# VCISwang/STCD

Hardware: AMD Instinct MI355X
Metric: image-pairs/sec (256x256 bf16 SiamUnet_diff train) (higher is better)
Workload: dtype bf16; 1 GPU; SiamUnet_diff(3,2) 256x256 full training step (fwd + cross_entropy + bwd + AdamW), 16 pairs/GPU, synthetic LEVIR-CD-shaped pairs resident in HBM; global_batch=16, image=256, parallelism=dp1

## Files before the change

include/stcd_hip.h:

```cpp
#ifndef STCD_HIP_H
#define STCD_HIP_H

#include <stdint.h>

#ifdef __cplusplus
extern "C" {
#endif

#define STCD_ABI_VERSION 2

#define STCD_ARCH_DIFF 0
#define STCD_ARCH_CONC 1
#define STCD_ARCH_SUB 2
#define STCD_ARCH_SNUNET 3
#define STCD_ARCH_SEGCD 4
#define STCD_ARCH_SEGCD_R18 5
#define STCD_ARCH_SEGCD_R34 6
#define STCD_ARCH_SEGCD_R101 7
#define STCD_ARCH_SEGCD_R152 8
#define STCD_ARCH_FCEF 9
#define STCD_ARCH_XCONC 10
#define STCD_ARCH_SNUNET_CONC 11
#define STCD_ARCH_SNUNET_CONC_DS 12
#define STCD_ARCH_UNETSEG 16
// ... 118 lines not shown
int64_t stcd_loss_iou_scratch_bytes(int batch, int classes, int64_t hw);
int stcd_loss_iou(const float* logits, const int64_t* target, int batch, int classes, int64_t hw, const float* weight, int mode,
                  float* loss_out, float* dlogits, void* scratch, void* hip_stream);
int stcd_confusion_update(const float* logits, const int64_t* target, int batch, int classes, int64_t hw,
                          int64_t* cm, void* hip_stream);

int stcd_adam_step(float* params, const float* grads, float* exp_avg, float* exp_avg_sq, int64_t numel, int64_t step,
                   double lr, double beta1, double beta2, double eps, double weight_decay, int decoupled, void* hip_stream);

int stcd_adam_hyper(int64_t step, double lr, double beta1, double beta2, double eps, double weight_decay, float* hyper_host8);
int stcd_adam_step_dev(float* params, const float* grads, float* exp_avg, float* exp_avg_sq, int64_t numel, const float* hyper_dev8,
                       int decoupled, void* hip_stream);

int stcd_pseudo_pair(const uint8_t* img_a, const uint8_t* donor, const uint8_t* mask, const uint8_t* change, const float* alpha,
                     const int32_t* erase_xywh, uint64_t seed, int batch, int height, int width, const float* mean3,
                     const float* std3, float* x1, float* x2, int64_t* c_label, int64_t* s_label_a, int64_t* s_label_b,
                     void* hip_stream);

int64_t stcd_augment_scratch_bytes(int n_images, int height, int width);
int stcd_augment(const float* x, const float* params, int n_images, int height, int width, const float* mean3, const float* std3,
                 float* out, void* scratch, int64_t scratch_bytes, void* hip_stream);

int stcd_scene_gather(const uint8_t* scene_a, const uint8_t* scene_b, int height, int width, int tile, int stride, int tiles_x,
                      int first_tile, int n_tiles, const float* mean3, const float* std3, float* x1, float* x2, void* hip_stream);
int stcd_scene_stitch(const float* logits, int classes, int height, int width, int tile, int stride, int tiles_x, int tiles_y,
                      int first_tile, int n_tiles, const float* window, float* acc, float* wsum, void* hip_stream);
int stcd_scene_finalize(const float* acc, const float* wsum, int classes, int height, int width, float threshold,
                        const uint8_t* label, uint8_t* mask, float* prob, int64_t* cm, void* hip_stream);
int stcd_scene_gather_d4(const uint8_t* scene_a, const uint8_t* scene_b, int height, int width, int tile, int stride, int tiles_x,
                         int first_tile, int n_tiles, const float* mean3, const float* std3, float* x1, float* x2, int d4,
                         void* hip_stream);
int stcd_scene_stitch_d4(const float* logits, int classes, int height, int width, int tile, int stride, int tiles_x, int tiles_y,
                         int first_tile, int n_tiles, const float* window, float* acc, float* wsum, int d4, void* hip_stream);
int stcd_scene_gather_one_d4(const uint8_t* scene, int height, int width, int tile, int stride, int tiles_x, int first_tile,
                             int n_tiles, const float* mean3, const float* std3, float* x, int d4, void* hip_stream);
#define STCD_SCENE_MAX_HEADS 3
int stcd_scene_stitch_heads_d4(const float* const* logits, int n_heads, int classes, int height, int width, int tile, int stride,
                               int tiles_x, int tiles_y, int first_tile, int n_tiles, const float* window, float* acc, float* wsum,
                               int d4, void* hip_stream);
int stcd_scene_finalize_seg(const float* acc, const float* wsum, int classes, int height, int width, float seg_threshold,
                            float change_threshold, const uint8_t* label_a, const uint8_t* label_b, const uint8_t* label_c,
                            uint8_t* seg_a, uint8_t* seg_b, uint8_t* change, uint8_t* gated, float* prob, int64_t* cm,
                            void* hip_stream);

#define STCD_SELFTRAIN_MAX_MODELS 8
int stcd_selftrain_score(const float* const* logits, int n_models, int batch, int classes, int64_t hw, float threshold,
                         const uint8_t* label, int mask_value, uint8_t* mask, int64_t* agree, int64_t* cm, void* hip_stream);

int stcd_scene_cell_agree(const uint8_t* const* masks, int n_models, int height, int width, int cell, int cells_x, int cells_y,
                          const uint8_t* label, int64_t* agree, int64_t* cm, void* hip_stream);
int stcd_mask_close(const uint8_t* in, int height, int width, int radius, int mask_value, uint8_t* out, void* hip_stream);

typedef struct stcd_conv_geom {
    int32_t n, hi, wi, ci, ldi;
    int32_t hm, wm, in_stride;
    int32_t ho, wo, out_stride, oy0, ox0;
    int32_t co, ldo;
    int32_t ntaps;
    int8_t dy[9], dx[9];
    int8_t pad_[2];
} stcd_conv_geom;

int stcd_op_conv(int dtype, int impl, const stcd_conv_geom* g, const void* in, const float* w, const float* bias,
                 void* out, void* scratch, int64_t scratch_bytes, void* hip_stream);
enum { STCD_CONV_SMALL = 0, STCD_CONV_RES = 1, STCD_CONV_TILE = 2, STCD_CONV_GEMM = 3, STCD_CONV_HALO = 4, STCD_CONV_DMA = 5 };
typedef struct stcd_conv_fused {
    int32_t kernel;
    int32_t groups;
    void* sum_acc;
    int32_t sum_c0, sum_c;
    float sum_scale1, sum_scale2;
    int32_t use_epi, relu;
    const void* gate;
    const void* res;
    int32_t ldg, ldr;
    float alpha, beta;
    const void* bw_y;
    const float* bw_stat;
    const float* bw_mask;
    void* bw_acc;
    int32_t bw_ldy;
    int32_t blocks, tiles_per_group, blocks_per_group, bn_rep;
    int32_t tile_m;
} stcd_conv_fused;
int stcd_op_conv_fused(const stcd_conv_geom* g, stcd_conv_fused* f, const void* in, const float* w, const float* bias, void* out,
                       void* scratch, int64_t scratch_bytes, void* hip_stream);
int stcd_op_wgrad(int dtype, int impl, const stcd_conv_geom* g, const void* in, const void* dout, float* dw,
                  void* scratch, int64_t scratch_bytes, void* hip_stream);
int64_t stcd_op_scratch_bytes(const stcd_conv_geom* g);

typedef struct stcd_map_geom {
    int32_t n, h, w, c, groups;
} stcd_map_geom;
int64_t stcd_op_ew_scratch_bytes(const stcd_map_geom* g);
int stcd_op_bn_act(int dtype, const stcd_map_geom* g, const void* y, int ldy, const float* gamma, const float* beta,
                   float* running_mean, float* running_var, const float* mask, int relu, int training, void* a, int lda,
                   void* pool, int ldp, float* stat, void* scratch, int64_t scratch_bytes, void* hip_stream);
int stcd_op_bn_act_pair(int dtype, const stcd_map_geom* g, const void* y, int ldy, const float* gamma, const float* beta,
                        float* running_mean, float* running_var, const float* mask, int fuse_mode, void* a, int lda, void* pool,
                        int ldp, void* fused, int ldf, float* stat, void* scratch, int64_t scratch_bytes, void* hip_stream);
int stcd_op_bn_act_bwd(int dtype, const stcd_map_geom* g, const void* da, int ldda, const void* y, int ldy, const float* stat,
                       const float* mask, int relu, void* dy, int lddy, float* dgamma, float* dbeta, void* scratch,
                       int64_t scratch_bytes, void* hip_stream);
int stcd_op_maxpool(int dtype, const stcd_map_geom* g, const void* a, int lda, void* pool, int ldp, void* hip_stream);
int stcd_op_maxpool_bwd(int dtype, const stcd_map_geom* g, const void* a, int lda, const void* dpool, int ldp, void* da, int ldda,
                        int accumulate, void* hip_stream);
int stcd_op_maxpool3(int dtype, const stcd_map_geom* g, const void* a, int lda, void* pool, int ldp, void* idx, void* hip_stream);
int stcd_op_maxpool3_bwd(int dtype, const stcd_map_geom* g, const void* idx, const void* dpool, int ldp, void* da, int ldda, void* hip_stream);
int64_t stcd_op_pairdw_scratch_bytes(const stcd_map_geom* g);
int stcd_op_pairdw(int dtype, const stcd_map_geom* g, const void* a, int lda, const float* w, const float* b, void* out, int ldo,
                   void* hip_stream);
int stcd_op_pairdw_bwd(int dtype, const stcd_map_geom* g, const void* a, int lda, const void* dout, int lddo, const float* w, void* da,
                       int ldda, float* dw, void* scratch, int64_t scratch_bytes, void* hip_stream);
int stcd_op_fuse(int dtype, int mode, const stcd_map_geom* g, const void* a, int lda, void* d, int ldd, void* hip_stream);
int stcd_op_fuse_bwd(int dtype, int mode, const stcd_map_geom* g, const void* a, int lda, const void* dd, int ldd, void* da, int ldda,
                     void* hip_stream);
int stcd_op_rep_pad(int dtype, const stcd_map_geom* g, void* d, int ld, int h0, int w0, void* hip_stream);
int stcd_op_rep_pad_bwd(int dtype, const stcd_map_geom* g, void* dd, int ld, int h0, int w0, void* hip_stream);
int stcd_op_skip_bwd(int dtype, int mode, const stcd_map_geom* g, const void* a, int lda, const void* y, int ldy, const void* dd,
                     int ldd, const void* dpool, int ldp, const float* stat, const float* mask, void* da, int ldda, void* dy,
                     int lddy, float* dgamma, float* dbeta, void* scratch, int64_t scratch_bytes, void* hip_stream);

int64_t stcd_op_cf_scratch_bytes(int64_t rows, int channels, int n, int q_tokens, int kv_tokens);
int stcd_op_cf_im2col(int dtype, const void* x, void* col, int ldc, int n, int h, int w, int c, int k, int stride, int pad, void* hip_stream);
int stcd_op_cf_col2im(int dtype, const void* dcol, int ldc, void* dx, int n, int h, int w, int c, int k, int stride, int pad, int accumulate,
                      void* hip_stream);
int stcd_op_cf_layernorm(int dtype, const void* x, void* y, const float* gamma, const float* beta, float* stats, int64_t rows, int c, float eps,
                         void* hip_stream);
int stcd_op_cf_layernorm_bwd(int dtype, const void* dy, const void* dy2, const void* x, const float* stats, const float* gamma, const void* add,
                             void* dx, float* dgamma, float* dbeta, void* scratch, int64_t rows, int c, void* hip_stream);
int stcd_op_cf_colsum(int dtype, const void* x, int64_t rows, int c, float* out, void* scratch, void* hip_stream);
int stcd_op_cf_attention(int dtype, const void* q, const void* kv, void* out, float* lse, int n, int q_tokens, int kv_tokens, int heads, int d,
                         float p, uint64_t seed, void* hip_stream);
int64_t stcd_op_cf_attention_scratch_bytes(int n, int q_tokens, int kv_tokens, int heads, int d);
int stcd_op_cf_attention_bwd(int dtype, const void* q, const void* kv, const void* out, const void* dout, const float* lse, void* dq, void* dkv,
                             void* scratch, int n, int q_tokens, int kv_tokens, int heads, int d, float p, uint64_t seed, void* hip_stream);
int stcd_op_cf_dwgelu(int dtype, const void* h, void* u, void* a, const float* w, const float* b, int n, int height, int width, int ch, float p,
                      uint64_t seed, void* hip_stream);
int64_t stcd_op_cf_dwgelu_scratch_bytes(int n, int height, int width, int ch);
int stcd_op_cf_dwgelu_bwd(int dtype, const void* h, const void* u, void* da, void* dh, const float* w, float* dw, float* db, void* scratch, int n,
                          int height, int width, int ch, float p, uint64_t seed, void* hip_stream);
int stcd_op_cf_resid_drop(int dtype, const void* x, const void* y, void* out, int n, int64_t rows_per_img, int c, float p, float path_p,
                          uint64_t seed, int backward, void* hip_stream);
int stcd_op_cf_bilinear(int dtype, const void* src, void* dst, int n, int h, int w, int out_h, int out_w, int c, int accumulate, int backward,
                        void* hip_stream);
int stcd_op_cf_elementwise(int dtype, int op, const void* x, const void* y, void* out, int64_t rows, int c, const float* alpha, float alpha_f,
                           float beta_f, float p, uint64_t seed, void* hip_stream);
int stcd_op_cf_prelu_bwd(int dtype, const void* dz, const void* y, void* dy, const float* alpha, float* dalpha, void* scratch, int64_t rows, int c,
                         void* hip_stream);

#ifdef __cplusplus
}
#endif
#endif
```

stcd_amd/_lib.py:

```python
from __future__ import annotations

import ctypes as C
import os

import torch

_HERE = os.path.dirname(os.path.abspath(__file__))
LIB_PATH = os.environ.get("STCD_LIB_PATH") or os.path.join(_HERE, "libstcd_hip.so")

ARCH_DIFF, ARCH_CONC, ARCH_SUB, ARCH_SNUNET, ARCH_SEGCD = 0, 1, 2, 3, 4
ARCH_SEGCD_R18, ARCH_SEGCD_R34, ARCH_SEGCD_R101, ARCH_SEGCD_R152 = 5, 6, 7, 8
ARCH_FCEF = 9
ARCH_XCONC = 10
ARCH_SNUNET_CONC = 11
ARCH_SNUNET_CONC_DS = 12
ARCH_UNETSEG = 16
ARCH_FFCTLCD = 32
ARCH_BASE_RESNET = 48
ARCH_BIT = 52
ARCH_CHANGEFORMER = 64
DTYPE_F32, DTYPE_BF16 = 0, 1
ARCH_IDS = {"diff": ARCH_DIFF, "conc": ARCH_CONC, "sub": ARCH_SUB, "fcef": ARCH_FCEF, "xconc": ARCH_XCONC, "snunet": ARCH_SNUNET, "snunet_conc": ARCH_SNUNET_CONC, "snunet_conc_ds": ARCH_SNUNET_CONC_DS, "segcd": ARCH_SEGCD,
            "segcd_resnet50": ARCH_SEGCD, "segcd_resnet18": ARCH_SEGCD_R18, "segcd_resnet34": ARCH_SEGCD_R34,
            "segcd_resnet101": ARCH_SEGCD_R101, "segcd_resnet152": ARCH_SEGCD_R152,
            "unetseg_resnet50": ARCH_UNETSEG, "unetseg_resnet18": ARCH_UNETSEG + 1, "unetseg_resnet34": ARCH_UNETSEG + 2,
            "unetseg_resnet101": ARCH_UNETSEG + 3, "unetseg_resnet152": ARCH_UNETSEG + 4,
            "ffctlcd_resnet50": ARCH_FFCTLCD, "ffctlcd_resnet18": ARCH_FFCTLCD + 1, "ffctlcd_resnet34": ARCH_FFCTLCD + 2,
            "ffctlcd_resnet101": ARCH_FFCTLCD + 3, "ffctlcd_resnet152": ARCH_FFCTLCD + 4,
            "base_resnet18_s5": ARCH_BASE_RESNET, "base_resnet18_s4": ARCH_BASE_RESNET + 1,
            "base_resnet34_s5": ARCH_BASE_RESNET + 2, "base_resnet34_s4": ARCH_BASE_RESNET + 3,
            "bit_s4_dd1_dh64": ARCH_BIT, "bit_s4_dd8_dh64": ARCH_BIT + 1, "bit_s4_dd8_dh8": ARCH_BIT + 2,
            "changeformer": ARCH_CHANGEFORMER}
DTYPE_IDS = {"fp32": DTYPE_F32, "f32": DTYPE_F32, "bf16": DTYPE_BF16}


class TensorInfo(C.Structure):
    _fields_ = [("name", C.c_char * 64), ("ndim", C.c_int32), ("shape", C.c_int64 * 4), ("offset", C.c_int64),
                ("numel", C.c_int64)]


class BnInfo(C.Structure):
    _fields_ = [("name", C.c_char * 64), ("channels", C.c_int32), ("calls_per_forward", C.c_int32),
                ("offset", C.c_int64)]


class DropoutInfo(C.Structure):
    _fields_ = [("name", C.c_char * 64), ("rows", C.c_int32), ("channels", C.c_int32), ("offset", C.c_int64)]


class ConvGeom(C.Structure):
    _fields_ = [("n", C.c_int32), ("hi", C.c_int32), ("wi", C.c_int32), ("ci", C.c_int32), ("ldi", C.c_int32),
                ("hm", C.c_int32), ("wm", C.c_int32), ("in_stride", C.c_int32),
                ("ho", C.c_int32), ("wo", C.c_int32), ("out_stride", C.c_int32), ("oy0", C.c_int32), ("ox0", C.c_int32),
                ("co", C.c_int32), ("ldo", C.c_int32), ("ntaps", C.c_int32),
                ("dy", C.c_int8 * 9), ("dx", C.c_int8 * 9), ("pad_", C.c_int8 * 2)]


class WsTensor(C.Structure):
    _fields_ = [("name", C.c_char * 96), ("offset_bytes", C.c_int64), ("n", C.c_int), ("h", C.c_int), ("w", C.c_int), ("c", C.c_int),
                ("ld", C.c_int), ("dtype", C.c_int)]


class CfConfig(C.Structure):
    _fields_ = [("in_ch", C.c_int32), ("out_ch", C.c_int32), ("embed_dims", C.c_int32 * 4), ("depths", C.c_int32 * 4),
                ("num_heads", C.c_int32 * 4), ("sr_ratios", C.c_int32 * 4), ("mlp_ratio", C.c_int32), ("embedding_dim", C.c_int32),
                ("patch1", C.c_int32), ("patch", C.c_int32), ("drop_rate", C.c_float), ("attn_drop", C.c_float),
                ("drop_path_rate", C.c_float), ("diff_drop", C.c_float)]


class CfSite(C.Structure):
    _fields_ = [("name", C.c_char * 96), ("ndim", C.c_int32), ("dims", C.c_int32 * 4), ("p", C.c_float)]


class MapGeom(C.Structure):
    _fields_ = [("n", C.c_int32), ("h", C.c_int32), ("w", C.c_int32), ("c", C.c_int32), ("groups", C.c_int32)]


CONV_SMALL, CONV_RES, CONV_TILE, CONV_GEMM, CONV_HALO, CONV_DMA = range(6)


class ConvFused(C.Structure):
    _fields_ = [("kernel", C.c_int32), ("groups", C.c_int32),
                ("sum_acc", C.c_void_p), ("sum_c0", C.c_int32), ("sum_c", C.c_int32), ("sum_scale1", C.c_float), ("sum_scale2", C.c_float),
                ("use_epi", C.c_int32), ("relu", C.c_int32), ("gate", C.c_void_p), ("res", C.c_void_p), ("ldg", C.c_int32), ("ldr", C.c_int32),
                ("alpha", C.c_float), ("beta", C.c_float),
                ("bw_y", C.c_void_p), ("bw_stat", C.c_void_p), ("bw_mask", C.c_void_p), ("bw_acc", C.c_void_p), ("bw_ldy", C.c_int32),
                ("blocks", C.c_int32), ("tiles_per_group", C.c_int32), ("blocks_per_group", C.c_int32), ("bn_rep", C.c_int32),
                ("tile_m", C.c_int32)]


_vp, _i, _i64, _f, _d = C.c_void_p, C.c_int, C.c_int64, C.c_float, C.c_double
_PROTOS = {
    "stcd_last_error": (C.c_char_p, []),
    "stcd_abi_version": (_i, []),
    "stcd_create": (_i, [_i, _i, _i, _i, C.POINTER(_vp)]),
    "stcd_destroy": (None, [_vp]),
    "stcd_cf_default_config": (_i, [C.POINTER(CfConfig)]),
    "stcd_create_changeformer": (_i, [C.POINTER(CfConfig), _i, C.POINTER(_vp)]),
    "stcd_output_floats": (_i64, [_vp]),
    "stcd_cf_output_info": (_i, [_vp, _i, C.POINTER(_i64), C.POINTER(_i), C.POINTER(_i)]),
    "stcd_cf_num_sites": (_i, [_vp]),
    "stcd_cf_site_get": (_i, [_vp, _i, C.POINTER(CfSite)]),
    "stcd_cf_site_seed": (C.c_uint32, [C.c_uint64, _i]),
    "stcd_cf_set_drop_rates": (_i, [_vp, _f, _f, _f]),
    "stcd_cf_set_aux_backward": (_i, [_vp, _i]),
    "stcd_set_wgrad_side": (_i, [_vp, _i]),
    "stcd_num_params": (_i, [_vp]),
    "stcd_param_info": (_i, [_vp, _i, C.POINTER(TensorInfo)]),
    "stcd_param_floats": (_i64, [_vp]),
    "stcd_num_bn": (_i, [_vp]),
    "stcd_bn_info_get": (_i, [_vp, _i, C.POINTER(BnInfo)]),
    "stcd_bn_floats": (_i64, [_vp]),
    "stcd_configure": (_i, [_vp, _i, _i, _i]),
    "stcd_workspace_bytes": (_i64, [_vp]),
    "stcd_num_dropout": (_i, [_vp]),
    "stcd_dropout_info_get": (_i, [_vp, _i, C.POINTER(DropoutInfo)]),
    "stcd_dropout_floats": (_i64, [_vp]),
    "stcd_set_dropout_p": (_i, [_vp, _f]),
    "stcd_forward": (_i, [_vp, _vp, _vp, _vp, _vp, _vp, C.c_uint64, _i, _vp, _vp, _vp]),
    "stcd_backward": (_i, [_vp, _vp, _vp, _vp, _vp, _i, _vp]),
    "stcd_grad_stage_range": (_i, [_vp, _i, C.POINTER(_i64), C.POINTER(_i64)]),
    "stcd_set_weights_tag": (_i, [_vp, C.c_uint64]),
    "stcd_set_debug": (_i, [_vp, _i]),
    "stcd_ws_tensor_count": (_i, [_vp]),
    "stcd_ws_tensor_get": (_i, [_vp, _i, C.POINTER(WsTensor)]),
    "stcd_profile_enable": (_i, [_vp, _i]),
    "stcd_profile_read": (_i, [_vp, _i, C.POINTER(C.c_double), C.POINTER(_i64), C.POINTER(C.c_double), C.POINTER(C.c_double)]),
    "stcd_profile_num_kernels": (_i, [_vp]),
    "stcd_profile_kernel": (_i, [_vp, _i, C.c_char_p, _i, C.POINTER(C.c_double), C.POINTER(_i64), C.POINTER(C.c_double), C.POINTER(C.c_double)]),
    "stcd_loss_scratch_bytes": (_i64, []),
    "stcd_loss_ce": (_i, [_vp, _vp, _i, _i, _i64, _i, _vp, _vp, _vp, _vp]),
    "stcd_loss_bce_dice": (_i, [_vp, _vp, _i64, _i, _vp, _vp, _vp, _vp]),
    "stcd_loss_contrastive": (_i, [_vp, _vp, _vp, _i64, _vp, _vp, _vp, _vp]),
    "stcd_loss_focal": (_i, [_vp, _vp, _i, _i, _i64, _vp, _f, _f, _i, _vp, _vp, _vp, _vp]),
    "stcd_loss_iou_scratch_bytes": (_i64, [_i, _i, _i64]),
    "stcd_loss_iou": (_i, [_vp, _vp, _i, _i, _i64, _vp, _i, _vp, _vp, _vp, _vp]),
    "stcd_confusion_update": (_i, [_vp, _vp, _i, _i, _i64, _vp, _vp]),
    "stcd_adam_step": (_i, [_vp, _vp, _vp, _vp, _i64, _i64, _d, _d, _d, _d, _d, _i, _vp]),
    "stcd_adam_hyper": (_i, [_i64, _d, _d, _d, _d, _d, C.POINTER(_f)]),
    "stcd_adam_step_dev": (_i, [_vp, _vp, _vp, _vp, _i64, _vp, _i, _vp]),
    "stcd_pseudo_pair": (_i, [_vp, _vp, _vp, _vp, _vp, _vp, C.c_uint64, _i, _i, _i, C.POINTER(_f), C.POINTER(_f), _vp, _vp, _vp, _vp, _vp, _vp]),
    "stcd_augment_scratch_bytes": (_i64, [_i, _i, _i]),
    "stcd_augment": (_i, [_vp, _vp, _i, _i, _i, C.POINTER(_f), C.POINTER(_f), _vp, _vp, _i64, _vp]),
    "stcd_scene_gather": (_i, [_vp, _vp, _i, _i, _i, _i, _i, _i, _i, C.POINTER(_f), C.POINTER(_f), _vp, _vp, _vp]),
    "stcd_scene_stitch": (_i, [_vp, _i, _i, _i, _i, _i, _i, _i, _i, _i, _vp, _vp, _vp, _vp]),
    "stcd_scene_finalize": (_i, [_vp, _vp, _i, _i, _i, _f, _vp, _vp, _vp, _vp, _vp]),
    "stcd_scene_gather_d4": (_i, [_vp, _vp, _i, _i, _i, _i, _i, _i, _i, C.POINTER(_f), C.POINTER(_f), _vp, _vp, _i, _vp]),
    "stcd_scene_stitch_d4": (_i, [_vp, _i, _i, _i, _i, _i, _i, _i, _i, _i, _vp, _vp, _vp, _i, _vp]),
    "stcd_scene_gather_one_d4": (_i, [_vp, _i, _i, _i, _i, _i, _i, _i, C.POINTER(_f), C.POINTER(_f), _vp, _i, _vp]),
    "stcd_scene_stitch_heads_d4": (_i, [C.POINTER(_vp), _i, _i, _i, _i, _i, _i, _i, _i, _i, _i, _vp, _vp, _vp, _i, _vp]),
    "stcd_scene_finalize_seg": (_i, [_vp, _vp, _i, _i, _i, _f, _f, _vp, _vp, _vp, _vp, _vp, _vp, _vp, _vp, _vp, _vp]),
    "stcd_selftrain_score": (_i, [C.POINTER(_vp), _i, _i, _i, _i64, _f, _vp, _i, _vp, _vp, _vp, _vp]),
    "stcd_scene_cell_agree": (_i, [C.POINTER(_vp), _i, _i, _i, _i, _i, _i, _vp, _vp, _vp, _vp]),
    "stcd_mask_close": (_i, [_vp, _i, _i, _i, _i, _vp, _vp]),
    "stcd_op_conv": (_i, [_i, _i, C.POINTER(ConvGeom), _vp, _vp, _vp, _vp, _vp, _i64, _vp]),
    "stcd_op_conv_fused": (_i, [C.POINTER(ConvGeom), C.POINTER(ConvFused), _vp, _vp, _vp, _vp, _vp, _i64, _vp]),
    "stcd_op_wgrad": (_i, [_i, _i, C.POINTER(ConvGeom), _vp, _vp, _vp, _vp, _i64, _vp]),
    "stcd_op_scratch_bytes": (_i64, [C.POINTER(ConvGeom)]),
    "stcd_op_ew_scratch_bytes": (_i64, [C.POINTER(MapGeom)]),
    "stcd_op_bn_act": (_i, [_i, C.POINTER(MapGeom), _vp, _i, _vp, _vp, _vp, _vp, _vp, _i, _i, _vp, _i, _vp, _i, _vp, _vp, _i64, _vp]),
    "stcd_op_bn_act_pair": (_i, [_i, C.POINTER(MapGeom), _vp, _i, _vp, _vp, _vp, _vp, _vp, _i, _vp, _i, _vp, _i, _vp, _i, _vp, _vp, _i64, _vp]),
    "stcd_op_bn_act_bwd": (_i, [_i, C.POINTER(MapGeom), _vp, _i, _vp, _i, _vp, _vp, _i, _vp, _i, _vp, _vp, _vp, _i64, _vp]),
    "stcd_op_maxpool": (_i, [_i, C.POINTER(MapGeom), _vp, _i, _vp, _i, _vp]),
    "stcd_op_maxpool_bwd": (_i, [_i, C.POINTER(MapGeom), _vp, _i, _vp, _i, _vp, _i, _i, _vp]),
    "stcd_op_maxpool3": (_i, [_i, C.POINTER(MapGeom), _vp, _i, _vp, _i, _vp, _vp]),
    "stcd_op_maxpool3_bwd": (_i, [_i, C.POINTER(MapGeom), _vp, _vp, _i, _vp, _i, _vp]),
    "stcd_op_pairdw_scratch_bytes": (_i64, [C.POINTER(MapGeom)]),
    "stcd_op_pairdw": (_i, [_i, C.POINTER(MapGeom), _vp, _i, _vp, _vp, _vp, _i, _vp]),
    "stcd_op_pairdw_bwd": (_i, [_i, C.POINTER(MapGeom), _vp, _i, _vp, _i, _vp, _vp, _i, _vp, _vp, _i64, _vp]),
    "stcd_op_fuse": (_i, [_i, _i, C.POINTER(MapGeom), _vp, _i, _vp, _i, _vp]),
    "stcd_op_fuse_bwd": (_i, [_i, _i, C.POINTER(MapGeom), _vp, _i, _vp, _i, _vp, _i, _vp]),
    "stcd_op_rep_pad": (_i, [_i, C.POINTER(MapGeom), _vp, _i, _i, _i, _vp]),
    "stcd_op_rep_pad_bwd": (_i, [_i, C.POINTER(MapGeom), _vp, _i, _i, _i, _vp]),
    "stcd_op_skip_bwd": (_i, [_i, _i, C.POINTER(MapGeom), _vp, _i, _vp, _i, _vp, _i, _vp, _i, _vp, _vp, _vp, _i, _vp, _i, _vp, _vp, _vp, _i64, _vp]),
    "stcd_op_cf_scratch_bytes": (_i64, [_i64, _i, _i, _i, _i]),
    "stcd_op_cf_im2col": (_i, [_i, _vp, _vp, _i, _i, _i, _i, _i, _i, _i, _i, _vp]),
    "stcd_op_cf_col2im": (_i, [_i, _vp, _i, _vp, _i, _i, _i, _i, _i, _i, _i, _i, _vp]),
    "stcd_op_cf_layernorm": (_i, [_i, _vp, _vp, _vp, _vp, _vp, _i64, _i, _f, _vp]),
    "stcd_op_cf_layernorm_bwd": (_i, [_i, _vp, _vp, _vp, _vp, _vp, _vp, _vp, _vp, _vp, _vp, _i64, _i, _vp]),
    "stcd_op_cf_colsum": (_i, [_i, _vp, _i64, _i, _vp, _vp, _vp]),
    "stcd_op_cf_attention": (_i, [_i, _vp, _vp, _vp, _vp, _i, _i, _i, _i, _i, _f, C.c_uint64, _vp]),
    "stcd_op_cf_attention_scratch_bytes": (_i64, [_i, _i, _i, _i, _i]),
    "stcd_op_cf_attention_bwd": (_i, [_i, _vp, _vp, _vp, _vp, _vp, _vp, _vp, _vp, _i, _i, _i, _i, _i, _f, C.c_uint64, _vp]),
    "stcd_op_cf_dwgelu": (_i, [_i, _vp, _vp, _vp, _vp, _vp, _i, _i, _i, _i, _f, C.c_uint64, _vp]),
    "stcd_op_cf_dwgelu_scratch_bytes": (_i64, [_i, _i, _i, _i]),
    "stcd_op_cf_dwgelu_bwd": (_i, [_i, _vp, _vp, _vp, _vp, _vp, _vp, _vp, _vp, _i, _i, _i, _i, _f, C.c_uint64, _vp]),
    "stcd_op_cf_resid_drop": (_i, [_i, _vp, _vp, _vp, _i, _i64, _i, _f, _f, C.c_uint64, _i, _vp]),
    "stcd_op_cf_bilinear": (_i, [_i, _vp, _vp, _i, _i, _i, _i, _i, _i, _i, _i, _vp]),
    "stcd_op_cf_elementwise": (_i, [_i, _i, _vp, _vp, _vp, _i64, _i, _vp, _f, _f, _f, C.c_uint64, _vp]),
    "stcd_op_cf_prelu_bwd": (_i, [_i, _vp, _vp, _vp, _vp, _vp, _vp, _i64, _i, _vp]),
}
EXPORTS = tuple(_PROTOS)

_lib = None


class StcdError(RuntimeError):
    pass


def lib():
    global _lib
    if _lib is None:
        if not os.path.exists(LIB_PATH):
            raise StcdError(
                f"{LIB_PATH} is missing: build it with `python -c 'import __graft_entry__ as g; g.build()'` "
                "or `make -C stcd_amd/csrc`.  The engine has no CPU fallback.")
        l = C.CDLL(LIB_PATH)
        for name, (res, args) in _PROTOS.items():
            fn = getattr(l, name)
            fn.restype, fn.argtypes = res, args
        if l.stcd_abi_version() != 2:
            raise StcdError("libstcd_hip.so ABI version mismatch")
        _lib = l
    return _lib


def check(rc: int):
    if rc != 0:
        raise StcdError(lib().stcd_last_error().decode("utf-8", "replace"))
```

stcd_amd/csrc/common.h:

```cpp
#pragma once
#include <hip/hip_runtime.h>
#include <stdint.h>
#include <stdio.h>
#include <stdlib.h>
#include <string>
#include <string.h>

#include "../../include/stcd_hip.h"

namespace stcd {

typedef __bf16 bf16;

enum DType { F32 = STCD_DTYPE_F32, BF16 = STCD_DTYPE_BF16 };
inline size_t dsize(int dt) { return dt == BF16 ? 2 : 4; }

void set_error(const std::string& msg);

static inline int env_int(const char* name, int dflt) { const char* v = getenv(name); return v ? atoi(v) : dflt; }
static inline bool env_flag(const char* name, bool dflt) { const char* v = getenv(name); return v && v[0] == (dflt ? '0' : '1') ? !dflt : dflt; }

#define STCD_CHECK_AS(fn, cond, msg)                                       \
    do {                                                                   \
        if (!(cond)) {                                                     \
// ... 171 lines not shown

void launch_conv_ref(int dt, const stcd_conv_geom& g, const void* in, const float* w, int kpad, int wld,
                     const float* bias, void* out, bool out_nchw_f32, hipStream_t s);
void launch_wgrad_ref(int dt, const stcd_conv_geom& g, const void* in, const void* dout, float* dw, int kpad, int wld,
                      hipStream_t s);
void launch_wgrad_ref_f64(int dt, const stcd_conv_geom& g, const void* in, const void* dout, double* dw, int kpad, int wld,
                          hipStream_t s);

struct ConvMfmaPlan {
    int CiB = 0, nchunks = 0, KS = 0, modeB = 0, NT = 0, NTtot = 0;
    int64_t wf_elems = 0;
    bool ok = false;
};
ConvMfmaPlan conv_mfma_plan(const stcd_conv_geom& g);
void launch_pack_frag(const stcd_conv_geom& g, const ConvMfmaPlan& p, const float* w, int kpad, int wld, void* dst,
                      hipStream_t s);
int launch_conv_mfma(const stcd_conv_geom& g, const ConvMfmaPlan& p, const void* in, const void* wf, const float* bias,
                     void* out, bool out_nchw_f32, hipStream_t s);
bool conv_mfma_x4_ok(const stcd_conv_geom g[4], const ConvMfmaPlan p[4]);
int launch_conv_mfma_x4(const stcd_conv_geom g[4], const ConvMfmaPlan p[4], const void* in, const void* const wf[4],
                        const float* bias, void* out, hipStream_t s);
struct ConvResPlan {
    int NT = 0, CW = 32, nslices = 0, P = 0, blocks = 0;
    int filt_bytes = 0, lds_bytes = 0;
    int single_halo = 0;
    bool ok = false;
};
ConvResPlan conv_res_plan(const stcd_conv_geom& g, const ConvMfmaPlan& p, int groups);
struct BwdSum {
    const void* Y = nullptr; int ldy = 0;
    const float* stat = nullptr;
    const float* mask = nullptr;
    long long* acc = nullptr;
    int groups = 1;
};
int launch_conv_res(const stcd_conv_geom& g, const ConvMfmaPlan& p, const ConvResPlan& rp, const void* in, const void* wf,
                    const float* bias, void* out, int groups, long long* stat_acc, int cpad, hipStream_t s, int stat_c0 = 0,
                    float s1_scale = BN_FS1, float s2_scale = BN_FS2, const XfSrc* xf = nullptr, const BwdSum* bs = nullptr);
bool conv_res_bwdsum_ok(const stcd_conv_geom& g, const ConvResPlan& rp);
bool conv_res_xf_ok(const stcd_conv_geom& g, const ConvResPlan& rp, int groups, const XfSrc& xf);
struct ConvTilePlan {
    int NT = 0, nparts = 0, nbuf = 0, nslices = 0, P = 0, blocks = 0, ntiles = 0;
    int filt_bytes = 0, lds_bytes = 0;
    bool ok = false;
};
ConvTilePlan conv_tile_plan(const stcd_conv_geom& g, const ConvMfmaPlan& p, int groups);
int launch_conv_tile(const stcd_conv_geom& g, const ConvMfmaPlan& p, const ConvTilePlan& tp, const void* in, const void* wf,
                     const float* bias, void* out, int groups, long long* stat_acc, int cpad, hipStream_t s, int stat_c0 = 0,
                     float s1_scale = BN_FS1, float s2_scale = BN_FS2);
struct ConvGemmPlan {
    int W = 0;
    int tiles_m = 0, tiles_n = 0, blocks = 0, lds_bytes = 0;
    int pix_chunks = 0;
    bool ok = false;
};
ConvGemmPlan conv_gemm_plan(const stcd_conv_geom& g, const ConvMfmaPlan& p, int groups);
struct ConvEpi {
    int relu = 0;
    const void* gate = nullptr; int ldg = 0;
    const void* res = nullptr; int ldr = 0;
    float alpha = 1.f, beta = 1.f;
};
int launch_conv_gemm(const stcd_conv_geom& g, const ConvMfmaPlan& p, const ConvGemmPlan& gp, const void* in, const void* wf,
                   const float* bias, void* out, int groups, long long* stat_acc, int cpad, hipStream_t s, int stat_c0 = 0,
                   float s1_scale = BN_FS1, float s2_scale = BN_FS2, const ConvEpi* epi = nullptr);
struct ConvHaloPlan {
    int NH = 0;
    int nslices = 0, P = 0, blocks = 0, lds_bytes = 0;
    bool ok = false;
};
ConvHaloPlan conv_halo_plan(const stcd_conv_geom& g, const ConvMfmaPlan& p);
int launch_conv_halo(const stcd_conv_geom& g, const ConvMfmaPlan& p, const ConvHaloPlan& hp, const void* in, const void* wf,
                     const float* bias, void* out, hipStream_t s, const ConvEpi* epi = nullptr);

struct ConvDmaPlan {
    int tiles_m = 0, tiles_n = 0, blocks = 0, lds_bytes = 0;
    bool ok = false;
};
ConvDmaPlan conv_dma_plan(const stcd_conv_geom& g, const ConvMfmaPlan& p);
int launch_conv_dma(const stcd_conv_geom& g, const ConvMfmaPlan& p, const ConvDmaPlan& dp, const void* in, const void* wf,
                    const float* bias, void* out, hipStream_t s, const ConvEpi* epi = nullptr);

bool conv_small_ok(const stcd_conv_geom& g, const ConvMfmaPlan& p);
int conv_small_blocks(const stcd_conv_geom& g, int groups);
int launch_conv_small(const stcd_conv_geom& g, const void* in, const void* wf_modeB, const float* bias, void* out,
                      bool out_nchw_f32, int groups, long long* stat_acc, int cpad, hipStream_t s, const XfSrc* xf = nullptr,
                      const BwdSum* bs = nullptr);
bool conv_small_call_ok(const stcd_conv_geom& g, int groups, const XfSrc* xf);
bool conv_small_bwdsum_ok(const stcd_conv_geom& g);
struct WgradMfmaPlan {
    int WCI = 1, NTW = 1, gx = 1, gy = 1, gz = 1;
    int64_t slab_floats = 0;
    int wi_valid = 0;
    int gemm = 0;
    int dma = 0;
    bool ok = false;
};
WgradMfmaPlan wgrad_mfma_plan(const stcd_conv_geom& g, int kpad, int wld, bool allow_wide = false, int force_co64 = -1);
int launch_wgrad_mfma(const stcd_conv_geom& g, const WgradMfmaPlan& p, const void* in, const void* dout, float* slab,
                      int kpad, int wld, hipStream_t s);
struct WgradJob {
    stcd_conv_geom g;
    int64_t in_off, dout_off, slab_off;
    int kpad, wld;
    int dymin, dxmin, HH, HWp;
    int tiles_x, tiles_y, ntiles;
    int xrow_bytes;
    int x_bytes, y_bytes;
    int co_valid;
    unsigned in_bytes, dout_bytes;
    int gx, gy, gz;
    int start;
    int lds_bytes;
    int wi_valid;
    int dma_L, dma_nk;
    int pad_;
    int64_t xf_stat_off, xf_mask_off;
    int xf_C, xf_groups, xf_npg, pad2_;
};
WgradMfmaPlan wgrad_gemm_plan(const stcd_conv_geom& g, int kpad, int wld);
WgradJob wgrad_gemm_make_job(const stcd_conv_geom& g, const WgradMfmaPlan& p, int64_t in_off, int64_t dout_off, int64_t slab_off,
                             int kpad, int wld);
int launch_wgrad_gemm_group(int W, const WgradJob* jobs_dev, int njobs, int total_blocks, const char* base, hipStream_t s);
WgradMfmaPlan wgrad_dma_plan(const stcd_conv_geom& g, int kpad, int wld);
void wgrad_dma_set_split(WgradMfmaPlan& p, const stcd_conv_geom& g, int S, int kpad, int wld);
WgradJob wgrad_dma_make_job(const stcd_conv_geom& g, const WgradMfmaPlan& p, int64_t in_off, int64_t dout_off, int64_t slab_off,
                            int kpad, int wld);
int launch_wgrad_dma_group(const WgradJob* jobs_dev, int njobs, int total_blocks, const char* base, hipStream_t s);
WgradJob wgrad_make_job(const stcd_conv_geom& g, const WgradMfmaPlan& p, int64_t in_off, int64_t dout_off, int64_t slab_off,
                        int kpad, int wld);
void wgrad_job_set_xf(WgradJob& a, int64_t stat_off, int64_t mask_off, int C, int groups, int npg);
int wgrad_variant_slots(int WCI, int NTW, bool t9, int lds_bytes);
int launch_wgrad_group(int WCI, int NTW, bool t9, const WgradJob* jobs_dev, int njobs, int total_blocks, int lds_bytes,
                       const char* base, hipStream_t s, bool xf = false);
struct PackSpec;
struct ReduceJob {
    int64_t start, count;
    int64_t slab_off;
    int64_t out_off;
    int64_t slab_stride;
    int gx, ntaps, K, N, kpad, wld;
    int ks, kn_major;
    int8_t ky[9], kx[9];
    int8_t tiled, parts, pad_[4];
};
void launch_reduce_jobs(const ReduceJob* jobs_dev, int njobs, int64_t total, const char* ws, float* grads, hipStream_t s);
void launch_reduce_dw(const float* slab, int gx, const stcd_conv_geom& g, int K, int N, int kpad, int wld,
                      const PackSpec* ps, float* out, hipStream_t s);

struct PackSpec {
    int ks;
    int kn_major;
    int K, N, wld;
    int kpad;
    int ntaps;
    int8_t ky[9], kx[9];
};
void launch_pack_w(const PackSpec& ps, const float* src, float* dst, hipStream_t s);
void launch_unpack_dw(const PackSpec& ps, const double* dwe, float* gsrc, hipStream_t s);

struct PackJob {
    int64_t start, count;
    int64_t src_off;
    int64_t dst_off;
    int kind;
    PackSpec ps;
    int Ci, Co, CiB, nchunks, KS, NTtot, modeB;
    int aux;
};
void launch_pack_jobs(const PackJob* jobs_dev, int njobs, int64_t total, const float* params, char* ws, hipStream_t s);
// ... 243 lines not shown
```

stcd_amd/csrc/engine.hip:

```cpp
#include <algorithm>
#include <climits>
#include <cstdint>
#include <array>
#include <cstring>
#include <memory>
#include <vector>

#include "common.h"

namespace stcd {

static thread_local std::string g_err;
void set_error(const std::string& msg) { g_err = msg; }

enum ConvKind { K_CONV3 = 0, K_CONVT3_S1 = 1, K_UPCONV = 2, K_CONV1 = 3, K_CONVT2 = 4, K_CONV3_S2 = 5, K_CONV1_S2 = 6, K_STEM7 = 7 };

struct TRef { int64_t off = -1; int ld = 0; };
struct GRef { int64_t off = -1; int ld = 0; int64_t goff = 0; };

static inline int round8(int c) { return (c + 7) & ~7; }

struct ConvW {
    std::string name;
    int kind = 0, cin = 0, cout = 0;
    int kin_p = 0, nout_p = 0;
    int64_t w_off = 0, b_off = 0;
    PackSpec fwd{}, dgrad{};
    int64_t wpk_fwd = -1, wpk_dgrad = -1, dwe = -1;
    int64_t dwe_floats = 0;
};
struct BnP {
    std::string name;
    int C = 0, calls = 1;
    int64_t g_off = 0, b_off = 0;
    int64_t run_off = 0;
};
struct DropP { std::string name; int rows = 0, C = 0; int64_t off = 0; };

struct ConvOp {
    stcd_conv_geom g{};
    int conv = -1; bool dgrad = false;
    int tap0 = 0;
    int kreal = 0, nreal = 0;
    ConvMfmaPlan plan; int64_t wf = -1;
    bool small = false;
    ConvResPlan res; int res_groups = 1;
    ConvGemmPlan gemm;
    ConvDmaPlan dma;
    ConvHaloPlan halo;
    ConvTilePlan tile;
};
struct WgradOp {
    stcd_conv_geom g{};
    int conv = -1, tap0 = 0, kreal = 0, nreal = 0;
    WgradMfmaPlan plan;
    int64_t slab = -1;
    int stage = 0;
    int64_t in_off = -1, dout_off = -1;
    bool grouped = false;
    int group = -1;
    int64_t xf_stat_off = -1, xf_mask_off = -1; int xf_C = 0, xf_groups = 1, xf_npg = 1;
    bool own_taps = false;
    int8_t oky[9] = {0}, okx[9] = {0};
};
struct WgradGroup {
    int WCI = 1, NTW = 1; bool t9 = false;
    bool xf = false;
    int gemm = 0;
    int dma = 0;
    std::vector<WgradJob> jobs;
    int total_blocks = 0, lds_bytes = 0;
    int64_t table_off = -1;
    double flops = 0.0, bytes = 0.0;
    int seen = 0; bool launched = false;
};

struct Cbrd {
    ConvOp fwd, dgr; WgradOp wg;
    int conv = -1, bn = -1, drop = -1;
    int N = 0, H = 0, W = 0, groups = 1, npg = 0;
    TRef in; int K = 0;
    TRef Y; GRef A; TRef P; TRef dPool; bool pool = false;
    GRef dA; TRef dY; TRef dIn; bool has_dIn = false;
    int64_t stat = -1;
    int64_t facc = -1, bacc = -1;
    const Cbrd* dgr_bwd = nullptr;
    bool bwd_sums_fused = false;
    int64_t dgr_sum_acc = -1; int dgr_sum_c0 = 0, dgr_sum_C = 0;
    TRef fuse_dst;
    bool virt = false; const Cbrd* xsrc = nullptr;
};
struct XConc {
    int level = 0, C = 0;
    int64_t w_off = 0, b_off = 0;
    int bn1 = -1;
    TRef G, dG, R, dR;
    int64_t stat1 = -1, facc1 = -1, bacc1 = -1, part = -1;
    Cbrd res;
};
struct UpConv {
    int conv = -1, level = 0;
    int N = 0, h = 0, w = 0, Ho = 0, Wo = 0, C = 0;
    TRef in, out, dOut, dIn;
    ConvOp fwd[4], dgr; WgradOp wg[4];
    int64_t bias_acc = -1; bool bias_fused = false;
};

enum ProfClass { PC_CONV = 0, PC_WGRAD = 1, PC_BN_STATS = 2, PC_BN_ACT = 3, PC_BN_BWD_REDUCE = 4, PC_BN_BWD_APPLY = 5,
                 PC_POOL_FUSE = 6, PC_PACK = 7, PC_COUNT = 8 };
struct ProfRec { hipEvent_t a, b; int klass; int name_id; double flops, bytes; };
struct Prof {
    bool on = false;
    std::vector<ProfRec> recs;
    std::vector<hipEvent_t> pool;
    std::vector<std::string> names;
    size_t used = 0;
    int intern(const std::string& n) {
        for (size_t i = 0; i < names.size(); ++i)
            if (names[i] == n) return (int)i;
        names.push_back(n);
        return (int)names.size() - 1;
    }
    hipEvent_t get() {
        if (used == pool.size()) { hipEvent_t ev; (void)hipEventCreate(&ev); pool.push_back(ev); }
        return pool[used++];
    }
    ~Prof() { for (auto ev : pool) (void)hipEventDestroy(ev); }
};

struct ViewRef { int64_t off = 0; int ld = 0; int64_t goff = 0; int gmask = 1; };
struct GLayer {
    std::string name;
    int conv = -1, bn = -1, kind = K_CONV3;
    int N = 0, Hi = 0, Wi = 0, Ho = 0, Wo = 0, K = 0, C = 0, groups = 2, npg = 0;
    bool relu = true;
    TRef in, Y, A, res;
    TRef dA, dIn, dRes;
    bool has_dIn = true;
    std::vector<ViewRef> extra_dst;
    std::vector<ViewRef> grad_src;
    bool grad_base = true;
    ConvOp fwd, dgr[4]; int ndgr = 0; WgradOp wg[8]; int nwg = 0;
    int64_t stat = -1, coef = -1, facc = -1, bacc = -1;
    int g_first = 0;
};
enum GStepKind { GS_LAYER = 0, GS_MAXPOOL = 1, GS_UPSAMPLE = 2, GS_ABSDIFF = 3, GS_BCONV = 4, GS_ABSPAIR = 5, GS_BILINEAR = 6,
                 GS_TOKENIZE = 7, GS_TOKENENC = 8, GS_TOKENDEC = 9 };
struct GStep { int kind = GS_LAYER; int layer = -1; TRef src, dst, dsrc, ddst; int N = 0, h = 0, w = 0, C = 0; };

struct SrcSlice { TRef src; TRef dsrc; int C = 0; int prod = -1; int grp = -1; };
struct NBlock {
    std::string name;
    int c1 = -1, bn1 = -1, c2 = -1, bn2 = -1;
    int N = 0, H = 0, W = 0, groups = 1, npg = 0, Cin = 0, C = 0;
    TRef in, dIn;
    std::vector<SrcSlice> srcs;
    int up = -1;
    TRef Y1, A1, Y2, Out, P, dOut, dP, dZ2, dA1;
    bool pool = false;
    int64_t stat1 = -1, stat2 = -1;
    int64_t facc1 = -1, bacc1 = -1, facc2 = -1, bacc2 = -1;
    int64_t d1_sum_acc = -1; int d1_sum_c0 = 0, d1_sum_C = 0;
    std::vector<ViewRef> extra_dst;
    std::vector<ViewRef> grad_src;
    bool grad_base = false;
    ConvOp f1, f2, d1, d2; WgradOp w1, w2;
};
struct SnUp {
    int conv = -1, N = 0, h = 0, w = 0, C = 0;
    TRef src, dsrc, out, dOut, tmp;
    ConvOp fwd[4], dgr; WgradOp wg[4];
    int64_t bias_acc = -1; bool bias_fused = false; int coff = 0;
};

struct CfPlan;
struct stcd_engine_impl {
    Prof prof;
    std::shared_ptr<CfPlan> cf;
    std::vector<NBlock> sn_blocks;
    std::vector<SnUp> sn_ups;
    std::vector<int> sn_order;
    std::vector<XConc> xc;
    int sn_final = -1;
    int64_t sn_w[4] = {0, 0, 0, 0};
    TRef snE, sndE, snZ, sndZ;
    int64_t sn_pool = -1, sn_argm = -1, sn_att = -1, sn_hid = -1, sn_sums = -1, sn_dpool = -1, sn_part = -1;
    int64_t sn_dout_begin = -1, sn_dout_end = -1;
    ConvOp sn_final_fwd, sn_final_dgr; WgradOp sn_final_wg;
    int64_t snc_w[5] = {0, 0, 0, 0, 0}, snc_b[5] = {0, 0, 0, 0, 0}, snc_scratch = -1;
    std::vector<GLayer> g_layers;
    std::vector<GStep> g_fwd;
    int g_stem = -1, g_head_conv = -1;
    int debug_flags = 0;
    std::vector<stcd_ws_tensor> ws_tensors;
    std::vector<std::array<int, 4>> g_blocks;
    int seg_x = 4, seg_layers[4] = {3, 4, 6, 3};
    int seg_dates = 2;
    bool seg_ffc = false;
    TRef g_pool_idc;
    std::vector<std::array<int, 2>> g_dec;
    TRef gP0, gdP0, gX3, gdX3, gFuseTmp;
    int64_t g_pool_idx = -1;
    int64_t g_stem_part = -1;
    int64_t g_raw3 = -1, g_draw3 = -1;
    ConvOp g_head_fwd, g_head_dgr; WgradOp g_head_wg;
    bool bres = false; int seg_nstage = 4;
    int g_head_c = 16;
    int g_cls = -1, g_pred_conv = -1;
    ConvOp g_pred_fwd, g_pred_dgr; WgradOp g_pred_wg;
    int64_t g_pred_bias_acc = -1;
    struct BitPlan {
        bool on = false; int L = 1, dh = 64;
        int64_t pos_off = 0, wa_off = 0, enc_off = 0, dec_off = 0;
        int64_t tok_in = -1, tok_out = -1, dtok_out = -1, dtok_in = -1, stat = -1, AP = -1, dAP = -1, xs = -1, dG = -1, dec_part = -1,
                dmh = -1, dm = -1, enc_part = -1, tok_part = -1;
        TRef dec_din;
    } bit;
    int arch = 0, in_ch = 3, label = 2, dt = F32;
    int64_t min_bn_count = 0;
    float drop_p = 0.2f;
    std::vector<stcd_tensor_info> params;
    int64_t param_floats = 0, enc_param_end = 0;
    std::vector<ConvW> convs;
    std::vector<BnP> bns;
    int64_t bn_floats = 0;
    bool configured = false, fwd_training = false;
    int B = 0, H = 0, W = 0;
    std::vector<DropP> drops;
    int64_t drop_floats = 0;
    int64_t ws_bytes = 0;
    std::vector<Cbrd> enc, dec;
    std::vector<UpConv> ups;
    int final_conv = -1;
    ConvOp final_fwd, final_dgr; WgradOp final_wg;
    const Cbrd* final_dgr_bwd = nullptr;
    const Cbrd* final_xsrc = nullptr;
    int use_virt = 0;
    int fc_virt_layers = 0;
    std::vector<ConvOp*> conv_ops;
    int64_t slab = -1, slab_floats = 0;
    std::vector<WgradOp*> wgrad_ops;
    std::vector<WgradGroup> wgroups[2];
    std::vector<ReduceJob> rjobs[2];
    int64_t rjobs_total[2] = {0, 0}, rjobs_off[2] = {-1, -1};
    std::vector<PackJob> jobs[2];
    int64_t jobs_total[2] = {0, 0}, jobs_off[2] = {-1, -1};
    const void* jobs_uploaded_ws = nullptr;
    uint64_t weights_tag = 0, packed_tag = 0;
    const void* packed_ws = nullptr; const void* packed_params = nullptr; int packed_level = -1;
    TRef X0, G, finalIn, dFinalIn;
    int Hs[5] = {0}, Ws[5] = {0};
    TRef D[4], dD[4], P[4], dP[4];
    int64_t zero_begin = -1, zero_end = -1;
    int64_t final_bias_acc = -1;
    std::vector<BiasJob> bias_jobs; int64_t bias_jobs_off = -1;
    int64_t masks = -1, dwe_begin = -1, dwe_end = -1, scratch8 = -1;
    int use_mfma = 1, use_small = 1, use_wgroup = 1, use_res = 1, use_skip_fused = 1, use_act_fuse = 1, use_gemm = 1, use_skip_recompute = 1, use_bwdsum = 1, use_bwdsum_res = 0, use_tile = 1, use_halo = 0;
    int wg_side_on = 1;
    static constexpr int WG_SIDE_DIV = 4;
    static constexpr int WGROUP_ROUNDS = 1, WGROUP_MIN_TILES = 8;
    bool wg_early = false; hipStream_t wg_cur_side = nullptr;
    hipStream_t wg_side = nullptr; hipEvent_t wg_fork = nullptr, wg_join = nullptr; int wg_side_dev = -1;
};

}

using namespace stcd;
struct stcd_engine : stcd_engine_impl {};

namespace stcd {

static const int ENC_STAGE_CONVS[4] = {2, 2, 3, 3};
static const int ENC_C[4] = {16, 32, 64, 128};
static const int SKIP_IDX[4] = {1, 3, 6, 9};

static void add_param(stcd_engine& e, const std::string& name, std::initializer_list<int64_t> shape, int64_t* off_out) {
    stcd_tensor_info ti;
    memset(&ti, 0, sizeof(ti));
    snprintf(ti.name, sizeof(ti.name), "%s", name.c_str());
    ti.ndim = (int)shape.size();
    int64_t n = 1;
    int i = 0;
    for (auto s : shape) { ti.shape[i++] = s; n *= s; }
    ti.numel = n;
    ti.offset = e.param_floats;
    *off_out = ti.offset;
    e.param_floats += (n + 3) & ~(int64_t)3;
    e.params.push_back(ti);
}

static void make_specs(ConvW& c, bool need_dgrad) {
    if (c.kind == K_STEM7) {
        c.fwd = PackSpec{}; c.dgrad = PackSpec{};
        c.fwd.ks = 7; c.fwd.K = c.cin; c.fwd.N = c.cout; c.fwd.kpad = c.kin_p; c.fwd.wld = c.nout_p;
        return;
    }
    if (c.kind == K_CONV3_S2) {
        PackSpec& f = c.fwd;
        f.ks = 3; f.K = c.cin; f.N = c.cout; f.kpad = c.kin_p; f.wld = c.nout_p; f.ntaps = 9; f.kn_major = 0;
        {
            int t = 0;
            for (int py = 0; py < 2; ++py)
                for (int px = 0; px < 2; ++px)
                    for (int ky = 0; ky < 3; ++ky)
                        for (int kx = 0; kx < 3; ++kx)
                            if ((ky != 1) == (py == 1) && (kx != 1) == (px == 1)) { f.ky[t] = ky; f.kx[t] = kx; ++t; }
        }
        PackSpec& d = c.dgrad;
        d.ks = 3; d.K = c.cout; d.N = c.cin; d.kpad = c.nout_p; d.wld = round8(c.cin); d.ntaps = need_dgrad ? 9 : 0; d.kn_major = 1;
        int t = 0;
        for (int py = 0; py < 2; ++py)
            for (int px = 0; px < 2; ++px)
                for (int dy = 0; dy <= py; ++dy)
                    for (int dx = 0; dx <= px; ++dx) { d.ky[t] = py + 1 - 2 * dy; d.kx[t] = px + 1 - 2 * dx; ++t; }
        return;
    }
    if (c.kind == K_CONV1 || c.kind == K_CONVT2 || c.kind == K_CONV1_S2) {
        const int ks = c.kind == K_CONVT2 ? 2 : 1;
        PackSpec& f = c.fwd;
        f.ks = ks; f.K = c.cin; f.N = c.cout; f.kpad = c.kin_p; f.wld = c.nout_p;
        f.ntaps = ks * ks;
        f.kn_major = c.kind == K_CONVT2;
        for (int t = 0; t < f.ntaps; ++t) { f.ky[t] = t / ks; f.kx[t] = t % ks; }
        PackSpec& d = c.dgrad;
        d.ks = ks; d.K = c.cout; d.N = c.cin; d.kpad = c.nout_p; d.wld = round8(c.cin);
        d.ntaps = need_dgrad ? ks * ks : 0;
        d.kn_major = c.kind != K_CONVT2;
        for (int t = 0; t < ks * ks; ++t) { d.ky[t] = t / ks; d.kx[t] = t % ks; }
        return;
    }
    PackSpec& f = c.fwd;
    f.ks = 3;
    f.K = c.cin; f.N = c.cout; f.kpad = c.kin_p; f.wld = c.nout_p;
    PackSpec& d = c.dgrad;
    d.ks = 3;
    d.K = c.cout; d.N = c.cin; d.kpad = c.nout_p; d.wld = round8(c.cin);
    d.ntaps = 0;
    if (c.kind == K_CONV3 || c.kind == K_CONVT3_S1) {
        f.ntaps = 9;
        f.kn_major = c.kind == K_CONVT3_S1;
// ... 114 lines not shown
        }
    }
}

struct Bump {
    int64_t cur = 0;
    int64_t take(int64_t bytes) {
        int64_t o = cur;
        cur += (bytes + 255) & ~(int64_t)255;
        return o;
    }
};

static int conv_index(const stcd_engine& e, const std::string& name) {
    for (size_t i = 0; i < e.convs.size(); ++i)
        if (e.convs[i].name == name) return (int)i;
    return -1;
}
static int bn_index(const stcd_engine& e, const std::string& name) {
    for (size_t i = 0; i < e.bns.size(); ++i)
        if (e.bns[i].name == name) return (int)i;
    return -1;
}

static stcd_conv_geom geom3(int N, int H, int W, int K, int ldi, int co, int ldo) {
    stcd_conv_geom g;
    memset(&g, 0, sizeof(g));
    g.n = N; g.hi = H; g.wi = W; g.ci = K; g.ldi = ldi;
    g.hm = H; g.wm = W; g.in_stride = 1;
    g.ho = H; g.wo = W; g.out_stride = 1; g.oy0 = 0; g.ox0 = 0;
    g.co = co; g.ldo = ldo;
    g.ntaps = 9;
    for (int t = 0; t < 9; ++t) { g.dy[t] = (int8_t)(t / 3 - 1); g.dx[t] = (int8_t)(t % 3 - 1); }
    return g;
}

static stcd_conv_geom geom_up_phase(const UpConv& U, int py, int px, int ldi, int ldo, int* tap0) {
    stcd_conv_geom g;
    memset(&g, 0, sizeof(g));
    g.n = U.N; g.hi = U.h; g.wi = U.w; g.ci = U.C; g.ldi = ldi;
    g.hm = U.h; g.wm = U.w; g.in_stride = 1;
    g.ho = U.Ho; g.wo = U.Wo; g.out_stride = 2; g.oy0 = py; g.ox0 = px;
    g.co = U.C; g.ldo = ldo;
    int t = 0;
    for (int dy = 0; dy <= py; ++dy)
        for (int dx = 0; dx <= px; ++dx) { g.dy[t] = (int8_t)dy; g.dx[t] = (int8_t)dx; ++t; }
    g.ntaps = t;
    static const int start[4] = {0, 1, 3, 5};
    *tap0 = start[py * 2 + px];
    return g;
}

static void conv_work(const stcd_engine& e, const stcd_conv_geom& g, int kreal, int nreal, double* flops, double* bytes);

static void pick_gemm_or_res(const stcd_engine& e, ConvOp& op, const stcd_conv_geom& g, int groups) {
    if (!e.use_gemm || op.small) return;
    if (op.res.ok && !(e.cf && op.res.NT == 1)) return;
    op.gemm = conv_gemm_plan(g, op.plan, groups);
    if (!op.gemm.ok) return;
    op.res = ConvResPlan();
    if ((int64_t)g.n * g.hm * g.wm >= 256 * 192) op.dma = conv_dma_plan(g, op.plan);
    if (e.use_halo && (int64_t)g.n * ((g.hm + 15) / 16) * ((g.wm + 15) / 16) >= 512) op.halo = conv_halo_plan(g, op.plan);
}

constexpr int TILE_MAX_TILES = 512;
static void pick_tile(const stcd_engine& e, ConvOp& op, const stcd_conv_geom& g, int groups) {
    if (!e.use_tile || !op.res.ok || op.gemm.ok || op.small) return;
    const ConvTilePlan tp = conv_tile_plan(g, op.plan, groups);
    if (tp.ok && tp.ntiles <= TILE_MAX_TILES) op.tile = tp;
}

static WgradMfmaPlan pick_wgrad_plan(const stcd_engine& e, const stcd_conv_geom& g, int kpad, int wld) {
    if (e.use_gemm && e.use_wgroup && 2.0 * g.n * g.hm * g.wm * (double)g.ci * g.co >= 0.8e9) {
        WgradMfmaPlan p = wgrad_gemm_plan(g, kpad, wld);
        if (p.ok) return p;
    }
    if (e.use_wgroup && (g.ntaps == 9 || (e.cf && g.ntaps == 4)) && (int64_t)g.n * g.hm * g.wm >= 65536) {
        WgradMfmaPlan p = wgrad_dma_plan(g, kpad, wld);
        if (p.ok) return p;
    }
    return wgrad_mfma_plan(g, kpad, wld, is_snunet(e.arch) || (e.cf && g.ntaps == 9));
}

static void plan_conv(const stcd_engine& e, ConvOp& op, int groups, bool with_tile) {
    op.plan = conv_mfma_plan(op.g);
    op.small = conv_small_ok(op.g, op.plan);
    if (e.use_res && !op.small) op.res = conv_res_plan(op.g, op.plan, groups);
    pick_gemm_or_res(e, op, op.g, groups);
    if (with_tile) pick_tile(e, op, op.g, groups);
}
static bool conv_on_ref(bool mfma, const ConvOp& op) { return !(mfma && op.plan.ok && op.wf >= 0); }
struct Binder {
    stcd_engine& e; Bump& ws;
    bool with_tile = false;
    void conv(ConvOp& op, const stcd_conv_geom& g, int conv, bool dgrad, int tap0, int kreal, int nreal, int groups = 1) const {
        op = ConvOp();
        op.g = g; op.conv = conv; op.dgrad = dgrad; op.tap0 = tap0; op.kreal = kreal; op.nreal = nreal; op.res_groups = groups;
        if (e.dt == BF16) plan_conv(e, op, groups, with_tile);
        if (op.plan.ok) op.wf = ws.take(op.plan.wf_elems * 2);
        e.conv_ops.push_back(&op);
    }
    void stem(ConvOp& op, const stcd_conv_geom& g, int conv, int groups) const {
        op = ConvOp();
        op.g = g; op.conv = conv; op.kreal = e.convs[conv].cin; op.nreal = g.co; op.res_groups = groups;
        op.plan = conv_mfma_plan(g);
        if (g.ldi == 8 && g.co % 64 == 0) op.gemm = conv_gemm_plan(g, op.plan, groups);
        op.gemm.pix_chunks = 1;
        if (!op.gemm.ok) return;
        op.wf = ws.take(op.plan.wf_elems * 2);
        e.conv_ops.push_back(&op);
    }
    void wgrad(WgradOp& op, const stcd_conv_geom& g, int conv, int64_t in_off, int64_t dout_off, int stage = 0, int tap0 = 0,
               int wi_valid = 0, const int8_t* own_ky = nullptr, const int8_t* own_kx = nullptr) const {
        const ConvW& cv = e.convs[conv];
        op = WgradOp();
        op.g = g; op.conv = conv; op.tap0 = tap0; op.kreal = cv.cin; op.nreal = cv.cout;
        op.in_off = in_off; op.dout_off = dout_off; op.stage = stage;
        op.own_taps = own_ky != nullptr;
        for (int t = 0; t < g.ntaps && op.own_taps; ++t) { op.oky[t] = own_ky[t]; op.okx[t] = own_kx[t]; }
        if (e.dt == BF16) { op.plan = pick_wgrad_plan(e, g, cv.fwd.kpad, cv.fwd.wld); op.plan.wi_valid = wi_valid; }
        e.wgrad_ops.push_back(&op);
    }
};
static void take_ref_images(stcd_engine& e, Bump& ws, bool with_dwe = true) {
    for (auto& c : e.convs) {
        c.wpk_fwd = ws.take((int64_t)c.fwd.ntaps * c.fwd.kpad * c.fwd.wld * 4);
        if (c.dgrad.ntaps) c.wpk_dgrad = ws.take((int64_t)c.dgrad.ntaps * c.dgrad.kpad * c.dgrad.wld * 4);
    }
    e.dwe_begin = ws.cur;
    for (auto& c : e.convs) {
        c.dwe_floats = (int64_t)c.fwd.ntaps * c.fwd.kpad * c.fwd.wld;
        c.dwe = with_dwe ? ws.take(c.dwe_floats * 8) : -1;
    }
    e.dwe_end = ws.cur;
}

static bool same_group(const WgradGroup& G, const WgradOp& op) {
    const bool t9 = !op.plan.dma && op.g.ntaps == 9;
    return G.gemm == op.plan.gemm && G.dma == op.plan.dma && G.WCI == op.plan.WCI && G.NTW == op.plan.NTW && G.t9 == t9 && G.xf == (op.xf_C > 0);
}

static bool cf_side_on() { static const bool on = env_flag("STCD_CF_SIDE", true); return on; }

static void build_pack_jobs(stcd_engine& e, Bump& ws) {
    for (int st = 0; st < 2; ++st) { e.rjobs[st].clear(); e.rjobs_total[st] = 0; }
    for (int st = 0; st < 2; ++st) e.wgroups[st].clear();
    if (e.dt == BF16 && e.use_mfma) {
        if (e.use_wgroup) {
            for (WgradOp* op : e.wgrad_ops) {
                if (!op->plan.ok) continue;
                const bool t9 = !op->plan.dma && op->g.ntaps == 9;
                std::vector<WgradGroup>& gs = e.wgroups[op->stage];
                size_t gi = 0;
                while (gi < gs.size() && !same_group(gs[gi], *op)) ++gi;
                if (gi == gs.size()) { WgradGroup g; g.WCI = op->plan.WCI; g.NTW = op->plan.NTW; g.t9 = t9; g.gemm = op->plan.gemm; g.dma = op->plan.dma; g.xf = op->xf_C > 0; gs.push_back(g); }
                op->grouped = true;
            }
            for (int st = 0; st < 2; ++st)
                for (WgradGroup& G : e.wgroups[st]) {
                    if (G.gemm) { G.lds_bytes = 2 * 2 * G.gemm * (64 * 64 + 8 * 32); continue; }
                    if (G.dma) {
                        G.lds_bytes = 128 * 1024;
                        std::vector<WgradOp*> dops;
                        for (WgradOp* op : e.wgrad_ops)
                            if (op->grouped && op->stage == st && op->plan.dma) dops.push_back(op);
                        auto blocks_at = [&](int64_t kt) {
                            int64_t b = 0;
                            for (WgradOp* op : dops) {
                                const int64_t M = (int64_t)op->g.n * op->g.hi * op->g.wi;
                                b += ((M + kt * 64 - 1) / (kt * 64)) * op->plan.gy * op->plan.gz;
                            }
                            return b;
                        };
                        int64_t lo = 1, hi = 1;
                        const int dma_blocks = e.wg_side_on && cf_side_on() ? 192 : 256;
                        while (blocks_at(hi) > dma_blocks) hi *= 2;
                        while (lo < hi) { const int64_t mid = (lo + hi) / 2; if (blocks_at(mid) <= dma_blocks) hi = mid; else lo = mid + 1; }
                        for (WgradOp* op : dops) {
                            const ConvW& cv = e.convs[op->conv];
                            const int64_t M = (int64_t)op->g.n * op->g.hi * op->g.wi;
                            int64_t S = (M + lo * 64 - 1) / (lo * 64);
                            const int64_t slab_bytes = (int64_t)op->g.ntaps * cv.fwd.kpad * cv.fwd.wld * 4;
                            S = std::min<int64_t>(S, std::max<int64_t>(1, ((int64_t)64 << 20) / slab_bytes));
                            wgrad_dma_set_split(op->plan, op->g, (int)S, cv.fwd.kpad, cv.fwd.wld);
                        }
                        continue;
                    }
                    std::vector<WgradOp*> ops;
                    int64_t W = 0;
                    for (WgradOp* op : e.wgrad_ops)
                        if (op->grouped && op->stage == st && same_group(G, *op)) {
                            ops.push_back(op);
                            const int64_t ntiles = (int64_t)op->g.n * ((op->g.wm + 15) / 16) * ((op->g.hm + 7) / 8);
// ... 217 lines not shown
            L.conv = conv_index(e, std::string("conv") + d.sfx[j]);
            L.bn = bn_index(e, std::string("bn") + d.sfx[j]);
            L.drop = add_drop(std::string("do") + d.sfx[j], B, d.cout[j]);
            const int C = d.cout[j];
            L.N = B; L.H = h; L.W = w; L.groups = 1; L.npg = B;
            L.in = in; L.K = K;
            L.Y = plain(B, h, w, C);
            TRef a = plain(B, h, w, C), da = plain(B, h, w, C);
            L.A.off = a.off; L.A.ld = C; L.A.goff = 0;
            L.dA.off = da.off; L.dA.ld = C; L.dA.goff = 0;
            L.dY = da;
            L.has_dIn = true; L.dIn = dIn;
            L.stat = ws.take((int64_t)4 * C * 4);
            e.dec.push_back(L);
            in = a; dIn = da; K = C;
            prevA = a; prevdA = da;
        }
    }
    if (fc_cross(e)) {
        for (int s = 0; s < 4; ++s) {
            XConc& X = e.xc[s];
            const int C = ENC_C[s], h = e.Hs[s], w = e.Ws[s];
            X.G = plain(B, h, w, C); X.dG = plain(B, h, w, C); X.R = plain(B, h, w, C); X.dR = plain(B, h, w, C);
            X.stat1 = ws.take((int64_t)4 * C * 4);
            X.part = ws.take(pairdw_partial_floats(B, h, w, C) * 4);
            Cbrd& L = X.res;
            L.drop = -1; L.N = B; L.H = h; L.W = w; L.groups = 1; L.npg = B;
            L.in = X.R; L.K = C;
            L.Y = plain(B, h, w, C);
            L.A.off = e.D[s].off + C * T; L.A.ld = e.D[s].ld; L.A.goff = 0;
            L.dA.off = e.dD[s].off + C * T; L.dA.ld = e.dD[s].ld; L.dA.goff = 0;
            L.dY = plain(B, h, w, C);
            L.has_dIn = true; L.dIn = X.dR;
            L.stat = ws.take((int64_t)4 * C * 4);
        }
    }
    e.G = plain(B, H, W, 8);
    for (auto& X : e.xc) {
        X.facc1 = za.take(bn_acc_bytes(1, X.C)); X.bacc1 = za.take(bn_acc_bytes(1, X.C));
        X.res.facc = za.take(bn_acc_bytes(1, X.C)); X.res.bacc = za.take(bn_acc_bytes(1, X.C));
    }
    for (auto& L : e.enc) { L.facc = za.take(bn_acc_bytes(L.groups, e.convs[L.conv].cout)); L.bacc = za.take(bn_acc_bytes(L.groups, e.convs[L.conv].cout)); }
    for (auto& L : e.dec) { L.facc = za.take(bn_acc_bytes(L.groups, e.convs[L.conv].cout)); L.bacc = za.take(bn_acc_bytes(L.groups, e.convs[L.conv].cout)); }
    for (auto& U : e.ups) U.bias_acc = za.take(bn_acc_bytes(1, U.C));
    e.final_bias_acc = za.take(bn_acc_bytes(1, 8));
    if (za.cur > e.zero_end) { set_error("internal: zero arena overflow"); return 1; }
    e.scratch8 = ws.take(256);
    e.masks = ws.take(e.drop_floats * 4);
    take_ref_images(e, ws);

    e.conv_ops.clear();
    e.wgrad_ops.clear();
    e.slab_floats = 0;
    const Binder bind{e, ws, true};
    auto wg_stage = [&](int conv) { return e.convs[conv].w_off < e.enc_param_end ? 1 : 0; };
    auto bind_cbrd = [&](Cbrd& L) {
        const ConvW& cv = e.convs[L.conv];
        bind.conv(L.fwd, geom3(L.N, L.H, L.W, L.K, L.in.ld, cv.cout, L.Y.ld), L.conv, false, 0, cv.cin, cv.cout, L.groups);
        bind.wgrad(L.wg, geom3(L.N, L.H, L.W, L.K, L.in.ld, cv.cout, L.dY.ld), L.conv, L.in.off, L.dY.off, wg_stage(L.conv));
        if (L.has_dIn)
            bind.conv(L.dgr, geom3(L.N, L.H, L.W, cv.dgrad.kpad, L.dY.ld, cv.cin, L.dIn.ld), L.conv, true, 0, cv.cout, cv.cin,
                      (e.use_bwdsum && e.use_bwdsum_res) ? L.groups : 1);
    };
    for (auto& L : e.enc) bind_cbrd(L);
    for (auto& L : e.dec) bind_cbrd(L);
    for (auto& X : e.xc) bind_cbrd(X.res);
    for (auto& U : e.ups) {
        const ConvW& cv = e.convs[U.conv];
        for (int ph = 0; ph < 4; ++ph) {
            int tap0;
            stcd_conv_geom g = geom_up_phase(U, ph >> 1, ph & 1, U.in.ld, U.out.ld, &tap0);
            bind.conv(U.fwd[ph], g, U.conv, false, tap0, U.C, U.C);
            bind.wgrad(U.wg[ph], g, U.conv, U.in.off, U.dOut.off, wg_stage(U.conv), tap0);
        }
        stcd_conv_geom gd;
        memset(&gd, 0, sizeof(gd));
        gd.n = U.N; gd.hi = U.Ho; gd.wi = U.Wo; gd.ci = cv.dgrad.kpad; gd.ldi = U.dOut.ld;
        gd.hm = U.h; gd.wm = U.w; gd.in_stride = 2;
        gd.ho = U.h; gd.wo = U.w; gd.out_stride = 1;
        gd.co = U.C; gd.ldo = U.dIn.ld;
        gd.ntaps = 9;
        for (int t = 0; t < 9; ++t) { gd.dy[t] = (int8_t)(t / 3 - 1); gd.dx[t] = (int8_t)(t % 3 - 1); }
        bind.conv(U.dgr, gd, U.conv, true, 0, U.C, U.C);
    }
    {
        const ConvW& cv = e.convs[e.final_conv];
        bind.conv(e.final_fwd, geom3(B, H, W, cv.kin_p, e.finalIn.ld, e.label, e.label), e.final_conv, false, 0, cv.cin, e.label);
        bind.wgrad(e.final_wg, geom3(B, H, W, cv.kin_p, e.finalIn.ld, e.label, 8), e.final_conv, e.finalIn.off, e.G.off, wg_stage(e.final_conv));
        bind.conv(e.final_dgr, geom3(B, H, W, cv.dgrad.kpad, 8, cv.cin, e.dFinalIn.ld), e.final_conv, true, 0, e.label, cv.cin);
    }
    e.slab = ws.take(e.slab_floats * 4);

    for (auto& L : e.enc) { L.dgr_bwd = nullptr; L.bwd_sums_fused = false; }
    for (auto& L : e.dec) { L.dgr_bwd = nullptr; L.bwd_sums_fused = false; }
    e.final_dgr_bwd = nullptr;
    if (e.use_bwdsum && e.dt == BF16 && e.use_mfma && e.use_small && !e.use_virt) {
        const int res_too = e.use_bwdsum_res;
        auto dest_ok = [&](const Cbrd& P, const ConvOp& dgr, int64_t dIn_off, int dIn_ld, int N) {
            const bool kern = (dgr.small && conv_small_bwdsum_ok(dgr.g)) ||
                              (res_too && !dgr.small && !dgr.gemm.ok && e.use_res && dgr.res.ok && dgr.res_groups == P.groups &&
                               conv_res_bwdsum_ok(dgr.g, dgr.res));
            return !P.pool && P.fuse_dst.off < 0 && !P.virt && kern && dgr.wf >= 0 && dIn_off == P.dA.off && dIn_ld == P.dA.ld &&
                   e.convs[P.conv].cout == dgr.g.co && P.N == N && N % P.groups == 0 &&
                   (P.groups == 1 || P.dA.goff == (int64_t)P.npg * P.H * P.W * P.dA.ld);
        };
        auto scan = [&](std::vector<Cbrd>& v) {
            for (size_t i = 1; i < v.size(); ++i) {
                Cbrd& N = v[i]; Cbrd& P = v[i - 1];
                if (N.has_dIn && N.dgr_sum_acc < 0 && dest_ok(P, N.dgr, N.dIn.off, N.dIn.ld, N.N)) { N.dgr_bwd = &P; P.bwd_sums_fused = true; }
            }
        };
        scan(e.enc); scan(e.dec);
        if (!e.dec.empty() && dest_ok(e.dec.back(), e.final_dgr, e.dFinalIn.off, e.dFinalIn.ld, e.dec.back().N)) {
            e.final_dgr_bwd = &e.dec.back(); e.dec.back().bwd_sums_fused = true;
        }
    }

    e.final_xsrc = nullptr; e.fc_virt_layers = 0;
    for (auto& L : e.enc) { L.virt = false; L.xsrc = nullptr; }
    for (auto& L : e.dec) { L.virt = false; L.xsrc = nullptr; }
    if (e.use_virt && e.dt == BF16 && e.use_mfma && e.use_wgroup && !fc_cross(e)) {
        auto fwd_ok = [&](const ConvOp& op, bool nchw) {
            if (op.wf < 0 || (op.gemm.ok && !nchw)) return false;
            if (op.small && e.use_small) return true;
            return op.res.ok && !nchw && !op.res.single_halo;
        };
        auto wg_ok = [&](const WgradOp& op) { return op.plan.ok && !op.plan.gemm && !op.plan.dma && op.plan.WCI < 4 && op.plan.NTW < 4; };
        auto link = [&](Cbrd& P, ConvOp& cf, WgradOp& cw, bool nchw) {
            if (P.pool || P.fuse_dst.off >= 0) return false;
            if (!fwd_ok(cf, nchw) || !wg_ok(cw)) return false;
            P.virt = true; ++e.fc_virt_layers;
            cw.in_off = P.Y.off;
            cw.xf_stat_off = P.stat;
            cw.xf_mask_off = (P.drop >= 0) ? e.masks + e.drops[P.drop].off * 4 : -1;
            cw.xf_C = e.convs[P.conv].cout; cw.xf_groups = P.groups; cw.xf_npg = P.npg;
            return true;
        };
        for (size_t i = 0; i + 1 < e.enc.size(); ++i) {
            Cbrd& P = e.enc[i]; Cbrd& Cn = e.enc[i + 1];
            if (Cn.in.off != P.A.off) continue;
            if (link(P, Cn.fwd, Cn.wg, false)) { Cn.xsrc = &P; Cn.in.off = P.Y.off; Cn.in.ld = P.Y.ld; }
        }
        for (size_t i = 0; i < e.dec.size(); ++i) {
            Cbrd& P = e.dec[i];
            if (i + 1 < e.dec.size() && e.dec[i + 1].in.off == P.A.off) {
                Cbrd& Cn = e.dec[i + 1];
                if (link(P, Cn.fwd, Cn.wg, false)) { Cn.xsrc = &P; Cn.in.off = P.Y.off; Cn.in.ld = P.Y.ld; }
            } else if (e.finalIn.off == P.A.off) {
                if (link(P, e.final_fwd, e.final_wg, true)) { e.final_xsrc = &P; e.finalIn.off = P.Y.off; e.finalIn.ld = P.Y.ld; }
            }
        }
    }

    e.bias_jobs.clear();
    {
        size_t di = 0;
        for (int k = 0; k < 4; ++k) {
            UpConv& U = e.ups[k];
            Cbrd& L = e.dec[di];
            int nb = 0;
            for (int j = 0; j < DEC[k].n; ++j) nb += DEC[k].cout[j] >= 0;
            di += nb;
            U.bias_fused = false;
            const bool even = 2 * U.h == U.Ho && 2 * U.w == U.Wo;
            if (e.dt == BF16 && e.use_mfma && nb > 0 && L.has_dIn && L.dIn.off == U.dOut.off && L.dgr.res.ok && L.dgr.wf >= 0 && even) {
                U.bias_fused = true;
// ... 51 lines not shown

struct Ctx {
    stcd_engine& e;
    char* ws;
    const float* params;
    float* grads;
    hipStream_t s;
    template <typename P = void> P* at(int64_t off) const { return (P*)(ws + off); }
};

struct ProfScope {
    Prof& p; hipStream_t s; bool on; hipEvent_t b;
    ProfScope(const Ctx& c, int klass, double flops, double bytes, const char* kernel = nullptr);
    ~ProfScope() { if (on) (void)hipEventRecord(b, s); }
};

ProfScope::ProfScope(const Ctx& c, int klass, double flops, double bytes, const char* kernel)
    : p(c.e.prof), s(c.s), on(c.e.prof.on), b(nullptr) {
    if (!on) return;
    static const char* DEF[PC_COUNT] = {"k_conv", "k_wgrad", "k_bn_reduce<T, 0>", "k_bn_act", "k_bn_reduce<T, 1>", "k_bn_bwd_apply",
                                        "k_pool_bwd|k_fuse|k_slice", "k_pack_jobs|k_reduce_dw"};
    ProfRec r;
    r.a = p.get(); r.b = p.get(); r.klass = klass; r.flops = flops; r.bytes = bytes;
    r.name_id = p.intern(kernel ? kernel : DEF[klass]);
    b = r.b;
    p.recs.push_back(r);
    (void)hipEventRecord(r.a, s);
}

static void conv_work(const stcd_engine& e, const stcd_conv_geom& g, int kreal, int nreal, double* flops, double* bytes) {
    double pos = (double)g.n * g.hm * g.wm;
    *flops = 2.0 * pos * g.ntaps * kreal * nreal;
    double in_px = g.in_stride == 1 ? pos : (double)g.n * (2.0 * g.hm) * (2.0 * g.wm);
    *bytes = (in_px * kreal + pos * nreal + (double)g.ntaps * kreal * nreal) * (double)dsize(e.dt);
}

static bool mfma_on(const stcd_engine& e) { return e.dt == BF16 && e.use_mfma; }

struct StatReq { long long* acc = nullptr; int groups = 1; int c0 = 0; int C = 0; float s1 = BN_FS1, s2 = BN_FS2; };

enum class ConvKernel { REF, MFMA, SMALL, RES, TILE, GEMM, HALO, DMA };
constexpr unsigned conv_kernel_bit(ConvKernel k) { return 1u << (int)k; }
struct ConvCall {
    bool nchw = false;
    int stat_groups = 0;
    bool bn_form = false;
    const XfSrc* xf = nullptr;
    bool bwd = false;
    unsigned allowed = ~0u;
};
static int conv_small_groups(const ConvCall& k) {
    return (k.xf && k.xf->on) ? k.xf->groups : (k.stat_groups > 0 && k.bn_form) ? k.stat_groups : 1;
}
static ConvKernel conv_kernel(bool mfma, bool use_small, const ConvOp& op, const ConvCall& k) {
    auto may = [&](ConvKernel x) { return (k.allowed & conv_kernel_bit(x)) != 0; };
    if (conv_on_ref(mfma, op)) return ConvKernel::REF;
    const bool xf_on = k.xf && k.xf->on, stats = k.stat_groups > 0;
    const bool small = op.small && use_small;
    if (k.bwd) return small ? ConvKernel::SMALL : ConvKernel::RES;
    if (op.gemm.ok && !k.nchw) {
        if (op.dma.ok && op.res_groups == 1 && !stats && may(ConvKernel::DMA)) return ConvKernel::DMA;
        if (op.halo.ok && !stats && may(ConvKernel::HALO)) return ConvKernel::HALO;
        return ConvKernel::GEMM;
    }
    if (small && conv_small_call_ok(op.g, conv_small_groups(k), k.xf)) return ConvKernel::SMALL;
    if (op.res.ok && !k.nchw && !small) {
        if (op.tile.ok && !xf_on && may(ConvKernel::TILE)) return ConvKernel::TILE;
        if (!xf_on || conv_res_xf_ok(op.g, op.res, op.res_groups, *k.xf)) return ConvKernel::RES;
    }
    return ConvKernel::MFMA;
}
static void conv_kernel_name(ConvKernel kern, const ConvOp& op, bool bwd, char (&kname)[64]) {
    switch (kern) {
        case ConvKernel::DMA: snprintf(kname, sizeof(kname), "k_conv_dma"); break;
        case ConvKernel::HALO: snprintf(kname, sizeof(kname), "k_conv_halo"); break;
        case ConvKernel::GEMM: snprintf(kname, sizeof(kname), "k_conv_gemm<%d>", op.gemm.W); break;
        case ConvKernel::TILE: snprintf(kname, sizeof(kname), "k_conv_tile<%d>", op.tile.NT); break;
        case ConvKernel::RES:
            if (bwd) snprintf(kname, sizeof(kname), "k_conv_res<bwd>");
            else snprintf(kname, sizeof(kname), "k_conv_res<%d, %d, %s>", op.res.NT, op.res.CW, op.res.single_halo ? "true" : "false");
            break;
        case ConvKernel::SMALL:
            if (bwd) snprintf(kname, sizeof(kname), "k_conv_small<bwd>");
            else snprintf(kname, sizeof(kname), "k_conv_small<1, %d>", (op.g.ntaps * op.g.ci + 31) / 32 <= 5 ? 5 : 9);
            break;
        case ConvKernel::MFMA: snprintf(kname, sizeof(kname), "k_conv_mfma<%d>", op.plan.NT); break;
        case ConvKernel::REF: snprintf(kname, sizeof(kname), "k_conv_ref"); break;
    }
}

static void exec_conv(const Ctx& c, const ConvOp& op, const void* in, const float* bias, void* out, bool nchw,
                      const StatReq* sr = nullptr, int* stat_chunks = nullptr, const ConvEpi* epi = nullptr, int* epi_fused = nullptr,
                      const XfSrc* xf = nullptr, const BwdSum* bs = nullptr) {
    const ConvW& cv = c.e.convs[op.conv];
    long long* stat_acc = sr ? sr->acc : nullptr;
    ConvCall call;
    call.nchw = nchw; call.xf = xf; call.bwd = bs != nullptr;
    call.stat_groups = stat_acc ? sr->groups : 0;
    call.bn_form = sr && sr->c0 == 0 && sr->C == op.g.co && sr->s1 == BN_FS1 && sr->s2 == BN_FS2;
    const ConvKernel kern = conv_kernel(mfma_on(c.e), c.e.use_small, op, call);
    double fl, by;
    conv_work(c.e, op.g, op.kreal, op.nreal, &fl, &by);
    if (bs) by += (double)op.g.n * op.g.ho * op.g.wo * op.g.co * 2.0;
    char kname[64];
    conv_kernel_name(kern, op, bs != nullptr, kname);
    ProfScope prof(c, PC_CONV, fl, by, kname);
    if (stat_chunks) *stat_chunks = 0;
    if (epi_fused) *epi_fused = 0;
    if (xf && xf->on && kern != ConvKernel::SMALL && kern != ConvKernel::RES) {
        set_error("internal: a virtual-activation input reached a convolution kernel without the staging transform");
        return;
    }
    const void* wf = op.wf >= 0 ? c.at(op.wf) : nullptr;
    const bool want = call.stat_groups > 0 && call.stat_groups == op.res_groups;
    long long* sp = want ? stat_acc : nullptr;
    const int sC = want ? sr->C : op.g.co, sc0 = want ? sr->c0 : 0;
    const float s1 = want ? sr->s1 : BN_FS1, s2 = want ? sr->s2 : BN_FS2;
    int rc = 0;
    switch (kern) {
        case ConvKernel::DMA:
        case ConvKernel::HALO:
            rc = kern == ConvKernel::DMA ? launch_conv_dma(op.g, op.plan, op.dma, in, wf, bias, out, c.s, epi)
                                         : launch_conv_halo(op.g, op.plan, op.halo, in, wf, bias, out, c.s, epi);
            if (epi_fused && epi) *epi_fused = 1;
            break;
        case ConvKernel::GEMM:
            rc = launch_conv_gemm(op.g, op.plan, op.gemm, in, wf, bias, out, op.res_groups, sp, sC, c.s, sc0, s1, s2, epi);
            if (stat_chunks && want) *stat_chunks = 1;
            if (epi_fused && epi) *epi_fused = 1;
            break;
        case ConvKernel::SMALL:
            if (bs) {
                rc = launch_conv_small(op.g, in, wf, bias, out, nchw, bs->groups, nullptr, op.g.co, c.s, nullptr, bs);
            } else {
                const int groups = conv_small_groups(call);
                long long* ssp = (call.stat_groups > 0 && call.bn_form && call.stat_groups == groups) ? stat_acc : nullptr;
                rc = launch_conv_small(op.g, in, wf, bias, out, nchw, groups, ssp, op.g.co, c.s, xf);
                if (stat_chunks && ssp) *stat_chunks = 1;
            }
            break;
        case ConvKernel::TILE:
            rc = launch_conv_tile(op.g, op.plan, op.tile, in, wf, bias, out, op.res_groups, sp, sC, c.s, sc0, s1, s2);
            if (stat_chunks && want) *stat_chunks = 1;
            break;
        case ConvKernel::RES:
            if (bs) {
                rc = launch_conv_res(op.g, op.plan, op.res, in, wf, bias, out, op.res_groups, nullptr, op.g.co, c.s, 0, BN_BS, BN_BS, nullptr, bs);
            } else {
                rc = launch_conv_res(op.g, op.plan, op.res, in, wf, bias, out, op.res_groups, sp, sC, c.s, sc0, s1, s2, xf);
                if (stat_chunks && want) *stat_chunks = 1;
            }
            break;
        case ConvKernel::MFMA:
            rc = launch_conv_mfma(op.g, op.plan, in, wf, bias, out, nchw, c.s);
            break;
        case ConvKernel::REF: {
            const PackSpec& ps = op.dgrad ? cv.dgrad : cv.fwd;
            const float* w = c.at<float>(op.dgrad ? cv.wpk_dgrad : cv.wpk_fwd) + (int64_t)op.tap0 * ps.kpad * ps.wld;
            launch_conv_ref(c.e.dt, op.g, in, w, ps.kpad, ps.wld, bias, out, nchw, c.s);
            break;
        }
    }
    if (rc != 0)
        set_error(bs ? std::string("fused BatchNorm-backward sums: the data-gradient launch of ") + cv.name + " does not fit " + kname
                     : std::string("internal: ") + kname + " rejected the " + (op.dgrad ? "data-gradient" : "forward") + " launch of " +
                           cv.name + " it was chosen for");
}

static bool exec_conv_x4(const Ctx& c, const ConvOp ops[4], const void* in, const float* bias, void* out) {
    if (!mfma_on(c.e)) return false;
    stcd_conv_geom g[4]; ConvMfmaPlan p[4]; const void* wf[4];
    double fl = 0.0, by = 0.0;
    for (int k = 0; k < 4; ++k) {
        if (!ops[k].plan.ok || ops[k].wf < 0) return false;
        g[k] = ops[k].g; p[k] = ops[k].plan; wf[k] = c.at(ops[k].wf);
        double f1, b1;
        conv_work(c.e, ops[k].g, ops[k].kreal, ops[k].nreal, &f1, &b1);
        fl += f1; by += b1;
    }
    if (!conv_mfma_x4_ok(g, p)) return false;
    char kname[64];
    snprintf(kname, sizeof(kname), "k_conv_mfma_x4<%d>", p[0].NT);
    ProfScope prof(c, PC_CONV, fl, by, kname);
    if (launch_conv_mfma_x4(g, p, in, wf, bias, out, c.s) != 0) set_error(std::string("internal: ") + kname + " rejected the launch it was chosen for");
    return true;
}

static void wgroup_member_ready(const Ctx& c, const WgradOp& op);
static void exec_wgrad(const Ctx& c, const WgradOp& op, const void* in, const void* dout) {
    const ConvW& cv = c.e.convs[op.conv];
    PackSpec sub = cv.fwd;
    sub.ntaps = op.g.ntaps;
    for (int t = 0; t < op.g.ntaps; ++t) {
        sub.ky[t] = op.own_taps ? op.oky[t] : cv.fwd.ky[op.tap0 + t];
        sub.kx[t] = op.own_taps ? op.okx[t] : cv.fwd.kx[op.tap0 + t];
    }
    double fl, by;
    conv_work(c.e, op.g, op.kreal, op.nreal, &fl, &by);
    if (mfma_on(c.e) && op.plan.ok && op.grouped) {
        if (c.e.wg_early) wgroup_member_ready(c, op);
        return;
    }
    if (mfma_on(c.e) && op.plan.ok) {
        int rc;
        {
            char kname[64];
            snprintf(kname, sizeof(kname), "k_wgrad_mfma<%d, %d>", op.plan.WCI, op.plan.NTW);
            ProfScope prof(c, PC_WGRAD, fl, by, kname);
            rc = launch_wgrad_mfma(op.g, op.plan, in, dout, c.at<float>(op.slab), sub.kpad, sub.wld, c.s);
        }
        if (rc == 0) return;
    }
    if (op.own_taps) { set_error("internal: no reference fallback for a launch with its own tap table"); return; }
    double* dwe = c.at<double>(cv.dwe) + (int64_t)op.tap0 * sub.kpad * sub.wld;
    if (mfma_on(c.e))
        (void)hipMemsetAsync(dwe, 0, (size_t)sub.ntaps * sub.kpad * sub.wld * 8, c.s);
    {
        ProfScope prof(c, PC_WGRAD, fl, by, "k_wgrad_ref");
        launch_wgrad_ref_f64(c.e.dt, op.g, in, dout, dwe, sub.kpad, sub.wld, c.s);
    }
    launch_unpack_dw(sub, dwe, c.grads + cv.w_off, c.s);
}

static int pack_all_weights(const Ctx& c, bool with_dgrad) {
    stcd_engine& e = c.e;
    if (e.jobs_uploaded_ws != (const void*)c.ws) {
        for (int k = 0; k < 2; ++k) {
            if (!e.jobs[k].empty())
                STCD_HIP(hipMemcpyAsync(c.at(e.jobs_off[k]), e.jobs[k].data(), e.jobs[k].size() * sizeof(PackJob),
                                        hipMemcpyHostToDevice, c.s));
            if (!e.rjobs[k].empty())
                STCD_HIP(hipMemcpyAsync(c.at(e.rjobs_off[k]), e.rjobs[k].data(), e.rjobs[k].size() * sizeof(ReduceJob),
                                        hipMemcpyHostToDevice, c.s));
            for (WgradGroup& G : e.wgroups[k])
                STCD_HIP(hipMemcpyAsync(c.at(G.table_off), G.jobs.data(), G.jobs.size() * sizeof(WgradJob), hipMemcpyHostToDevice, c.s));
        }
        if (!e.bias_jobs.empty())
            STCD_HIP(hipMemcpyAsync(c.at(e.bias_jobs_off), e.bias_jobs.data(), e.bias_jobs.size() * sizeof(BiasJob), hipMemcpyHostToDevice, c.s));
        e.jobs_uploaded_ws = c.ws;
    }
    const int k = with_dgrad ? 1 : 0;
    if (k == 0 && e.weights_tag != 0 && e.weights_tag == e.packed_tag && e.packed_ws == (const void*)c.ws && e.packed_params == (const void*)c.params)
        return 0;
    ProfScope prof(c, PC_PACK, 0.0, 0.0);
    launch_pack_jobs(c.at<PackJob>(e.jobs_off[k]), (int)e.jobs[k].size(), e.jobs_total[k], c.params, c.ws, c.s);
    e.packed_tag = k == 0 ? e.weights_tag : 0; e.packed_ws = c.ws; e.packed_params = c.params; e.packed_level = k;
    return 0;
}

static void launch_wgroup(const Ctx& c, WgradGroup& G) {
    {
        char kname[64];
        if (G.dma) snprintf(kname, sizeof(kname), "k_wgrad_dma");
        else if (G.gemm) snprintf(kname, sizeof(kname), "k_wgrad_gemm<%d>", G.gemm);
        else snprintf(kname, sizeof(kname), "k_wgrad_group<%d, %d, %s>", G.WCI, G.NTW, G.t9 ? "true" : "false");
        ProfScope prof(c, PC_WGRAD, G.flops, G.bytes, kname);
        G.launched = true;
        if (G.dma) {
            launch_wgrad_dma_group(c.at<WgradJob>(G.table_off), (int)G.jobs.size(), G.total_blocks, c.ws, c.s);
            return;
        }
// ... 50 lines not shown
static void cbrd_forward(const Ctx& c, const Cbrd& L, float* bn_running, bool training) {
    stcd_engine& e = c.e;
    const ConvW& cv = e.convs[L.conv];
    const BnP& bn = e.bns[L.bn];
    const int C = cv.cout;
    int fused_chunks = 0;
    StatReq sr; sr.acc = training ? c.at<long long>(L.facc) : nullptr; sr.groups = L.groups; sr.C = C;
    XfSrc xf;
    if (L.xsrc) xf = xf_source(c, *L.xsrc, bn_running, training);
    exec_conv(c, L.fwd, c.at(L.in.off), c.params + cv.b_off, c.at(L.Y.off), false, &sr, &fused_chunks, nullptr, nullptr, L.xsrc ? &xf : nullptr);
    const int64_t ppg = (int64_t)L.npg * L.H * L.W;
    const double act_bytes = (double)L.N * L.H * L.W * C * (double)dsize(e.dt);
    float* stat = c.at<float>(L.stat);
    if (training) {
        if (!fused_chunks) {
            ProfScope ps(c, PC_BN_STATS, 0.0, act_bytes);
            launch_bn_stats(e.dt, c.at(L.Y.off), L.Y.ld, C, L.groups, ppg, c.at<long long>(L.facc), c.s);
        }
    }
    if (L.virt) return;
    BnActArgs a;
    a.Y = c.at(L.Y.off); a.ldy = L.Y.ld;
    a.A = skip_recomputed(e, L) ? nullptr : c.at(L.A.off); a.lda = L.A.ld; a.a_group_off = L.A.goff;
    a.P = L.pool ? c.at(L.P.off) : nullptr; a.ldp = L.P.ld;
    a.stat = stat;
    a.mask = (training && e.drop_p > 0.f && L.drop >= 0) ? c.at<float>(e.masks) + e.drops[L.drop].off : nullptr;
    a.C = C; a.groups = L.groups; a.npg = L.npg; a.H = L.H; a.W = L.W; a.relu = 1;
    a.facc = training ? c.at<long long>(L.facc) : nullptr;
    a.gamma = c.params + bn.g_off; a.beta = c.params + bn.b_off;
    a.running_mean = bn_running + bn.run_off; a.running_var = bn_running + bn.run_off + C;
    if (L.fuse_dst.off >= 0 && e.use_act_fuse && L.groups == 2) {
        ProfScope ps(c, PC_BN_ACT, 0.0, act_bytes * (a.A ? 2.75 : 1.75), "k_bn_act_pair");
        launch_bn_act_pair(e.dt, a, c.at(L.fuse_dst.off), L.fuse_dst.ld, e.arch == STCD_ARCH_DIFF ? 0 : 1, c.s);
        return;
    }
    ProfScope ps(c, PC_BN_ACT, 0.0, act_bytes * (L.pool ? 2.25 : 2.0));
    launch_bn_act(e.dt, a, c.s);
}

static BwdSum bwd_sum_of(const Ctx& c, const Cbrd& P) {
    stcd_engine& e = c.e;
    BwdSum b;
    b.Y = c.at(P.Y.off); b.ldy = P.Y.ld; b.stat = c.at<float>(P.stat);
    b.mask = (e.drop_p > 0.f && P.drop >= 0) ? c.at<float>(e.masks) + e.drops[P.drop].off : nullptr;
    b.acc = c.at<long long>(P.bacc); b.groups = P.groups;
    return b;
}

static void cbrd_backward(const Ctx& c, const Cbrd& L, int skip_chunks = 0) {
    stcd_engine& e = c.e;
    const ConvW& cv = e.convs[L.conv];
    const BnP& bn = e.bns[L.bn];
    const int C = cv.cout;
    const int64_t HW = (int64_t)L.H * L.W, ppg = (int64_t)L.npg * HW;
    const float* stat = c.at<float>(L.stat);
    const float* mask = (e.drop_p > 0.f && L.drop >= 0) ? c.at<float>(e.masks) + e.drops[L.drop].off : nullptr;
    long long* bacc = c.at<long long>(L.bacc);
    const double act_bytes = (double)L.N * HW * C * (double)dsize(e.dt);
    (void)ppg;
    if (!skip_chunks && !L.bwd_sums_fused) {
        ProfScope ps(c, PC_BN_BWD_REDUCE, 0.0, 2.0 * act_bytes);
        launch_bn_bwd_reduce(e.dt, c.at(L.dA.off), L.dA.ld, L.dA.goff, c.at(L.Y.off), L.Y.ld, stat, mask, C, L.groups, L.npg, HW, 1,
                             bacc, c.s);
    }
    {
        ProfScope ps(c, PC_BN_BWD_APPLY, 0.0, 3.0 * act_bytes);
        launch_bn_bwd_apply(e.dt, c.at(L.dA.off), L.dA.ld, L.dA.goff, c.at(L.dY.off), L.dY.ld, c.at(L.Y.off), L.Y.ld, stat, bacc,
                            c.grads + bn.g_off, c.grads + bn.b_off, mask, C, L.groups, L.npg, HW, 1, c.s);
    }
    exec_wgrad(c, L.wg, c.at(L.in.off), c.at(L.dY.off));
    if (L.has_dIn) {
        StatReq sr;
        if (L.dgr_sum_acc >= 0) { sr.acc = c.at<long long>(L.dgr_sum_acc); sr.groups = 1; sr.c0 = L.dgr_sum_c0; sr.C = L.dgr_sum_C; sr.s1 = sr.s2 = BN_BS; }
        BwdSum bs;
        if (L.dgr_bwd) bs = bwd_sum_of(c, *L.dgr_bwd);
        exec_conv(c, L.dgr, c.at(L.dY.off), nullptr, c.at(L.dIn.off), false, L.dgr_sum_acc >= 0 ? &sr : nullptr, nullptr, nullptr, nullptr, nullptr,
                  L.dgr_bwd ? &bs : nullptr);
    }
}

static void upconv_forward(const Ctx& c, const UpConv& U) {
    stcd_engine& e = c.e;
    const ConvW& cv = e.convs[U.conv];
    if (!exec_conv_x4(c, U.fwd, c.at(U.in.off), c.params + cv.b_off, c.at(U.out.off)))
        for (int ph = 0; ph < 4; ++ph) exec_conv(c, U.fwd[ph], c.at(U.in.off), c.params + cv.b_off, c.at(U.out.off), false);
    launch_rep_pad(e.dt, c.at(U.out.off), U.out.ld, U.N, U.Ho, U.Wo, 2 * U.h, 2 * U.w, U.C, c.s);
}

static void upconv_backward(const Ctx& c, const UpConv& U) {
    stcd_engine& e = c.e;
    const ConvW& cv = e.convs[U.conv];
    launch_rep_pad_bwd(e.dt, c.at(U.dOut.off), U.dOut.ld, U.N, U.Ho, U.Wo, 2 * U.h, 2 * U.w, U.C, c.s);
    if (U.bias_fused && mfma_on(e)) {
    } else if (2 * U.h == U.Ho && 2 * U.w == U.Wo) {
        launch_bias_grad(e.dt, c.at(U.dOut.off), U.dOut.ld, (int64_t)U.N * U.Ho * U.Wo, U.C, c.grads + cv.b_off, c.s,
                         e.dt == BF16 ? c.at<long long>(U.bias_acc) : nullptr);
    } else {
        const int64_t T = (int64_t)dsize(e.dt);
        for (int n = 0; n < U.N; ++n)
            for (int y = 0; y < 2 * U.h; ++y)
                launch_bias_grad(e.dt, c.at<char>(U.dOut.off) + ((int64_t)(n * U.Ho + y) * U.Wo) * U.dOut.ld * T, U.dOut.ld,
                                 2 * U.w, U.C, c.grads + cv.b_off, c.s, e.dt == BF16 ? c.at<long long>(U.bias_acc) : nullptr);
    }
    for (int ph = 0; ph < 4; ++ph) exec_wgrad(c, U.wg[ph], c.at(U.in.off), c.at(U.dOut.off));
    exec_conv(c, U.dgr, c.at(U.dOut.off), nullptr, c.at(U.dIn.off), false);
}

static void xconc_forward(const Ctx& c, const XConc& X, const Cbrd& skip, float* bn_running, bool training) {
    stcd_engine& e = c.e;
    const BnP& bn = e.bns[X.bn1];
    const int C = X.C, B = X.res.N, h = X.res.H, w = X.res.W;
    {
        ProfScope ps(c, PC_POOL_FUSE, 0.0, 3.0 * B * h * w * C * (double)dsize(e.dt), "k_pairdw_fwd");
        launch_pairdw_fwd(e.dt, c.at(skip.A.off), skip.A.ld, skip.A.goff, c.at(X.G.off), X.G.ld, c.params + X.w_off, c.params + X.b_off, B, h, w, C, c.s);
    }
    if (training) launch_bn_stats(e.dt, c.at(X.G.off), X.G.ld, C, 1, (int64_t)B * h * w, c.at<long long>(X.facc1), c.s);
    BnActArgs a;
    a.Y = c.at(X.G.off); a.ldy = X.G.ld;
    a.A = c.at(X.R.off); a.lda = X.R.ld; a.a_group_off = 0;
    a.P = nullptr; a.ldp = 0;
    a.stat = c.at<float>(X.stat1);
    a.mask = nullptr;
    a.C = C; a.groups = 1; a.npg = B; a.H = h; a.W = w; a.relu = 1;
    a.facc = training ? c.at<long long>(X.facc1) : nullptr;
    a.gamma = c.params + bn.g_off; a.beta = c.params + bn.b_off;
    a.running_mean = bn_running + bn.run_off; a.running_var = bn_running + bn.run_off + C;
    launch_bn_act(e.dt, a, c.s);
    cbrd_forward(c, X.res, bn_running, training);
}
static void xconc_backward(const Ctx& c, const XConc& X, const Cbrd& skip) {
    stcd_engine& e = c.e;
    const BnP& bn = e.bns[X.bn1];
    const int C = X.C, B = X.res.N, h = X.res.H, w = X.res.W;
    const int64_t HW = (int64_t)h * w;
    cbrd_backward(c, X.res);
    launch_bn_bwd_reduce(e.dt, c.at(X.dR.off), X.dR.ld, 0, c.at(X.G.off), X.G.ld, c.at<float>(X.stat1), nullptr, C, 1, B, HW, 1,
                         c.at<long long>(X.bacc1), c.s);
    launch_bn_bwd_apply(e.dt, c.at(X.dR.off), X.dR.ld, 0, c.at(X.dG.off), X.dG.ld, c.at(X.G.off), X.G.ld, c.at<float>(X.stat1),
                        c.at<long long>(X.bacc1), c.grads + bn.g_off, c.grads + bn.b_off, nullptr, C, 1, B, HW, 1, c.s);
    ProfScope ps(c, PC_POOL_FUSE, 0.0, 6.0 * B * h * w * C * (double)dsize(e.dt), "k_pairdw_bwd");
    launch_pairdw_bwd_data(e.dt, c.at(X.dG.off), X.dG.ld, c.at(skip.dA.off), skip.dA.ld, skip.dA.goff, c.params + X.w_off, B, h, w, C, c.s);
    launch_pairdw_bwd_filter(e.dt, c.at(skip.A.off), skip.A.ld, skip.A.goff, c.at(X.dG.off), X.dG.ld, c.grads + X.w_off, c.at<float>(X.part),
                             B, h, w, C, c.s);
}

static int forward_fcsiam(stcd_engine& e, const float* x1, const float* x2, const float* params, float* bn_running,
                          const float* masks, uint64_t seed, int training, float* logits, void* workspace, hipStream_t s) {
    Ctx c{e, (char*)workspace, params, nullptr, s};
    const int B = e.B, dt = e.dt;
    const int64_t T = (int64_t)dsize(dt);
    if (training && e.drop_p > 0.f) {
        if (masks) STCD_HIP(hipMemcpyAsync(c.at(e.masks), masks, e.drop_floats * 4, hipMemcpyDeviceToDevice, s));
        else launch_dropout_gen(c.at<float>(e.masks), e.drop_floats, seed, e.drop_p, s);
    } else if (training && e.fc_virt_layers > 0) {
        launch_dropout_gen(c.at<float>(e.masks), e.drop_floats, seed, 0.f, s);
    }
    if (pack_all_weights(c, training != 0)) return 1;
    if (training) STCD_HIP(hipMemsetAsync(c.at(e.zero_begin), 0, e.zero_end - e.zero_begin, s));
    launch_in_pack(dt, x1, x2, c.at(e.X0.off), B, e.in_ch, e.H, e.W, s, e.arch == STCD_ARCH_FCEF ? 0 : 2);
    for (auto& L : e.enc) cbrd_forward(c, L, bn_running, training != 0);
    size_t di = 0;
    for (int k = 0; k < 4; ++k) {
        const UpConv& U = e.ups[k];
        const int s_ = U.level, C = ENC_C[s_];
        upconv_forward(c, U);
        const Cbrd& skip = e.enc[SKIP_IDX[s_]];
        if (fc_cross(e)) xconc_forward(c, e.xc[s_], skip, bn_running, training != 0);
// ... 1288 lines not shown
                        c.at(e.gFuseTmp.off), 16, (int64_t)B * HW * 16, B, HW, 16, s);
    }
    for (int k = (int)e.g_fwd.size() - 1; k >= 0; --k) {
        const GStep& st = e.g_fwd[k];
        if (st.kind == GS_LAYER) glayer_backward(c, e.g_layers[st.layer]);
        else if (st.kind == GS_UPSAMPLE)
            launch_upsample2_bwd(dt, c.at(st.ddst.off), st.ddst.ld, c.at(st.dsrc.off), st.dsrc.ld, st.N, st.h, st.w, st.C, s);
        else if (st.kind == GS_ABSDIFF) {
            const int64_t hw = (int64_t)st.h * st.w;
            launch_fuse_bwd(dt, 0, c.at(st.src.off), st.src.ld, (int64_t)st.N * hw * st.src.ld,
                            c.at<char>(st.dsrc.off) + (int64_t)2 * st.N * hw * st.dsrc.ld * T, st.dsrc.ld,
                            c.at(st.ddst.off), st.ddst.ld, (int64_t)st.N * hw * st.ddst.ld, st.N, hw, st.C, s);
        }
        else if (st.kind == GS_TOKENDEC) {
            auto& b = e.bit;
            const int n = st.h * st.w;
            const double rows = (double)st.N * n;
            {
                ProfScope ps(c, PC_POOL_FUSE, 3.0 * 12288.0 * b.L * rows, rows * 32 * ((b.L + 2.0) * (double)T + 8.0 * (b.L - 1)), "k_bit_dec_bwd");
                if (launch_bit_dec_bwd(dt, c.at(st.src.off), c.at(b.xs), c.at(st.ddst.off), c.at<float>(b.dG), c.at(st.dsrc.off), c.at<float>(b.AP),
                                       params + b.dec_off, c.at<float>(b.dec_part), n, st.N, b.L, b.dh, s)) return 1;
            }
            ProfScope ps(c, PC_POOL_FUSE, 2.0 * b.L * st.N * 6.0 * 8 * b.dh * 32 * 4, 4.0 * (double)bit_dec_part_floats(n, st.N, b.L), "k_bit_sum_parts|k_bit_dec_unfold|k_bit_dec_mfinish");
            launch_bit_dec_finish(c.at<float>(b.dec_part), c.at<float>(b.dAP), c.at<float>(b.tok_out), params + b.dec_off, grads + b.dec_off,
                                  c.at<float>(b.dmh), c.at<float>(b.dm), c.at<float>(b.dtok_out), n, st.N, b.L, b.dh, s);
        } else if (st.kind == GS_TOKENENC) {
            auto& b = e.bit;
            ProfScope ps(c, PC_POOL_FUSE, 6.0 * B * 8 * (4.0 * 512 * 32 + 2.0 * 32 * 64), 4.0 * (double)bit_enc_part_floats(B, 64) * 2, "k_bit_enc<true>");
            launch_bit_enc_bwd(c.at<float>(b.tok_in), params + b.pos_off, params + b.enc_off, c.at<float>(b.dtok_out), c.at<float>(b.dtok_in),
                               c.at<float>(b.enc_part), grads + b.enc_off, grads + b.pos_off, B, 64, s);
        } else if (st.kind == GS_TOKENIZE) {
            auto& b = e.bit;
            ProfScope ps(c, PC_POOL_FUSE, 48.0 * 32 * st.N * st.h * st.w, 4.0 * st.N * st.h * st.w * 32 * (double)T, "k_bit_tok_bwd");
            launch_bit_tok_bwd(dt, c.at(st.src.off), params + b.wa_off, c.at<float>(b.stat), c.at<float>(b.dtok_in), c.at(b.dec_din.off),
                               c.at(st.dsrc.off), c.at<float>(b.tok_part), grads + b.wa_off, st.N, st.h * st.w, s);
        }
        else if (st.kind == GS_BILINEAR) {
            ProfScope ps(c, PC_POOL_FUSE, 0.0, 17.0 * st.N * st.h * st.w * st.C * (double)T, "k_bilinear_bwd");
            launch_bilinear_bwd(dt, c.at(st.ddst.off), st.ddst.ld, c.at(st.dsrc.off), st.dsrc.ld, st.N, st.h, st.w, 4 * st.h, 4 * st.w, st.C, 0, s);
        } else if (st.kind == GS_ABSPAIR) {
            const int64_t hw = (int64_t)st.h * st.w;
            ProfScope ps(c, PC_POOL_FUSE, 0.0, 5.0 * st.N * hw * st.C * (double)T, "k_fuse_bwd");
            launch_fuse_bwd(dt, 0, c.at(st.src.off), st.src.ld, (int64_t)st.N * hw * st.src.ld, c.at(st.ddst.off), st.ddst.ld,
                            c.at(st.dsrc.off), st.dsrc.ld, (int64_t)st.N * hw * st.dsrc.ld, st.N, hw, st.C, s);
        } else if (st.kind == GS_BCONV) {
            { ProfScope ps(c, PC_POOL_FUSE, 0.0, (double)st.N * st.h * st.w * 32 * (double)T, "k_bias_grad");
            launch_bias_grad(dt, c.at(st.ddst.off), st.ddst.ld, (int64_t)st.N * st.h * st.w, 32, grads + e.convs[e.g_pred_conv].b_off, s,
                             dt == BF16 ? c.at<long long>(e.g_pred_bias_acc) : nullptr); }
            exec_wgrad(c, e.g_pred_wg, c.at(st.src.off), c.at(st.ddst.off));
            exec_conv(c, e.g_pred_dgr, c.at(st.ddst.off), nullptr, c.at(st.dsrc.off), false);
        }
        else {
            launch_slice(dt, c.at(st.ddst.off), st.ddst.ld, c.at(e.g_pool_idc.off), e.g_pool_idc.ld, (int64_t)st.N * (st.h / 2) * (st.w / 2), st.C, 1, s);
            launch_maxpool3_bwd(dt, c.at<unsigned char>(e.g_pool_idx), c.at(st.ddst.off), st.ddst.ld, c.at(st.dsrc.off), st.dsrc.ld, st.N, st.h, st.w, st.C, s);
        }
    }
    reduce_stage(c, 0);
    launch_bias_finish(c.at<BiasJob>(e.bias_jobs_off), (int)e.bias_jobs.size(), c.ws, c.grads, s);
    STCD_HIP(hipGetLastError());
    return 0;
}

#include "engine_cf.inl"

}

extern "C" {

const char* stcd_last_error(void) { return stcd::g_err.c_str(); }
int stcd_abi_version(void) { return STCD_ABI_VERSION; }

static void engine_env_switches(stcd_engine* e) {
    e->use_mfma = !env_flag("STCD_FORCE_REF_KERNELS", false);
    e->use_small = !env_flag("STCD_NO_SMALL_KERNEL", false);
    e->use_gemm = !env_flag("STCD_NO_GEMM_KERNEL", false);
    e->use_res = !env_flag("STCD_NO_RES_KERNEL", false);
    e->use_halo = env_flag("STCD_HALO_KERNEL", false);
    e->use_tile = !env_flag("STCD_NO_TILE_KERNEL", false);
    e->use_wgroup = !env_flag("STCD_NO_WGRAD_GROUPS", false);
    e->use_act_fuse = !env_flag("STCD_NO_ACT_FUSE", false);
    e->use_skip_fused = !env_flag("STCD_NO_SKIP_FUSED", false);
    e->use_skip_recompute = !env_flag("STCD_NO_SKIP_RECOMPUTE", false);
    e->use_bwdsum = !env_flag("STCD_NO_BWDSUM_FUSE", false);
    e->use_bwdsum_res = env_flag("STCD_BWDSUM_RES", false);
    e->use_virt = env_int("STCD_VIRT_ACT", e->use_virt) != 0;
    e->wg_side_on = env_int("STCD_WGRAD_SIDE", e->wg_side_on) != 0;
}

int stcd_cf_default_config(stcd_cf_config* cfg) {
    STCD_CHECK(cfg != nullptr, "cfg is null");
    static const int E[4] = {64, 128, 320, 512}, DP[4] = {3, 3, 4, 3}, HD[4] = {1, 2, 4, 8}, SR[4] = {8, 4, 2, 1};
    memset(cfg, 0, sizeof(*cfg));
    cfg->in_ch = 3; cfg->out_ch = 2;
    for (int i = 0; i < 4; ++i) { cfg->embed_dims[i] = E[i]; cfg->depths[i] = DP[i]; cfg->num_heads[i] = HD[i]; cfg->sr_ratios[i] = SR[i]; }
    cfg->mlp_ratio = 4; cfg->embedding_dim = 256; cfg->patch1 = 7; cfg->patch = 7;
    cfg->drop_rate = 0.1f; cfg->attn_drop = 0.1f; cfg->drop_path_rate = 0.1f; cfg->diff_drop = 0.6f;
    return 0;
}

int stcd_create_changeformer(const stcd_cf_config* cfg, int dtype, stcd_engine** out) {
    STCD_CHECK(out != nullptr && cfg != nullptr, "null argument");
    STCD_CHECK(cfg->in_ch >= 1 && cfg->in_ch <= 8, "in_ch must be in [1,8]");
    STCD_CHECK(cfg->out_ch >= 1 && cfg->out_ch <= 8, "out_ch must be in [1,8]");
    STCD_CHECK(dtype == STCD_DTYPE_F32 || dtype == STCD_DTYPE_BF16, "unknown dtype");
    STCD_CHECK(cfg->mlp_ratio >= 1 && cfg->embedding_dim >= 8 && cfg->embedding_dim % 8 == 0, "embedding_dim must be a positive multiple of 8");
    STCD_CHECK((cfg->embedding_dim & (cfg->embedding_dim - 1)) == 0, "embedding_dim must be a power of two (BatchNorm kernels)");
    STCD_CHECK((cfg->patch1 & 1) && (cfg->patch & 1) && cfg->patch1 >= 3 && cfg->patch >= 3, "patch sizes must be odd and >= 3");
    for (int i = 0; i < 4; ++i) {
        STCD_CHECK(cfg->embed_dims[i] >= 8 && cfg->embed_dims[i] % 8 == 0 && cfg->embed_dims[i] <= 1024, "embed_dims must be multiples of 8, <= 1024");
        STCD_CHECK(cfg->depths[i] >= 1 && cfg->num_heads[i] >= 1 && cfg->sr_ratios[i] >= 1, "depths, num_heads and sr_ratios must be >= 1");
        STCD_CHECK(cfg->embed_dims[i] % cfg->num_heads[i] == 0, "embed_dims must be divisible by num_heads");
    }
    for (float p : {cfg->drop_rate, cfg->attn_drop, cfg->drop_path_rate, cfg->diff_drop}) STCD_CHECK(p >= 0.f && p < 1.f, "drop rates must be in [0,1)");
    std::unique_ptr<stcd_engine> e(new stcd_engine());
    e->arch = STCD_ARCH_CHANGEFORMER; e->in_ch = cfg->in_ch; e->label = cfg->out_ch; e->dt = dtype;
    engine_env_switches(e.get());
    e->cf = std::make_shared<CfPlan>();
    CfPlan& P = *e->cf;
    for (int i = 0; i < 4; ++i) { P.E[i] = cfg->embed_dims[i]; P.depths[i] = cfg->depths[i]; P.heads[i] = cfg->num_heads[i]; P.srs[i] = cfg->sr_ratios[i]; }
    P.mlp_ratio = cfg->mlp_ratio; P.D = cfg->embedding_dim; P.patch1 = cfg->patch1; P.patch = cfg->patch;
    P.drop = cfg->drop_rate; P.attn_drop = cfg->attn_drop; P.drop_path = cfg->drop_path_rate; P.diff_drop = cfg->diff_drop;
    build_cf_tables(*e);
    *out = e.release();
    return 0;
}

int stcd_cf_num_sites(const stcd_engine* e) { return e && e->cf && e->configured ? (int)e->cf->sites.size() : 0; }
int stcd_cf_site_get(const stcd_engine* e, int i, stcd_cf_site* out) {
    STCD_CHECK(e && e->cf && e->configured && out && i >= 0 && i < (int)e->cf->sites.size(), "bad argument");
    memset(out, 0, sizeof(*out));
    const CfPlan::Site& s = e->cf->sites[i];
    snprintf(out->name, sizeof(out->name), "%s", s.name.c_str());
    out->ndim = s.nd;
    for (int k = 0; k < s.nd; ++k) out->dims[k] = s.dims[k];
    out->p = s.p;
    return 0;
}
uint32_t stcd_cf_site_seed(uint64_t seed, int site) { return cf_site_seed(seed, site); }
int stcd_cf_set_aux_backward(stcd_engine* e, int on) {
    STCD_CHECK(e && e->cf, "not a ChangeFormer engine");
    if (e->cf->aux_bwd != (on != 0)) e->configured = false;
    e->cf->aux_bwd = on != 0;
    return 0;
}
int stcd_set_wgrad_side(stcd_engine* e, int on) {
    STCD_CHECK(e, "null engine");
    if ((e->wg_side_on != 0) != (on != 0)) e->configured = false;
    e->wg_side_on = on != 0;
    return 0;
}
int stcd_cf_set_drop_rates(stcd_engine* e, float drop_rate, float attn_drop, float diff_drop) {
    STCD_CHECK(e && e->cf, "not a ChangeFormer engine");
    for (float p : {drop_rate, attn_drop, diff_drop}) STCD_CHECK(p >= 0.f && p < 1.f, "drop rates must be in [0,1)");
    e->cf->drop = drop_rate; e->cf->attn_drop = attn_drop; e->cf->diff_drop = diff_drop;
    e->configured = false;
    return 0;
}
int64_t stcd_output_floats(const stcd_engine* e) {
    if (!e || !e->configured) return 0;
    if (e->cf) return e->cf->out_floats;
    const int maps = (is_segcd(e->arch) && !is_unetseg(e->arch) && !is_bres(e->arch)) ? 3 : sn_out_maps(e->arch);
    return (int64_t)maps * e->B * e->label * e->H * e->W;
}
int stcd_cf_output_info(const stcd_engine* e, int i, int64_t* offset, int* height, int* width) {
    STCD_CHECK(e && e->cf && e->configured && offset && height && width && i >= 0 && i < 5, "bad argument");
    if (i < 4) { *offset = e->cf->df[i].out_off; *height = e->cf->df[i].h; *width = e->cf->df[i].w; }
// ... 370 lines not shown
    if (wd.ok) wgrad_dma_set_split(wd, *g, op_dma_splits(*g, wd), g->ci, g->co);
    return std::max<int64_t>(p.wf_elems * 2, std::max(std::max(std::max(w.slab_floats, ww.slab_floats), wg.ok ? wg.slab_floats : 0), wd.ok ? wd.slab_floats : 0) * 4) + 1024;
}
int stcd_op_conv(int dtype, int impl, const stcd_conv_geom* g, const void* in, const float* w, const float* bias,
                 void* out, void* scratch, int64_t scratch_bytes, void* hip_stream) {
    if (check_geom(g)) return 1;
    STCD_CHECK(in && w && out, "null pointer argument");
    if (impl == 1 || impl == 2 || impl == 3 || impl == 6 || impl == 8) {
        STCD_CHECK(dtype == STCD_DTYPE_BF16, "the MFMA implementation is bf16 only");
        ConvMfmaPlan p = conv_mfma_plan(*g);
        STCD_CHECK(p.ok, "geometry not supported by the MFMA kernel");
        STCD_CHECK(scratch && scratch_bytes >= p.wf_elems * 2, "scratch too small for the fragment-order filter");
        launch_pack_frag(*g, p, w, g->ci, g->co, scratch, (hipStream_t)hip_stream);
        if (impl == 3) {
            const ConvHaloPlan hp = conv_halo_plan(*g, p);
            STCD_CHECK(hp.ok, "geometry not supported by the resident-halo kernel (3x3 stride 1, Ci % 64 == 0, Co % 128 == 0)");
            STCD_CHECK(launch_conv_halo(*g, p, hp, in, scratch, bias, out, (hipStream_t)hip_stream) == 0, "launch failed");
            STCD_HIP(hipGetLastError());
            return 0;
        }
        if (impl == 6) {
            const ConvDmaPlan dp = conv_dma_plan(*g, p);
            STCD_CHECK(dp.ok, "geometry not supported by the LDS-DMA kernel (Ci % 64 == 0, Co % 256 == 0, (Ci / 64) * taps even and >= 4)");
            STCD_CHECK(launch_conv_dma(*g, p, dp, in, scratch, bias, out, (hipStream_t)hip_stream) == 0, "launch failed");
            STCD_HIP(hipGetLastError());
            return 0;
        }
        if (impl == 8) {
            const ConvTilePlan tp = conv_tile_plan(*g, p, 1);
            STCD_CHECK(tp.ok, "geometry not supported by the LDS-DMA tile kernel (3x3 stride 1 over the full map, Ci % 64 == 0, Co % 16 == 0)");
            STCD_CHECK(launch_conv_tile(*g, p, tp, in, scratch, bias, out, 1, nullptr, g->co, (hipStream_t)hip_stream) == 0, "launch failed");
            STCD_HIP(hipGetLastError());
            return 0;
        }
        if (impl == 1) {
            stcd_engine sw;
            sw.dt = BF16;
            engine_env_switches(&sw);
            ConvOp op;
            op.g = *g;
            plan_conv(sw, op, 1, false);
            op.wf = 0;
            ConvCall call;
            call.allowed = ~(conv_kernel_bit(ConvKernel::DMA) | conv_kernel_bit(ConvKernel::HALO) | conv_kernel_bit(ConvKernel::TILE));
            int rc = 1;
            switch (conv_kernel(true, sw.use_small, op, call)) {
                case ConvKernel::SMALL: rc = launch_conv_small(*g, in, scratch, bias, out, false, 1, nullptr, g->co, (hipStream_t)hip_stream); break;
                case ConvKernel::RES: rc = launch_conv_res(*g, p, op.res, in, scratch, bias, out, 1, nullptr, g->co, (hipStream_t)hip_stream); break;
                case ConvKernel::GEMM: rc = launch_conv_gemm(*g, p, op.gemm, in, scratch, bias, out, 1, nullptr, g->co, (hipStream_t)hip_stream); break;
                case ConvKernel::MFMA: rc = launch_conv_mfma(*g, p, in, scratch, bias, out, false, (hipStream_t)hip_stream); break;
                default: break;
            }
            STCD_CHECK(rc == 0, "the chosen kernel rejected the geometry");
            STCD_HIP(hipGetLastError());
            return 0;
        }
        STCD_CHECK(launch_conv_mfma(*g, p, in, scratch, bias, out, false, (hipStream_t)hip_stream) == 0, "LDS budget exceeded");
        STCD_HIP(hipGetLastError());
        return 0;
    }
    STCD_CHECK(impl == 0, "impl must be 0 (reference FMA), 1 (MFMA, auto-selected kernel), 2 (generic MFMA kernel), 3 (resident-halo kernel), 6 (LDS-DMA kernel) or 8 (LDS-DMA tile kernel)");
    launch_conv_ref(dtype, *g, in, w, g->ci, g->co, bias, out, false, (hipStream_t)hip_stream);
    STCD_HIP(hipGetLastError());
    return 0;
}
int stcd_op_conv_fused(const stcd_conv_geom* g, stcd_conv_fused* f, const void* in, const float* w, const float* bias, void* out,
                       void* scratch, int64_t scratch_bytes, void* hip_stream) {
    if (check_geom(g)) return 1;
    STCD_CHECK(f != nullptr, "the fused-features request is null");
    f->blocks = f->tiles_per_group = f->blocks_per_group = f->tile_m = 0;
    f->bn_rep = BN_REP;
    STCD_CHECK(in && w && out, "null pointer argument");
    STCD_CHECK(f->kernel >= STCD_CONV_SMALL && f->kernel <= STCD_CONV_DMA, "kernel must be one of STCD_CONV_*");
    const int groups = f->groups;
    STCD_CHECK(groups >= 1 && g->n % groups == 0, "groups must be >= 1 and divide n (whole images per BatchNorm group)");
    const bool sums = f->sum_acc != nullptr, epi_on = f->use_epi != 0, bwd = f->bw_acc != nullptr;
    const bool k_small = f->kernel == STCD_CONV_SMALL, k_res = f->kernel == STCD_CONV_RES, k_tile = f->kernel == STCD_CONV_TILE;
    const bool k_gemm = f->kernel == STCD_CONV_GEMM, k_halo = f->kernel == STCD_CONV_HALO, k_dma = f->kernel == STCD_CONV_DMA;
    STCD_CHECK(!sums || k_small || k_res || k_tile || k_gemm, "fused sums: k_conv_small, k_conv_res, k_conv_tile and k_conv_gemm only");
    STCD_CHECK(!epi_on || k_gemm || k_halo || k_dma, "ConvEpi: k_conv_gemm, k_conv_halo and k_conv_dma only");
    STCD_CHECK(!bwd || k_small || k_res, "BatchNorm-backward sums: k_conv_small and k_conv_res only");
    STCD_CHECK(!(k_halo || k_dma) || groups == 1, "k_conv_halo and k_conv_dma know one group");
    STCD_CHECK(!(bwd && sums), "a data gradient with BatchNorm-backward sums carries no forward sums");
    if (sums) {
        STCD_CHECK(f->sum_c0 >= 0 && f->sum_c >= 1 && f->sum_c0 + f->sum_c <= g->co, "the summed channel slice lies outside the output channels");
        STCD_CHECK(f->sum_scale1 > 0.f && f->sum_scale2 > 0.f, "the sum scales must be positive");
        STCD_CHECK(!k_small || (f->sum_c0 == 0 && f->sum_c == g->co && f->sum_scale1 == BN_FS1 && f->sum_scale2 == BN_FS2),
                   "k_conv_small sums all its channels at the BatchNorm scales (2^26, 2^18)");
    }
    ConvEpi epi;
    if (epi_on) {
        STCD_CHECK(!f->gate || (f->ldg >= g->co && f->ldg % 8 == 0), "gate: the pixel stride must be a multiple of 8 and >= co");
        STCD_CHECK(!f->res || (f->ldr >= g->co && f->ldr % 8 == 0), "res: the pixel stride must be a multiple of 8 and >= co");
        STCD_CHECK(f->res || (f->alpha == 1.f && f->beta == 1.f), "alpha / beta combine the output with a residual: without one they must be 1");
        epi.relu = f->relu ? 1 : 0;
        epi.gate = f->gate; epi.ldg = f->ldg; epi.res = f->res; epi.ldr = f->ldr; epi.alpha = f->alpha; epi.beta = f->beta;
    }
    BwdSum bs;
    if (bwd) {
        STCD_CHECK(f->bw_y && f->bw_stat, "BatchNorm-backward sums need the layer's conv output and its statistics");
        STCD_CHECK(f->bw_ldy >= g->co && f->bw_ldy % 4 == 0, "bw_y: the pixel stride must be a multiple of 4 and >= co");
        bs.Y = f->bw_y; bs.ldy = f->bw_ldy; bs.stat = f->bw_stat; bs.mask = f->bw_mask; bs.acc = (long long*)f->bw_acc; bs.groups = groups;
    }
    const ConvMfmaPlan p = conv_mfma_plan(*g);
    STCD_CHECK(p.ok, "geometry not supported by the MFMA kernels");
    STCD_CHECK(scratch && scratch_bytes >= p.wf_elems * 2, "scratch too small for the fragment-order filter");
    hipStream_t s = (hipStream_t)hip_stream;
    long long* const acc = (long long*)f->sum_acc;
    const int sC = sums ? f->sum_c : g->co, sc0 = sums ? f->sum_c0 : 0;
    const float s1 = sums ? f->sum_scale1 : BN_FS1, s2 = sums ? f->sum_scale2 : BN_FS2;
    const int64_t tiles16 = (int64_t)g->n * ((g->hm + 15) / 16) * ((g->wm + 15) / 16);
    ConvResPlan rp; ConvTilePlan tp; ConvGemmPlan gp; ConvHaloPlan hp; ConvDmaPlan dp;
    if (k_small) {
        STCD_CHECK(conv_small_ok(*g, p) && conv_small_call_ok(*g, groups, nullptr), "geometry not supported by k_conv_small (one n-tile, <= 5 k-steps)");
        STCD_CHECK(!bwd || conv_small_bwdsum_ok(*g), "k_conv_small forms BatchNorm-backward sums for 16 channels out, whole 8 x 16 tiles, 3 or 5 k-steps");
        f->blocks = conv_small_blocks(*g, groups);
        f->blocks_per_group = f->blocks / groups;
        f->tiles_per_group = (int)((int64_t)g->n * ((g->hm + 7) / 8) * ((g->wm + 15) / 16) / groups);
    } else if (k_res) {
        rp = conv_res_plan(*g, p, groups);
        STCD_CHECK(rp.ok, "geometry not supported by k_conv_res (3x3 stride 1, Ci % 32 == 0)");
        STCD_CHECK(!bwd || conv_res_bwdsum_ok(*g, rp), "this k_conv_res plan forms no BatchNorm-backward sums (slices of one or two n-tiles, double halo)");
        f->blocks = rp.blocks; f->blocks_per_group = rp.P; f->tiles_per_group = (int)(tiles16 / groups);
    } else if (k_tile) {
        tp = conv_tile_plan(*g, p, groups);
        STCD_CHECK(tp.ok, "geometry not supported by k_conv_tile (3x3 stride 1 over the full map, Ci % 64 == 0, Co % 16 == 0)");
        f->blocks = tp.blocks; f->blocks_per_group = tp.P; f->tiles_per_group = (int)(tiles16 / groups);
    } else if (k_gemm) {
        gp = conv_gemm_plan(*g, p, groups);
        STCD_CHECK(gp.ok, "geometry not supported by k_conv_gemm (Ci % 64 == 0, Co % 64 == 0)");
        f->blocks = gp.blocks; f->blocks_per_group = gp.tiles_m; f->tiles_per_group = gp.tiles_m; f->tile_m = 32 * gp.W;
    } else if (k_halo) {
        hp = conv_halo_plan(*g, p);
        STCD_CHECK(hp.ok, "geometry not supported by k_conv_halo (3x3 stride 1, Ci % 128 == 0, Co % 128 == 0)");
        f->blocks = hp.blocks; f->blocks_per_group = hp.P; f->tiles_per_group = (int)tiles16;
    } else {
        dp = conv_dma_plan(*g, p);
        STCD_CHECK(dp.ok, "geometry not supported by k_conv_dma (Ci % 64 == 0, Co % 256 == 0, (Ci / 64) * taps even and >= 4)");
        f->blocks = dp.blocks; f->blocks_per_group = std::min(dp.blocks, dp.tiles_m); f->tiles_per_group = dp.tiles_m;
    }
    launch_pack_frag(*g, p, w, g->ci, g->co, scratch, s);
    int rc = 1;
    if (k_small) rc = launch_conv_small(*g, in, scratch, bias, out, false, groups, acc, sC, s, nullptr, bwd ? &bs : nullptr);
    else if (k_res) rc = launch_conv_res(*g, p, rp, in, scratch, bias, out, groups, acc, sC, s, sc0, s1, s2, nullptr, bwd ? &bs : nullptr);
    else if (k_tile) rc = launch_conv_tile(*g, p, tp, in, scratch, bias, out, groups, acc, sC, s, sc0, s1, s2);
    else if (k_gemm) rc = launch_conv_gemm(*g, p, gp, in, scratch, bias, out, groups, acc, sC, s, sc0, s1, s2, epi_on ? &epi : nullptr);
    else if (k_halo) rc = launch_conv_halo(*g, p, hp, in, scratch, bias, out, s, epi_on ? &epi : nullptr);
    else rc = launch_conv_dma(*g, p, dp, in, scratch, bias, out, s, epi_on ? &epi : nullptr);
    STCD_CHECK(rc == 0, "the named kernel's launcher rejected the combination");
    STCD_HIP(hipGetLastError());
    return 0;
}
int stcd_op_wgrad(int dtype, int impl, const stcd_conv_geom* g, const void* in, const void* dout, float* dw, void* scratch,
                  int64_t scratch_bytes, void* hip_stream) {
    if (check_geom(g)) return 1;
    STCD_CHECK(in && dout && dw, "null pointer argument");
    if (impl == 1 || impl == 4 || impl == 5) {
        STCD_CHECK(dtype == STCD_DTYPE_BF16, "the MFMA implementation is bf16 only");
        WgradMfmaPlan p = wgrad_mfma_plan(*g, g->ci, g->co, impl >= 4, impl == 5 ? 1 : 0);
        STCD_CHECK(p.ok, "geometry not supported by the MFMA kernel");
        STCD_CHECK(scratch && scratch_bytes >= p.slab_floats * 4, "scratch too small for the partial slabs");
        STCD_CHECK(launch_wgrad_mfma(*g, p, in, dout, (float*)scratch, g->ci, g->co, (hipStream_t)hip_stream) == 0, "LDS budget exceeded");
        launch_reduce_dw((const float*)scratch, p.gx, *g, g->ci, g->co, g->ci, g->co, nullptr, dw, (hipStream_t)hip_stream);
        STCD_HIP(hipGetLastError());
        return 0;
    }
    if (impl == 7) {
        STCD_CHECK(dtype == STCD_DTYPE_BF16, "the MFMA implementation is bf16 only");
        WgradMfmaPlan p = wgrad_dma_plan(*g, g->ci, g->co);
        STCD_CHECK(p.ok, "geometry not supported by the LDS-DMA weight-gradient kernel (stride 1, full map >= 64 wide, Ci % 256 == 0, Co % 256 == 0)");
        wgrad_dma_set_split(p, *g, op_dma_splits(*g, p), g->ci, g->co);
        const int64_t table = (p.slab_floats * 4 + 255) & ~(int64_t)255;
        STCD_CHECK(scratch && scratch_bytes >= table + (int64_t)sizeof(WgradJob), "scratch too small for the partial slabs + job table");
        WgradJob j = wgrad_dma_make_job(*g, p, (int64_t)(intptr_t)in, (int64_t)(intptr_t)dout, (int64_t)(intptr_t)scratch, g->ci, g->co);
        STCD_HIP(hipMemcpyAsync((char*)scratch + table, &j, sizeof(j), hipMemcpyHostToDevice, (hipStream_t)hip_stream));
        STCD_HIP(hipStreamSynchronize((hipStream_t)hip_stream));
        launch_wgrad_dma_group((const WgradJob*)((char*)scratch + table), 1, p.gx * p.gy * p.gz, nullptr, (hipStream_t)hip_stream);
        launch_reduce_dw((const float*)scratch, p.gx, *g, g->ci, g->co, g->ci, g->co, nullptr, dw, (hipStream_t)hip_stream);
        STCD_HIP(hipGetLastError());
        return 0;
    }
    if (impl == 3) {
        STCD_CHECK(dtype == STCD_DTYPE_BF16, "the MFMA implementation is bf16 only");
        WgradMfmaPlan p = wgrad_gemm_plan(*g, g->ci, g->co);
        STCD_CHECK(p.ok, "geometry not supported by the GEMM weight-gradient kernel (one tap, Ci >= 64, Co >= 64)");
        const int64_t table = (p.slab_floats * 4 + 255) & ~(int64_t)255;
        STCD_CHECK(scratch && scratch_bytes >= table + (int64_t)sizeof(WgradJob), "scratch too small for the partial slabs + job table");
        WgradJob j = wgrad_gemm_make_job(*g, p, (int64_t)(intptr_t)in, (int64_t)(intptr_t)dout, (int64_t)(intptr_t)scratch, g->ci, g->co);
        STCD_HIP(hipMemcpyAsync((char*)scratch + table, &j, sizeof(j), hipMemcpyHostToDevice, (hipStream_t)hip_stream));
        STCD_HIP(hipStreamSynchronize((hipStream_t)hip_stream));
        launch_wgrad_gemm_group(p.gemm, (const WgradJob*)((char*)scratch + table), 1, p.gx * p.gy * p.gz, nullptr, (hipStream_t)hip_stream);
        launch_reduce_dw((const float*)scratch, p.gx, *g, g->ci, g->co, g->ci, g->co, nullptr, dw, (hipStream_t)hip_stream);
        STCD_HIP(hipGetLastError());
        return 0;
    }
    STCD_CHECK(impl == 0, "impl must be 0 (reference FMA), 1 / 4 (MFMA tile kernel, 4: wide tile allowed), 3 (MFMA position-GEMM kernel) or 7 (LDS-DMA kernel)");
    STCD_HIP(hipMemsetAsync(dw, 0, (size_t)g->ntaps * g->ci * g->co * 4, (hipStream_t)hip_stream));
    launch_wgrad_ref(dtype, *g, in, dout, dw, g->ci, g->co, (hipStream_t)hip_stream);
    STCD_HIP(hipGetLastError());
    return 0;
}

}
```

stcd_amd/csrc/kernels_conv_mfma.hip:

```cpp
#include "common.h"

namespace stcd {

typedef __attribute__((ext_vector_type(8))) __bf16 bf16x8;
typedef __attribute__((ext_vector_type(4))) float f32x4;
typedef __attribute__((ext_vector_type(4))) unsigned u32x4;

struct ConvMfmaArgs {
    stcd_conv_geom g;
    const bf16* in;
    const bf16* wf;
    const float* bias;
    void* out;
    int out_nchw;
    int CiB, nchunks, KS;
    int modeB;
    int NTtot;
    int dymin, dxmin, HH, HWp, swmask;
    int tiles_x, tiles_y;
    int halo_bytes, wbuf_bytes;
    int tap[9];
};

static inline void fill_taps(const stcd_conv_geom& g, int* tap) {
// ... 858 lines not shown
    (void)hipGetLastError();
    return std::max(1, per_cu) * cus;
}

int launch_wgrad_group(int WCI, int NTW, bool t9, const WgradJob* jobs_dev, int njobs, int total_blocks, int lds_bytes,
                       const char* base, hipStream_t s, bool xf) {
    if (njobs <= 0 || total_blocks <= 0) return 0;
    if (lds_bytes > 128 * 1024) return 1;
    if (lds_bytes > 64 * 1024) {
        static bool attr_set = false;
        if (!attr_set) {
            (void)hipFuncSetAttribute((const void*)k_wgrad_group<4, 2, true>, hipFuncAttributeMaxDynamicSharedMemorySize, 160 * 1024);
            (void)hipFuncSetAttribute((const void*)k_wgrad_group<4, 2, false>, hipFuncAttributeMaxDynamicSharedMemorySize, 160 * 1024);
            (void)hipFuncSetAttribute((const void*)k_wgrad_group<4, 4, true>, hipFuncAttributeMaxDynamicSharedMemorySize, 160 * 1024);
            (void)hipFuncSetAttribute((const void*)k_wgrad_group<4, 4, false>, hipFuncAttributeMaxDynamicSharedMemorySize, 160 * 1024);
            attr_set = true;
        }
    }
    if (xf) {
#define WG_GROUP_XF(W_, N_, T_) k_wgrad_group<W_, N_, T_, true><<<(unsigned)total_blocks, 256, (size_t)lds_bytes, s>>>(jobs_dev, njobs, base)
        if (WCI == 4 || NTW == 4) return 1;
        WG_DISPATCH(WCI, NTW, t9, WG_GROUP_XF);
#undef WG_GROUP_XF
        return 0;
    }
#define WG_GROUP(W_, N_, T_) k_wgrad_group<W_, N_, T_><<<(unsigned)total_blocks, 256, (size_t)lds_bytes, s>>>(jobs_dev, njobs, base)
    WG_DISPATCH(WCI, NTW, t9, WG_GROUP);
#undef WG_GROUP
    return 0;
}

int launch_wgrad_mfma(const stcd_conv_geom& g, const WgradMfmaPlan& p, const void* in, const void* dout, float* slab,
                      int kpad, int wld, hipStream_t s) {
    if (!p.ok) return 1;
    const WgradJob a = wgrad_make_job(g, p, (int64_t)(intptr_t)in, (int64_t)(intptr_t)dout, (int64_t)(intptr_t)slab, kpad, wld);
    if (a.lds_bytes > 128 * 1024) return 1;
    if (a.lds_bytes > 64 * 1024) {
        static bool attr_set = false;
        if (!attr_set) {
            (void)hipFuncSetAttribute((const void*)k_wgrad_mfma<4, 2, true>, hipFuncAttributeMaxDynamicSharedMemorySize, 160 * 1024);
            (void)hipFuncSetAttribute((const void*)k_wgrad_mfma<4, 2, false>, hipFuncAttributeMaxDynamicSharedMemorySize, 160 * 1024);
            (void)hipFuncSetAttribute((const void*)k_wgrad_mfma<4, 4, true>, hipFuncAttributeMaxDynamicSharedMemorySize, 160 * 1024);
            (void)hipFuncSetAttribute((const void*)k_wgrad_mfma<4, 4, false>, hipFuncAttributeMaxDynamicSharedMemorySize, 160 * 1024);
            attr_set = true;
        }
    }
    dim3 grid((unsigned)p.gx, (unsigned)p.gy, (unsigned)p.gz);
    const bool t9 = g.ntaps == 9;
#define WG_ONE(W_, N_, T_) k_wgrad_mfma<W_, N_, T_><<<grid, 256, (size_t)a.lds_bytes, s>>>(a)
    WG_DISPATCH(p.WCI, p.NTW, t9, WG_ONE);
#undef WG_ONE
    return 0;
}

void launch_reduce_dw(const float* slab, int gx, const stcd_conv_geom& g, int K, int N, int kpad, int wld,
                      const PackSpec* ps, float* out, hipStream_t s) {
    const int total = g.ntaps * K * N;
    PackSpec dummy{};
    if (gx >= 128 && total <= 16384)
        k_reduce_dw<64><<<(total + 3) / 4, 256, 0, s>>>(slab, gx, (int64_t)g.ntaps * kpad * wld, g.ntaps, K, N, kpad, wld,
                                                          ps ? *ps : dummy, ps ? 1 : 0, out);
    else
        k_reduce_dw<16><<<(total + 15) / 16, 256, 0, s>>>(slab, gx, (int64_t)g.ntaps * kpad * wld, g.ntaps, K, N, kpad, wld,
                                                            ps ? *ps : dummy, ps ? 1 : 0, out);
}

struct ConvSmallArgs {
    stcd_conv_geom g;
    const bf16* in;
    const bf16* wf;
    const float* bias;
    void* out;
    int out_nchw;
    int KS, NTtot, Ci;
    int dymin, dxmin, HH, HWp;
    int tiles_x, tiles_y, ntiles, groups;
    int halo_bytes;
    long long* stat_acc;
    int cpad;
    int tap[9];
    XfSrc xf;
    const bf16* bw_Y; int bw_ldy; const float* bw_stat; const float* bw_mask;
    float s1_scale, s2_scale;
};

template <int NT, int KSMAX, bool XF = false, int FAST = 0, bool BWD = false>
__global__ void __launch_bounds__(256, 2)
k_conv_small(const ConvSmallArgs a) {
    constexpr bool EXACT = FAST >= 1, FULL = FAST == 2;
    static_assert(!BWD || (FULL && NT == 1 && !XF), "BWD: full-tile single-n-tile data gradients only");
    extern __shared__ __attribute__((aligned(16))) char smem[];
    const int tid = threadIdx.x, lane = tid & 63, wid = tid >> 6;
    const int q = lane >> 4, r = lane & 15;
    const int is = a.g.in_stride, HWp = a.HWp, Ci = a.Ci, nch8 = Ci >> 3;
    const int KS = a.KS;
    bf16* const halo0 = reinterpret_cast<bf16*>(smem);
    const int halo_elems = a.halo_bytes >> 1;

    bf16x8 wreg[KSMAX][NT];
    int aoff[KSMAX];
#pragma unroll
    for (int ks = 0; ks < KSMAX; ++ks) {
        const int kk = EXACT ? ks : min(ks, KS - 1);
#pragma unroll
        for (int t2 = 0; t2 < NT; ++t2)
            wreg[ks][t2] = *reinterpret_cast<const bf16x8*>(a.wf + ((int64_t)(kk * a.NTtot + t2) * 64 + lane) * 8);
        const int kl = kk * 32 + 8 * q;
        int t = kl / Ci, c = kl - t * Ci;
        if (t >= a.g.ntaps) { t = 0; c = 0; }
        int tw = 0;
#pragma unroll
        for (int tt = 0; tt < 9; ++tt) tw = t == tt ? a.tap[tt] : tw;
        aoff[ks] = ((TAP_DY(tw) - a.dymin) * HWp + (TAP_DX(tw) - a.dxmin)) * Ci + c;
    }

    const int bpg = gridDim.x / a.groups, grp = blockIdx.x / bpg, bl = blockIdx.x - grp * bpg;
    const int tpg = a.ntiles / a.groups;
    float s1[NT][4], s2[NT][4];
#pragma unroll
    for (int t2 = 0; t2 < NT; ++t2)
#pragma unroll
        for (int j = 0; j < 4; ++j) s1[t2][j] = s2[t2][j] = 0.f;

    const int npieces = a.HH * HWp * nch8;
    constexpr int MAXP = 3;
    int poff[MAXP], phy[MAXP], phx[MAXP];
#pragma unroll
    for (int p = 0; p < MAXP; ++p) {
        const int i = tid + p * 256;
        const int ch = i % nch8, pix = i / nch8;
        phx[p] = pix % HWp + a.dxmin;
        phy[p] = (i < npieces) ? pix / HWp + a.dymin : (1 << 28);
        poff[p] = (phy[p] * a.g.wi + phx[p]) * a.g.ldi + ch * 8;
    }
    float bv[NT][4];
#pragma unroll
    for (int t2 = 0; t2 < NT; ++t2)
#pragma unroll
        for (int j = 0; j < 4; ++j) {
            const int cb = t2 * 16 + 4 * q + j;
            bv[t2][j] = (a.bias && cb < a.g.co) ? a.bias[cb] : 0.f;
        }
    float bw_mean[4], bw_inv[4], bw_sc[4], bw_sh[4];
    if constexpr (BWD) {
        const float* st = a.bw_stat + (int64_t)grp * 4 * a.g.co + 4 * q;
#pragma unroll
        for (int j = 0; j < 4; ++j) { bw_mean[j] = st[j]; bw_inv[j] = st[a.g.co + j]; bw_sc[j] = st[2 * a.g.co + j]; bw_sh[j] = st[3 * a.g.co + j]; }
    }
    const int tiles_img = a.tiles_x * a.tiles_y;
    const int dn = bpg / tiles_img, drem = bpg - dn * tiles_img, dty = drem / a.tiles_x, dtx = drem - dty * a.tiles_x;
    int tile = grp * tpg + bl;
    const int tile_end = (grp + 1) * tpg;
    int tn = tile / tiles_img, trem = tile - tn * tiles_img, tty = trem / a.tiles_x, ttx = trem - tty * a.tiles_x;
    auto advance = [&](int& n_, int& y_, int& x_) {
        x_ += dtx; if (x_ >= a.tiles_x) { x_ -= a.tiles_x; ++y_; }
        y_ += dty; if (y_ >= a.tiles_y) { y_ -= a.tiles_y; ++n_; }
        n_ += dn;
    };
    uint4 pre[MAXP];
    unsigned xf_ok = 0;
    float4 xf_m0 = make_float4(1.f, 1.f, 1.f, 1.f), xf_m1 = xf_m0;
    float xf_sc[8], xf_sh[8];
    float xf_fs[8], xf_fh[8];
    const int xch = (tid % nch8) * 8;
    auto fetch = [&](int n_, int y_, int x_) {
        const int gy0 = y_ * 8 * is, gx0 = x_ * 16 * is;
        const bf16* org = a.in + (((int64_t)n_ * a.g.hi + gy0) * a.g.wi + gx0) * a.g.ldi;
        if constexpr (XF) xf_ok = 0;
#pragma unroll
        for (int p = 0; p < MAXP; ++p) {
            const unsigned gy = (unsigned)(gy0 + phy[p]), gx = (unsigned)(gx0 + phx[p]);
            pre[p] = make_uint4(0, 0, 0, 0);
            if (gy < (unsigned)a.g.hi && gx < (unsigned)a.g.wi) {
                pre[p] = *reinterpret_cast<const uint4*>(org + poff[p]);
                if constexpr (XF) xf_ok |= 1u << p;
            }
        }
        if constexpr (XF) {
            if (a.xf.mask) {
                const float4* mp = reinterpret_cast<const float4*>(a.xf.mask + (int64_t)n_ * a.xf.C + xch);
                xf_m0 = mp[0]; xf_m1 = mp[1];
            }
        }
    };
    auto stash = [&](int buf_) {
        if constexpr (XF) {
            xf_fold8(xf_sc, xf_sh, xf_m0, xf_m1, xf_fs, xf_fh);
#pragma unroll
            for (int p = 0; p < MAXP; ++p) {
                const int i = tid + p * 256;
                if (i < npieces) *reinterpret_cast<uint4*>(halo0 + buf_ * halo_elems + i * 8) = xf_act8(pre[p], xf_fs, xf_fh, 0u - ((xf_ok >> p) & 1u));
            }
        } else {
#pragma unroll
            for (int p = 0; p < MAXP; ++p) {
                const int i = tid + p * 256;
                if (i < npieces) *reinterpret_cast<uint4*>(halo0 + buf_ * halo_elems + i * 8) = pre[p];
            }
        }
    };

    int buf = 0;
    if (tile < tile_end) fetch(tn, tty, ttx);
    if constexpr (XF) {
        float* tab = reinterpret_cast<float*>(smem + 2 * a.halo_bytes);
        bn_fwd_table(tab, a.xf.facc, a.xf.gamma, a.xf.beta, a.xf.rmean, a.xf.rvar, a.xf.stat, a.xf.C, a.xf.groups, a.xf.ppg,
                     a.xf.momentum, a.xf.eps, a.xf.publish != 0 && blockIdx.x == 0);
        __syncthreads();
#pragma unroll
        for (int j = 0; j < 8; ++j) { xf_sc[j] = tab[(grp * 2 + 0) * a.xf.C + xch + j]; xf_sh[j] = tab[(grp * 2 + 1) * a.xf.C + xch + j]; }
    }
    if (tile < tile_end) stash(0);
    __syncthreads();
    const int base0 = ((wid * 2) * is * HWp + r * is) * Ci, rowstep = is * HWp * Ci;
    for (; tile < tile_end; tile += bpg, buf ^= 1) {
        int nn = tn, ny = tty, nx = ttx;
        advance(nn, ny, nx);
        const bool have_next = tile + bpg < tile_end;
        if (have_next) fetch(nn, ny, nx);
        uint2 bw_y[2];
        float4 bw_mk = make_float4(1.f, 1.f, 1.f, 1.f);
        if constexpr (BWD) {
            const bf16* yrow = a.bw_Y + (((int64_t)tn * a.g.ho + tty * 8 + wid * 2) * a.g.wo + ttx * 16 + r) * a.bw_ldy + 4 * q;
            bw_y[0] = *reinterpret_cast<const uint2*>(yrow);
            bw_y[1] = *reinterpret_cast<const uint2*>(yrow + (int64_t)a.g.wo * a.bw_ldy);
            if (a.bw_mask) bw_mk = *reinterpret_cast<const float4*>(a.bw_mask + (int64_t)tn * a.g.co + 4 * q);
        }
        f32x4 acc[2][NT];
#pragma unroll
        for (int m = 0; m < 2; ++m)
#pragma unroll
            for (int t2 = 0; t2 < NT; ++t2) acc[m][t2] = f32x4{0.f, 0.f, 0.f, 0.f};
        const bf16* hb = halo0 + buf * halo_elems;
#pragma unroll
        for (int ks = 0; ks < KSMAX; ++ks) {
            if (EXACT || ks < KS) {
                const bf16x8 a0 = *reinterpret_cast<const bf16x8*>(hb + base0 + aoff[ks]);
                const bf16x8 a1 = *reinterpret_cast<const bf16x8*>(hb + base0 + rowstep + aoff[ks]);
#pragma unroll
                for (int t2 = 0; t2 < NT; ++t2) {
                    acc[0][t2] = __builtin_amdgcn_mfma_f32_16x16x32_bf16(wreg[ks][t2], a0, acc[0][t2], 0, 0, 0);
                    acc[1][t2] = __builtin_amdgcn_mfma_f32_16x16x32_bf16(wreg[ks][t2], a1, acc[1][t2], 0, 0, 0);
                }
            }
        }
        if (have_next) stash(buf ^ 1);
        const int mx = ttx * 16 + r;
#pragma unroll
        for (int m = 0; m < 2; ++m) {
            const int my = tty * 8 + wid * 2 + m;
            if constexpr (FULL) {
                const int oy = my * a.g.out_stride + a.g.oy0, ox = mx * a.g.out_stride + a.g.ox0;
                bf16* orow = reinterpret_cast<bf16*>(a.out) + (((int64_t)tn * a.g.ho + oy) * a.g.wo + ox) * a.g.ldo + 4 * q;
#pragma unroll
                for (int t2 = 0; t2 < NT; ++t2) {
                    uint2 pk;
                    pk.x = pack_bf16x2(acc[m][t2][0] + bv[t2][0], acc[m][t2][1] + bv[t2][1]);
                    pk.y = pack_bf16x2(acc[m][t2][2] + bv[t2][2], acc[m][t2][3] + bv[t2][3]);
                    *reinterpret_cast<uint2*>(orow + t2 * 16) = pk;
                    const float rv[4] = {__uint_as_float(pk.x << 16), __uint_as_float(pk.x & 0xffff0000u),
                                         __uint_as_float(pk.y << 16), __uint_as_float(pk.y & 0xffff0000u)};
                    if constexpr (BWD) {
                        const float y[4] = {__uint_as_float(bw_y[m].x << 16), __uint_as_float(bw_y[m].x & 0xffff0000u),
                                            __uint_as_float(bw_y[m].y << 16), __uint_as_float(bw_y[m].y & 0xffff0000u)};
                        const float mk[4] = {bw_mk.x, bw_mk.y, bw_mk.z, bw_mk.w};
#pragma unroll
                        for (int j = 0; j < 4; ++j) {
                            const float z = y[j] * bw_sc[j] + bw_sh[j];
                            float dz = rv[j] * mk[j];
                            if (!(z > 0.f)) dz = 0.f;
                            s1[t2][j] += dz;
                            s2[t2][j] += dz * (y[j] - bw_mean[j]) * bw_inv[j];
                        }
                    } else {
#pragma unroll
                        for (int j = 0; j < 4; ++j) { s1[t2][j] += rv[j]; s2[t2][j] += rv[j] * rv[j]; }
                    }
                }
                continue;
            }
            if (my >= a.g.hm || mx >= a.g.wm) continue;
            const int oy = my * a.g.out_stride + a.g.oy0, ox = mx * a.g.out_stride + a.g.ox0;
            if (a.out_nchw) {
                float* o = reinterpret_cast<float*>(a.out) + ((int64_t)tn * a.g.co * a.g.ho + oy) * a.g.wo + ox;
#pragma unroll
                for (int t2 = 0; t2 < NT; ++t2)
#pragma unroll
                    for (int j = 0; j < 4; ++j) {
                        const int cb = t2 * 16 + 4 * q + j;
                        if (cb < a.g.co) o[(int64_t)cb * a.g.ho * a.g.wo] = acc[m][t2][j] + bv[t2][j];
                    }
            } else {
                bf16* orow = reinterpret_cast<bf16*>(a.out) + (((int64_t)tn * a.g.ho + oy) * a.g.wo + ox) * a.g.ldo + 4 * q;
#pragma unroll
                for (int t2 = 0; t2 < NT; ++t2) {
                    const int cb = t2 * 16 + 4 * q;
                    if (cb >= a.g.co) continue;
                    float v[4];
#pragma unroll
                    for (int j = 0; j < 4; ++j) v[j] = acc[m][t2][j] + bv[t2][j];
                    bf16* o = orow + t2 * 16;
                    if (cb + 3 < a.g.co) {
                        uint2 pk;
                        pk.x = pack_bf16x2(v[0], v[1]);
                        pk.y = pack_bf16x2(v[2], v[3]);
                        *reinterpret_cast<uint2*>(o) = pk;
                    } else {
#pragma unroll
                        for (int j = 0; j < 4; ++j)
                            if (cb + j < a.g.co) o[j] = (bf16)v[j];
                    }
#pragma unroll
                    for (int j = 0; j < 4; ++j) {
                        const float rv = round_as<bf16>(v[j]);
                        s1[t2][j] += rv;
                        s2[t2][j] += rv * rv;
                    }
                }
            }
        }
        tn = nn; tty = ny; ttx = nx;
        barrier_lds();
    }

    if (a.stat_acc) {
        float* red = reinterpret_cast<float*>(smem);
#pragma unroll
        for (int t2 = 0; t2 < NT; ++t2)
#pragma unroll
            for (int j = 0; j < 4; ++j) {
                float x = s1[t2][j], y = s2[t2][j];
#pragma unroll
                for (int o = 1; o < 16; o <<= 1) { x += __shfl_xor(x, o, 64); y += __shfl_xor(y, o, 64); }
                if (r == 0) {
                    red[(((wid * NT + t2) * 4 + q) * 4 + j) * 2] = x;
                    red[(((wid * NT + t2) * 4 + q) * 4 + j) * 2 + 1] = y;
                }
            }
        __syncthreads();
        for (int i = tid; i < NT * 16 * 2; i += 256) {
            const int which = i / (NT * 16), c = i - which * NT * 16;
            const int t2 = c >> 4, qq = (c >> 2) & 3, j = c & 3;
            float acc_ = 0.f;
#pragma unroll
            for (int w = 0; w < 4; ++w) acc_ += red[(((w * NT + t2) * 4 + qq) * 4 + j) * 2 + which];
            if (c < a.cpad) bn_acc_add(a.stat_acc, bl, a.groups, a.cpad, grp, which, c, acc_, which ? a.s2_scale : a.s1_scale);
        }
    }
}

bool conv_small_ok(const stcd_conv_geom& g, const ConvMfmaPlan& p) {
    if (!p.ok || (!p.modeB && p.nchunks != 1)) return false;
    const int K = g.ntaps * g.ci;
    const int ks = (K + 31) / 32;
    const int nt = (g.co + 15) / 16;
    int dymin, dymax, dxmin, dxmax;
    taps_extent(g, &dymin, &dymax, &dxmin, &dxmax);
    const int HH = 7 * g.in_stride + (dymax - dymin) + 1, HWp = 15 * g.in_stride + (dxmax - dxmin) + 1;
    return ks <= 5 && nt <= 1 && g.ci <= 32 && HH * HWp * (g.ci / 8) <= 3 * 256;
}

int conv_small_blocks(const stcd_conv_geom& g, int groups) {
    const int64_t ntiles = (int64_t)g.n * ((g.hm + 7) / 8) * ((g.wm + 15) / 16);
    int64_t per_group = ntiles / groups;
    int64_t bpg = std::min<int64_t>(per_group, 2048 / groups);
    if (bpg < 1) bpg = 1;
    return (int)(bpg * groups);
}

bool conv_small_bwdsum_ok(const stcd_conv_geom& g) {
    const int ks = (g.ntaps * g.ci + 31) / 32;
    return g.co == 16 && g.hm % 8 == 0 && g.wm % 16 == 0 && g.hm == g.ho && g.wm == g.wo && g.out_stride == 1 && g.oy0 == 0 && g.ox0 == 0 &&
           (ks == 3 || ks == 5);
}
bool conv_small_call_ok(const stcd_conv_geom& g, int groups, const XfSrc* xf) {
    if (groups < 1 || g.n % groups != 0) return false;
    return !(xf && xf->on) || (xf->C == g.ci && xf->groups == groups);
}
int launch_conv_small(const stcd_conv_geom& g, const void* in, const void* wf_modeB, const float* bias, void* out,
                      bool out_nchw, int groups, long long* stat_acc, int cpad, hipStream_t s, const XfSrc* xf, const BwdSum* bs) {
    ConvSmallArgs a;
    a.bw_Y = nullptr; a.bw_ldy = 0; a.bw_stat = nullptr; a.bw_mask = nullptr; a.s1_scale = BN_FS1; a.s2_scale = BN_FS2;
    a.g = g;
    a.in = (const bf16*)in; a.wf = (const bf16*)wf_modeB; a.bias = bias; a.out = out; a.out_nchw = out_nchw ? 1 : 0;
    a.Ci = g.ci;
    a.KS = (g.ntaps * g.ci + 31) / 32;
    const int nt = (g.co + 15) / 16;
    a.NTtot = nt;
    int dymax, dxmax;
    taps_extent(g, &a.dymin, &dymax, &a.dxmin, &dxmax);
    a.HH = 7 * g.in_stride + (dymax - a.dymin) + 1;
    a.HWp = 15 * g.in_stride + (dxmax - a.dxmin) + 1;
    a.tiles_x = (g.wm + 15) / 16;
    a.tiles_y = (g.hm + 7) / 8;
    a.ntiles = g.n * a.tiles_x * a.tiles_y;
    a.groups = groups;
    a.halo_bytes = (a.HH * a.HWp * g.ci * 2 + 255) & ~255;
    a.stat_acc = stat_acc;
    a.cpad = cpad;
    fill_taps(g, a.tap);
    if (!conv_small_call_ok(g, groups, xf)) return 1;
    const int blocks = conv_small_blocks(g, groups);
    size_t lds = std::max<size_t>(2 * (size_t)a.halo_bytes, 4 * 2 * 16 * 2 * 4 * 2);
    const bool use_xf = xf && xf->on;
    if (use_xf) {
        a.xf = *xf;
        lds = 2 * (size_t)a.halo_bytes + (size_t)xf->groups * 2 * xf->C * 4;
    }
    if (bs) {
        if (!conv_small_bwdsum_ok(g) || out_nchw || use_xf || nt != 1 || stat_acc || bs->groups != groups || !bs->acc) return 1;
        a.bw_Y = (const bf16*)bs->Y; a.bw_ldy = bs->ldy; a.bw_stat = bs->stat; a.bw_mask = bs->mask;
        a.stat_acc = bs->acc; a.cpad = g.co; a.s1_scale = BN_BS; a.s2_scale = BN_BS;
        if (a.KS == 3) k_conv_small<1, 3, false, 2, true><<<blocks, 256, lds, s>>>(a);
        else k_conv_small<1, 5, false, 2, true><<<blocks, 256, lds, s>>>(a);
        return 0;
    }
    if (nt != 1) return 1;
    const bool full = !out_nchw && g.co == nt * 16 && g.hm % 8 == 0 && g.wm % 16 == 0;
#define LAUNCH_SMALL(N_, K_, F_) do { if (use_xf) k_conv_small<N_, K_, true, F_><<<blocks, 256, lds, s>>>(a); else k_conv_small<N_, K_, false, F_><<<blocks, 256, lds, s>>>(a); } while (0)
#define LAUNCH_SMALL_K(N_, K_) do { if (full) LAUNCH_SMALL(N_, K_, 2); else LAUNCH_SMALL(N_, K_, 1); } while (0)
#define LAUNCH_SMALL_N(N_) do { \
        if (a.KS == 3) LAUNCH_SMALL_K(N_, 3); \
        else if (a.KS == 5) LAUNCH_SMALL_K(N_, 5); \
        else if (a.KS <= 5) LAUNCH_SMALL(N_, 5, 0); \
        else if (a.KS == 9) LAUNCH_SMALL_K(N_, 9); \
        else LAUNCH_SMALL(N_, 9, 0); } while (0)
    LAUNCH_SMALL_N(1);
#undef LAUNCH_SMALL_K
#undef LAUNCH_SMALL_N
#undef LAUNCH_SMALL
    return 0;
}

struct ConvResArgs {
    stcd_conv_geom g;
    const bf16* in;
    const bf16* wf;
    const float* bias;
    bf16* out;
    int NTtot, KSp;
    int nchunks;
    int nslices, P, groups;
    int tiles_x, tiles_y, ntiles;
    int filt_bytes;
    long long* stat_acc;
    int cpad;
    int stat_c0;
    float s1_scale, s2_scale;
    unsigned in_bytes;
    int8_t tix[3][3];
    XfSrc xf;
    const bf16* bw_Y; int bw_ldy; const float* bw_stat; const float* bw_mask;
};

constexpr int RES_HW = 18;

template <int NT, int CW, bool SH = false, bool PIPE = false, bool XF = false, bool BWD = false>
__global__ void __launch_bounds__(256, (CW == 64 && NT == 4) ? 1 : 2)
k_conv_res(const ConvResArgs a) {
    static_assert(!BWD || (NT <= 2 && !SH && !XF), "BWD: one or two n-tiles, double halo, plain input");
    extern __shared__ __attribute__((aligned(16))) char smem[];
    constexpr int KSC = CW / 32, CH8 = CW / 8, LG8 = CW == 64 ? 3 : 2, SW = CH8 - 1;
    constexpr int HALO_BYTES = RES_HW * RES_HW * CW * 2;
    constexpr int NPIECE = RES_HW * RES_HW * CH8, MAXP = (NPIECE + 255) / 256, PIXSTEP = 256 >> LG8;
    const int tid = threadIdx.x, lane = tid & 63, wid = tid >> 6;
    const int q = lane >> 4, r = lane & 15;
    const int P = a.P;
    const int bl = blockIdx.x % P, rest = blockIdx.x / P, slice = rest % a.nslices, grp = rest / a.nslices;
    char* const filt = smem;
    char* const halo0 = smem + a.filt_bytes;
    float* const xf_tab = reinterpret_cast<float*>(smem + a.filt_bytes + (SH ? 1 : 2) * HALO_BYTES);
    const int ntaps = 9;
    const int nsteps = a.nchunks / KSC;

    const int nfrag = a.nchunks * ntaps * NT;
    constexpr int FB = 9;
    auto filt_src = [&](int f) -> int64_t {
        const int ntl = f % NT, ft = f / NT, t = ft % ntaps, c32 = ft / ntaps;
        return ((int64_t)((c32 / a.KSp) * ntaps + t) * a.KSp + (c32 % a.KSp)) * a.NTtot + slice * NT + ntl;
    };
    const int swid = __builtin_amdgcn_readfirstlane(wid);
    uint4 fv[FB];
#pragma unroll
    for (int k = 0; k < FB; ++k) fv[k] = *reinterpret_cast<const uint4*>(a.wf + (filt_src(min(swid + 4 * k, nfrag - 1)) * 64 + lane) * 8);

    const int ch = tid & SW;
    int pyx[MAXP], poff[MAXP], plds[MAXP];
#pragma unroll
    for (int p = 0; p < MAXP; ++p) {
        const int pix = min((tid >> LG8) + p * PIXSTEP, RES_HW * RES_HW - 1);
        const int hx = pix % RES_HW, hy = pix / RES_HW;
        pyx[p] = ((hy - 1) << 16) | ((hx - 1) & 0xffff);
        poff[p] = ((hy * a.g.wi + hx) * a.g.ldi + ch * 8) * 2;
        plds[p] = (pix * CH8 + (ch ^ ((hx >> 1) & SW))) * 16;
    }
    float bv[NT][4];
#pragma unroll
    for (int t2 = 0; t2 < NT; ++t2) {
        const int cb = (slice * NT + t2) * 16 + 4 * q;
        if (a.bias && cb + 3 < a.g.co) {
            const float4 b4 = *reinterpret_cast<const float4*>(a.bias + cb);
            bv[t2][0] = b4.x; bv[t2][1] = b4.y; bv[t2][2] = b4.z; bv[t2][3] = b4.w;
        } else {
#pragma unroll
            for (int j = 0; j < 4; ++j) bv[t2][j] = (a.bias && cb + j < a.g.co) ? a.bias[cb + j] : 0.f;
        }
    }
    float s1[NT][4], s2[NT][4];
#pragma unroll
    for (int t2 = 0; t2 < NT; ++t2)
#pragma unroll
        for (int j = 0; j < 4; ++j) s1[t2][j] = s2[t2][j] = 0.f;

// ... 920 lines not shown
```

Measured before the change: 7889 image-pairs/sec.

## Add small-tile kernels for 16-channel transposed-conv upsampling and stride-2 convs

```diff
diff --git a/include/stcd_hip.h b/include/stcd_hip.h
--- a/include/stcd_hip.h
+++ b/include/stcd_hip.h
@@ -224,9 +224,13 @@
     int32_t bw_ldy;
     int32_t blocks, tiles_per_group, blocks_per_group, bn_rep;
     int32_t tile_m;
+    void* in_sum_acc;
 } stcd_conv_fused;
 int stcd_op_conv_fused(const stcd_conv_geom* g, stcd_conv_fused* f, const void* in, const float* w, const float* bias, void* out,
                        void* scratch, int64_t scratch_bytes, void* hip_stream);
+int stcd_op_upconv(int impl, int n, int h, int w, int c, const void* in, int ldi, const float* wt, const float* bias, void* out,
+                   int ho, int wo, int ldo, void* scratch, int64_t scratch_bytes, void* hip_stream);
+int stcd_op_bias_grad(const void* dy, int ld, int64_t pixels, int c, void* acc, void* hip_stream);
 int stcd_op_wgrad(int dtype, int impl, const stcd_conv_geom* g, const void* in, const void* dout, float* dw,
                   void* scratch, int64_t scratch_bytes, void* hip_stream);
 int64_t stcd_op_scratch_bytes(const stcd_conv_geom* g);
diff --git a/stcd_amd/_lib.py b/stcd_amd/_lib.py
--- a/stcd_amd/_lib.py
+++ b/stcd_amd/_lib.py
@@ -86,7 +86,7 @@
                 ("alpha", C.c_float), ("beta", C.c_float),
                 ("bw_y", C.c_void_p), ("bw_stat", C.c_void_p), ("bw_mask", C.c_void_p), ("bw_acc", C.c_void_p), ("bw_ldy", C.c_int32),
                 ("blocks", C.c_int32), ("tiles_per_group", C.c_int32), ("blocks_per_group", C.c_int32), ("bn_rep", C.c_int32),
-                ("tile_m", C.c_int32)]
+                ("tile_m", C.c_int32), ("in_sum_acc", C.c_void_p)]
 
 
 _vp, _i, _i64, _f, _d = C.c_void_p, C.c_int, C.c_int64, C.c_float, C.c_double
@@ -155,6 +155,8 @@
     "stcd_mask_close": (_i, [_vp, _i, _i, _i, _i, _vp, _vp]),
     "stcd_op_conv": (_i, [_i, _i, C.POINTER(ConvGeom), _vp, _vp, _vp, _vp, _vp, _i64, _vp]),
     "stcd_op_conv_fused": (_i, [C.POINTER(ConvGeom), C.POINTER(ConvFused), _vp, _vp, _vp, _vp, _vp, _i64, _vp]),
+    "stcd_op_upconv": (_i, [_i, _i, _i, _i, _i, _vp, _i, _vp, _vp, _vp, _i, _i, _i, _vp, _i64, _vp]),
+    "stcd_op_bias_grad": (_i, [_vp, _i, _i64, _i, _vp, _vp]),
     "stcd_op_wgrad": (_i, [_i, _i, C.POINTER(ConvGeom), _vp, _vp, _vp, _vp, _i64, _vp]),
     "stcd_op_scratch_bytes": (_i64, [C.POINTER(ConvGeom)]),
     "stcd_op_ew_scratch_bytes": (_i64, [C.POINTER(MapGeom)]),
diff --git a/stcd_amd/csrc/common.h b/stcd_amd/csrc/common.h
--- a/stcd_amd/csrc/common.h
+++ b/stcd_amd/csrc/common.h
@@ -277,10 +277,14 @@
                     const float* bias, void* out, hipStream_t s, const ConvEpi* epi = nullptr);
 
 bool conv_small_ok(const stcd_conv_geom& g, const ConvMfmaPlan& p);
+bool conv_small_s2_ok(const stcd_conv_geom& g, const ConvMfmaPlan& p);
 int conv_small_blocks(const stcd_conv_geom& g, int groups);
 int launch_conv_small(const stcd_conv_geom& g, const void* in, const void* wf_modeB, const float* bias, void* out,
                       bool out_nchw_f32, int groups, long long* stat_acc, int cpad, hipStream_t s, const XfSrc* xf = nullptr,
-                      const BwdSum* bs = nullptr);
+                      const BwdSum* bs = nullptr, long long* in_acc = nullptr);
+bool upconv_small_ok(const stcd_conv_geom g[4], const ConvMfmaPlan p[4]);
+int launch_upconv_small(const stcd_conv_geom g[4], const ConvMfmaPlan p[4], const void* in, const void* const wf[4], const float* bias,
+                        void* out, hipStream_t s);
 bool conv_small_call_ok(const stcd_conv_geom& g, int groups, const XfSrc* xf);
 bool conv_small_bwdsum_ok(const stcd_conv_geom& g);
 struct WgradMfmaPlan {
diff --git a/stcd_amd/csrc/engine.hip b/stcd_amd/csrc/engine.hip
--- a/stcd_amd/csrc/engine.hip
+++ b/stcd_amd/csrc/engine.hip
@@ -44,6 +44,7 @@
     int kreal = 0, nreal = 0;
     ConvMfmaPlan plan; int64_t wf = -1;
     bool small = false;
+    bool small_s2 = false;
     ConvResPlan res; int res_groups = 1;
     ConvGemmPlan gemm;
     ConvDmaPlan dma;
@@ -104,6 +105,7 @@
     TRef in, out, dOut, dIn;
     ConvOp fwd[4], dgr; WgradOp wg[4];
     int64_t bias_acc = -1; bool bias_fused = false;
+    bool fwd_small = false;
 };
 
 enum ProfClass { PC_CONV = 0, PC_WGRAD = 1, PC_BN_STATS = 2, PC_BN_ACT = 3, PC_BN_BWD_REDUCE = 4, PC_BN_BWD_APPLY = 5,
@@ -255,7 +257,7 @@
     int64_t final_bias_acc = -1;
     std::vector<BiasJob> bias_jobs; int64_t bias_jobs_off = -1;
     int64_t masks = -1, dwe_begin = -1, dwe_end = -1, scratch8 = -1;
-    int use_mfma = 1, use_small = 1, use_wgroup = 1, use_res = 1, use_skip_fused = 1, use_act_fuse = 1, use_gemm = 1, use_skip_recompute = 1, use_bwdsum = 1, use_bwdsum_res = 0, use_tile = 1, use_halo = 0;
+    int use_mfma = 1, use_small = 1, use_wgroup = 1, use_res = 1, use_skip_fused = 1, use_act_fuse = 1, use_gemm = 1, use_skip_recompute = 1, use_bwdsum = 1, use_bwdsum_res = 0, use_tile = 1, use_halo = 0, use_upconv_small = 1;
     int wg_side_on = 1;
     static constexpr int WG_SIDE_DIV = 4;
     static constexpr int WGROUP_ROUNDS = 1, WGROUP_MIN_TILES = 8;
@@ -536,9 +538,14 @@
     return wgrad_mfma_plan(g, kpad, wld, is_snunet(e.arch) || (e.cf && g.ntaps == 9));
 }
 
+constexpr int UPCONV_SMALL_MIN_TILES = 512;
+static bool upconv_small_fills(const stcd_conv_geom& g) {
+    return (int64_t)g.n * ((g.hm + 7) / 8) * ((g.wm + 15) / 16) >= UPCONV_SMALL_MIN_TILES;
+}
 static void plan_conv(const stcd_engine& e, ConvOp& op, int groups, bool with_tile) {
     op.plan = conv_mfma_plan(op.g);
     op.small = conv_small_ok(op.g, op.plan);
+    if (!op.small && e.use_upconv_small && conv_small_s2_ok(op.g, op.plan) && upconv_small_fills(op.g)) op.small = op.small_s2 = true;
     if (e.use_res && !op.small) op.res = conv_res_plan(op.g, op.plan, groups);
     pick_gemm_or_res(e, op, op.g, groups);
     if (with_tile) pick_tile(e, op, op.g, groups);
@@ -563,6 +570,12 @@
         if (!op.gemm.ok) return;
         op.wf = ws.take(op.plan.wf_elems * 2);
         e.conv_ops.push_back(&op);
+    }
+    bool upconv_small(const ConvOp ops[4]) const {
+        if (e.dt != BF16 || !e.use_upconv_small) return false;
+        stcd_conv_geom g[4]; ConvMfmaPlan p[4];
+        for (int k = 0; k < 4; ++k) { if (ops[k].wf < 0) return false; g[k] = ops[k].g; p[k] = ops[k].plan; }
+        return upconv_small_ok(g, p) && upconv_small_fills(g[0]);
     }
     void wgrad(WgradOp& op, const stcd_conv_geom& g, int conv, int64_t in_off, int64_t dout_off, int stage = 0, int tap0 = 0,
                int wi_valid = 0, const int8_t* own_ky = nullptr, const int8_t* own_kx = nullptr) const {
@@ -946,6 +959,7 @@
         gd.ntaps = 9;
         for (int t = 0; t < 9; ++t) { gd.dy[t] = (int8_t)(t / 3 - 1); gd.dx[t] = (int8_t)(t % 3 - 1); }
         bind.conv(U.dgr, gd, U.conv, true, 0, U.C, U.C);
+        U.fwd_small = bind.upconv_small(U.fwd);
     }
     {
         const ConvW& cv = e.convs[e.final_conv];
@@ -1163,6 +1177,7 @@
             break;
         case ConvKernel::SMALL:
             if (bwd) snprintf(kname, sizeof(kname), "k_conv_small<bwd>");
+            else if (op.small_s2) snprintf(kname, sizeof(kname), "k_conv_small<s2>");
             else snprintf(kname, sizeof(kname), "k_conv_small<1, %d>", (op.g.ntaps * op.g.ci + 31) / 32 <= 5 ? 5 : 9);
             break;
         case ConvKernel::MFMA: snprintf(kname, sizeof(kname), "k_conv_mfma<%d>", op.plan.NT); break;
@@ -1248,7 +1263,7 @@
                            cv.name + " it was chosen for");
 }
 
-static bool exec_conv_x4(const Ctx& c, const ConvOp ops[4], const void* in, const float* bias, void* out) {
+static bool exec_conv_x4(const Ctx& c, const ConvOp ops[4], const void* in, const float* bias, void* out, bool small = false) {
     if (!mfma_on(c.e)) return false;
     stcd_conv_geom g[4]; ConvMfmaPlan p[4]; const void* wf[4];
     double fl = 0.0, by = 0.0;
@@ -1258,6 +1273,11 @@
         double f1, b1;
         conv_work(c.e, ops[k].g, ops[k].kreal, ops[k].nreal, &f1, &b1);
         fl += f1; by += b1;
+    }
+    if (small && c.e.use_small) {
+        ProfScope prof(c, PC_CONV, fl, by, "k_upconv_small");
+        if (launch_upconv_small(g, p, in, wf, bias, out, c.s) != 0) set_error("internal: k_upconv_small rejected the launch it was chosen for");
+        return true;
     }
     if (!conv_mfma_x4_ok(g, p)) return false;
     char kname[64];
@@ -1474,7 +1494,7 @@
 static void upconv_forward(const Ctx& c, const UpConv& U) {
     stcd_engine& e = c.e;
     const ConvW& cv = e.convs[U.conv];
-    if (!exec_conv_x4(c, U.fwd, c.at(U.in.off), c.params + cv.b_off, c.at(U.out.off)))
+    if (!exec_conv_x4(c, U.fwd, c.at(U.in.off), c.params + cv.b_off, c.at(U.out.off), U.fwd_small))
         for (int ph = 0; ph < 4; ++ph) exec_conv(c, U.fwd[ph], c.at(U.in.off), c.params + cv.b_off, c.at(U.out.off), false);
     launch_rep_pad(e.dt, c.at(U.out.off), U.out.ld, U.N, U.Ho, U.Wo, 2 * U.h, 2 * U.w, U.C, c.s);
 }
@@ -2929,6 +2949,7 @@
     e->use_skip_fused = !env_flag("STCD_NO_SKIP_FUSED", false);
     e->use_skip_recompute = !env_flag("STCD_NO_SKIP_RECOMPUTE", false);
     e->use_bwdsum = !env_flag("STCD_NO_BWDSUM_FUSE", false);
+    e->use_upconv_small = !env_flag("STCD_NO_UPCONV_SMALL", false);
     e->use_bwdsum_res = env_flag("STCD_BWDSUM_RES", false);
     e->use_virt = env_int("STCD_VIRT_ACT", e->use_virt) != 0;
     e->wg_side_on = env_int("STCD_WGRAD_SIDE", e->wg_side_on) != 0;
@@ -3465,6 +3486,8 @@
     STCD_CHECK(!bwd || k_small || k_res, "BatchNorm-backward sums: k_conv_small and k_conv_res only");
     STCD_CHECK(!(k_halo || k_dma) || groups == 1, "k_conv_halo and k_conv_dma know one group");
     STCD_CHECK(!(bwd && sums), "a data gradient with BatchNorm-backward sums carries no forward sums");
+    const bool in_sums = f->in_sum_acc != nullptr;
+    STCD_CHECK(!in_sums || (k_small && !sums && !bwd && groups == 1), "input sums: k_conv_small's stride-2 form alone, one group, no other sums");
     if (sums) {
         STCD_CHECK(f->sum_c0 >= 0 && f->sum_c >= 1 && f->sum_c0 + f->sum_c <= g->co, "the summed channel slice lies outside the output channels");
         STCD_CHECK(f->sum_scale1 > 0.f && f->sum_scale2 > 0.f, "the sum scales must be positive");
@@ -3495,7 +3518,11 @@
     const int64_t tiles16 = (int64_t)g->n * ((g->hm + 15) / 16) * ((g->wm + 15) / 16);
     ConvResPlan rp; ConvTilePlan tp; ConvGemmPlan gp; ConvHaloPlan hp; ConvDmaPlan dp;
     if (k_small) {
-        STCD_CHECK(conv_small_ok(*g, p) && conv_small_call_ok(*g, groups, nullptr), "geometry not supported by k_conv_small (one n-tile, <= 5 k-steps)");
+        const bool s2 = conv_small_s2_ok(*g, p);
+        STCD_CHECK((conv_small_ok(*g, p) || s2) && conv_small_call_ok(*g, groups, nullptr),
+                   "geometry not supported by k_conv_small (one n-tile, <= 5 k-steps; stride 2: 3x3 taps, 16 channels in)");
+        STCD_CHECK(!s2 || (groups == 1 && !sums && !bwd), "k_conv_small's stride-2 form knows one group and sums nothing of its output");
+        STCD_CHECK(!in_sums || s2, "input sums: k_conv_small's stride-2 form alone");
         STCD_CHECK(!bwd || conv_small_bwdsum_ok(*g), "k_conv_small forms BatchNorm-backward sums for 16 channels out, whole 8 x 16 tiles, 3 or 5 k-steps");
         f->blocks = conv_small_blocks(*g, groups);
         f->blocks_per_group = f->blocks / groups;
@@ -3524,13 +3551,51 @@
     }
     launch_pack_frag(*g, p, w, g->ci, g->co, scratch, s);
     int rc = 1;
-    if (k_small) rc = launch_conv_small(*g, in, scratch, bias, out, false, groups, acc, sC, s, nullptr, bwd ? &bs : nullptr);
+    if (k_small) rc = launch_conv_small(*g, in, scratch, bias, out, false, groups, acc, sC, s, nullptr, bwd ? &bs : nullptr, (long long*)f->in_sum_acc);
     else if (k_res) rc = launch_conv_res(*g, p, rp, in, scratch, bias, out, groups, acc, sC, s, sc0, s1, s2, nullptr, bwd ? &bs : nullptr);
     else if (k_tile) rc = launch_conv_tile(*g, p, tp, in, scratch, bias, out, groups, acc, sC, s, sc0, s1, s2);
     else if (k_gemm) rc = launch_conv_gemm(*g, p, gp, in, scratch, bias, out, groups, acc, sC, s, sc0, s1, s2, epi_on ? &epi : nullptr);
     else if (k_halo) rc = launch_conv_halo(*g, p, hp, in, scratch, bias, out, s, epi_on ? &epi : nullptr);
     else rc = launch_conv_dma(*g, p, dp, in, scratch, bias, out, s, epi_on ? &epi : nullptr);
     STCD_CHECK(rc == 0, "the named kernel's launcher rejected the combination");
+    STCD_HIP(hipGetLastError());
+    return 0;
+}
+int stcd_op_upconv(int impl, int n, int h, int w, int c, const void* in, int ldi, const float* wt, const float* bias, void* out,
+                   int ho, int wo, int ldo, void* scratch, int64_t scratch_bytes, void* hip_stream) {
+    STCD_CHECK(impl == 0 || impl == 1, "impl must be 0 (k_conv_mfma_x4) or 1 (k_upconv_small)");
+    STCD_CHECK(in && wt && out && scratch, "null pointer argument");
+    STCD_CHECK(n >= 1 && h >= 1 && w >= 1 && c >= 8 && c % 8 == 0 && c <= 64, "bad sizes (channels: a multiple of 8, <= 64)");
+    STCD_CHECK(ldi >= c && ldi % 8 == 0 && ldo >= c && ldo % 8 == 0, "pixel strides must be multiples of 8 and >= c");
+    STCD_CHECK(ho >= 2 * h && wo >= 2 * w, "the output buffer is smaller than 2h x 2w");
+    STCD_CHECK((int64_t)n * ho * wo * ldo < ((int64_t)1 << 40), "bad sizes");
+    UpConv U;
+    U.N = n; U.h = h; U.w = w; U.C = c; U.Ho = ho; U.Wo = wo;
+    stcd_conv_geom g[4]; ConvMfmaPlan p[4]; const void* wf[4];
+    int64_t off = 0;
+    for (int ph = 0; ph < 4; ++ph) {
+        int tap0;
+        g[ph] = geom_up_phase(U, ph >> 1, ph & 1, ldi, ldo, &tap0);
+        p[ph] = conv_mfma_plan(g[ph]);
+        STCD_CHECK(p[ph].ok, "geometry not supported by the MFMA kernels");
+        wf[ph] = (const char*)scratch + off;
+        off += (p[ph].wf_elems * 2 + 255) & ~(int64_t)255;
+    }
+    STCD_CHECK(scratch_bytes >= off, "scratch too small for the four fragment-order filters (64 KiB always suffice)");
+    if (impl == 1) STCD_CHECK(upconv_small_ok(g, p), "geometry not supported by k_upconv_small (16 channels, h % 8 == 0, w % 16 == 0)");
+    else STCD_CHECK(conv_mfma_x4_ok(g, p), "geometry not supported by k_conv_mfma_x4");
+    hipStream_t s = (hipStream_t)hip_stream;
+    static const int start[4] = {0, 1, 3, 5};
+    for (int ph = 0; ph < 4; ++ph) launch_pack_frag(g[ph], p[ph], wt + (int64_t)start[ph] * c * c, c, c, (void*)wf[ph], s);
+    const int rc = impl == 1 ? launch_upconv_small(g, p, in, wf, bias, out, s) : launch_conv_mfma_x4(g, p, in, wf, bias, out, s);
+    STCD_CHECK(rc == 0, "the named kernel's launcher rejected the launch");
+    STCD_HIP(hipGetLastError());
+    return 0;
+}
+int stcd_op_bias_grad(const void* dy, int ld, int64_t pixels, int c, void* acc, void* hip_stream) {
+    STCD_CHECK(dy && acc, "null pointer argument");
+    STCD_CHECK(pixels >= 1 && c >= 8 && c % 8 == 0 && c <= 256 && ld >= c && ld % 8 == 0, "bad sizes (channels: a multiple of 8, <= 256)");
+    launch_bias_grad(BF16, dy, ld, pixels, c, nullptr, (hipStream_t)hip_stream, (long long*)acc);
     STCD_HIP(hipGetLastError());
     return 0;
 }
diff --git a/stcd_amd/csrc/kernels_conv_mfma.hip b/stcd_amd/csrc/kernels_conv_mfma.hip
--- a/stcd_amd/csrc/kernels_conv_mfma.hip
+++ b/stcd_amd/csrc/kernels_conv_mfma.hip
@@ -964,13 +964,16 @@
     XfSrc xf;
     const bf16* bw_Y; int bw_ldy; const float* bw_stat; const float* bw_mask;
     float s1_scale, s2_scale;
+    long long* in_acc;
 };
 
-template <int NT, int KSMAX, bool XF = false, int FAST = 0, bool BWD = false>
+template <int NT, int KSMAX, bool XF = false, int FAST = 0, bool BWD = false, int MAXP = 3, bool INSUM = false>
 __global__ void __launch_bounds__(256, 2)
 k_conv_small(const ConvSmallArgs a) {
     constexpr bool EXACT = FAST >= 1, FULL = FAST == 2;
     static_assert(!BWD || (FULL && NT == 1 && !XF), "BWD: full-tile single-n-tile data gradients only");
+    static_assert(!INSUM || (!XF && !BWD && MAXP == 5), "INSUM: the 16-channel stride-2 data gradient only (two chunks per pixel)");
+    constexpr bool OSUM = MAXP == 3;
     extern __shared__ __attribute__((aligned(16))) char smem[];
     const int tid = threadIdx.x, lane = tid & 63, wid = tid >> 6;
     const int q = lane >> 4, r = lane & 15;
@@ -1005,7 +1008,6 @@
         for (int j = 0; j < 4; ++j) s1[t2][j] = s2[t2][j] = 0.f;
 
     const int npieces = a.HH * HWp * nch8;
-    constexpr int MAXP = 3;
     int poff[MAXP], phy[MAXP], phx[MAXP];
 #pragma unroll
     for (int p = 0; p < MAXP; ++p) {
@@ -1040,6 +1042,11 @@
         n_ += dn;
     };
     uint4 pre[MAXP];
+    unsigned in_own = 0;
+    float in_sum[8];
+#pragma unroll
+    for (int j = 0; j < 8; ++j) in_sum[j] = 0.f;
+    const unsigned in_he = (unsigned)(is * a.g.hm), in_we = (unsigned)(is * a.g.wm);
     unsigned xf_ok = 0;
     float4 xf_m0 = make_float4(1.f, 1.f, 1.f, 1.f), xf_m1 = xf_m0;
     float xf_sc[8], xf_sh[8];
@@ -1049,6 +1056,7 @@
         const int gy0 = y_ * 8 * is, gx0 = x_ * 16 * is;
         const bf16* org = a.in + (((int64_t)n_ * a.g.hi + gy0) * a.g.wi + gx0) * a.g.ldi;
         if constexpr (XF) xf_ok = 0;
+        if constexpr (INSUM) in_own = 0;
 #pragma unroll
         for (int p = 0; p < MAXP; ++p) {
             const unsigned gy = (unsigned)(gy0 + phy[p]), gx = (unsigned)(gx0 + phx[p]);
@@ -1056,6 +1064,7 @@
             if (gy < (unsigned)a.g.hi && gx < (unsigned)a.g.wi) {
                 pre[p] = *reinterpret_cast<const uint4*>(org + poff[p]);
                 if constexpr (XF) xf_ok |= 1u << p;
+                if constexpr (INSUM) in_own |= (phy[p] >= 0 && phx[p] >= 0 && gy < in_he && gx < in_we) ? 1u << p : 0u;
             }
         }
         if constexpr (XF) {
@@ -1078,6 +1087,18 @@
             for (int p = 0; p < MAXP; ++p) {
                 const int i = tid + p * 256;
                 if (i < npieces) *reinterpret_cast<uint4*>(halo0 + buf_ * halo_elems + i * 8) = pre[p];
+            }
+            if constexpr (INSUM) {
+#pragma unroll
+                for (int p = 0; p < MAXP; ++p) {
+                    const unsigned m = 0u - ((in_own >> p) & 1u);
+                    const unsigned w4[4] = {pre[p].x & m, pre[p].y & m, pre[p].z & m, pre[p].w & m};
+#pragma unroll
+                    for (int j = 0; j < 4; ++j) {
+                        in_sum[2 * j] += __uint_as_float(w4[j] << 16);
+                        in_sum[2 * j + 1] += __uint_as_float(w4[j] & 0xffff0000u);
+                    }
+                }
             }
         }
     };
@@ -1154,7 +1175,7 @@
                             s1[t2][j] += dz;
                             s2[t2][j] += dz * (y[j] - bw_mean[j]) * bw_inv[j];
                         }
-                    } else {
+                    } else if constexpr (OSUM) {
 #pragma unroll
                         for (int j = 0; j < 4; ++j) { s1[t2][j] += rv[j]; s2[t2][j] += rv[j] * rv[j]; }
                     }
@@ -1192,11 +1213,13 @@
                         for (int j = 0; j < 4; ++j)
                             if (cb + j < a.g.co) o[j] = (bf16)v[j];
                     }
-#pragma unroll
-                    for (int j = 0; j < 4; ++j) {
-                        const float rv = round_as<bf16>(v[j]);
-                        s1[t2][j] += rv;
-                        s2[t2][j] += rv * rv;
+                    if constexpr (OSUM) {
+#pragma unroll
+                        for (int j = 0; j < 4; ++j) {
+                            const float rv = round_as<bf16>(v[j]);
+                            s1[t2][j] += rv;
+                            s2[t2][j] += rv * rv;
+                        }
                     }
                 }
             }
@@ -1205,7 +1228,7 @@
         barrier_lds();
     }
 
-    if (a.stat_acc) {
+    if (OSUM && a.stat_acc) {
         float* red = reinterpret_cast<float*>(smem);
 #pragma unroll
         for (int t2 = 0; t2 < NT; ++t2)
@@ -1227,6 +1250,25 @@
 #pragma unroll
             for (int w = 0; w < 4; ++w) acc_ += red[(((w * NT + t2) * 4 + qq) * 4 + j) * 2 + which];
             if (c < a.cpad) bn_acc_add(a.stat_acc, bl, a.groups, a.cpad, grp, which, c, acc_, which ? a.s2_scale : a.s1_scale);
+        }
+    }
+    if constexpr (INSUM) {
+#pragma unroll
+        for (int j = 0; j < 8; ++j)
+#pragma unroll
+            for (int o = 2; o < 64; o <<= 1) in_sum[j] += __shfl_xor(in_sum[j], o, 64);
+        __syncthreads();
+        float* red = reinterpret_cast<float*>(smem);
+        if (lane < 2) {
+#pragma unroll
+            for (int j = 0; j < 8; ++j) red[(wid * 2 + lane) * 8 + j] = in_sum[j];
+        }
+        __syncthreads();
+        if (tid < 16) {
+            float acc_ = 0.f;
+#pragma unroll
+            for (int w = 0; w < 4; ++w) acc_ += red[w * 16 + tid];
+            bn_acc_add(a.in_acc, blockIdx.x, 1, Ci, 0, 0, tid, acc_, BN_BS);
         }
     }
 }
@@ -1241,11 +1283,17 @@
     const int HH = 7 * g.in_stride + (dymax - dymin) + 1, HWp = 15 * g.in_stride + (dxmax - dxmin) + 1;
     return ks <= 5 && nt <= 1 && g.ci <= 32 && HH * HWp * (g.ci / 8) <= 3 * 256;
 }
+bool conv_small_s2_ok(const stcd_conv_geom& g, const ConvMfmaPlan& p) {
+    if (!p.ok || !p.modeB || g.in_stride != 2 || g.ntaps != 9 || g.ci != 16 || g.co > 16) return false;
+    int dymin, dymax, dxmin, dxmax;
+    taps_extent(g, &dymin, &dymax, &dxmin, &dxmax);
+    return dymin == -1 && dymax == 1 && dxmin == -1 && dxmax == 1;
+}
 
 int conv_small_blocks(const stcd_conv_geom& g, int groups) {
     const int64_t ntiles = (int64_t)g.n * ((g.hm + 7) / 8) * ((g.wm + 15) / 16);
     int64_t per_group = ntiles / groups;
-    int64_t bpg = std::min<int64_t>(per_group, 2048 / groups);
+    int64_t bpg = std::min<int64_t>(per_group, (g.in_stride == 2 ? 1024 : 2048) / groups);
     if (bpg < 1) bpg = 1;
     return (int)(bpg * groups);
 }
@@ -1260,8 +1308,10 @@
     return !(xf && xf->on) || (xf->C == g.ci && xf->groups == groups);
 }
 int launch_conv_small(const stcd_conv_geom& g, const void* in, const void* wf_modeB, const float* bias, void* out,
-                      bool out_nchw, int groups, long long* stat_acc, int cpad, hipStream_t s, const XfSrc* xf, const BwdSum* bs) {
+                      bool out_nchw, int groups, long long* stat_acc, int cpad, hipStream_t s, const XfSrc* xf, const BwdSum* bs,
+                      long long* in_acc) {
     ConvSmallArgs a;
+    a.in_acc = in_acc;
     a.bw_Y = nullptr; a.bw_ldy = 0; a.bw_stat = nullptr; a.bw_mask = nullptr; a.s1_scale = BN_FS1; a.s2_scale = BN_FS2;
     a.g = g;
     a.in = (const bf16*)in; a.wf = (const bf16*)wf_modeB; a.bias = bias; a.out = out; a.out_nchw = out_nchw ? 1 : 0;
@@ -1290,6 +1340,7 @@
         lds = 2 * (size_t)a.halo_bytes + (size_t)xf->groups * 2 * xf->C * 4;
     }
     if (bs) {
+        if (in_acc || g.in_stride != 1) return 1;
         if (!conv_small_bwdsum_ok(g) || out_nchw || use_xf || nt != 1 || stat_acc || bs->groups != groups || !bs->acc) return 1;
         a.bw_Y = (const bf16*)bs->Y; a.bw_ldy = bs->ldy; a.bw_stat = bs->stat; a.bw_mask = bs->mask;
         a.stat_acc = bs->acc; a.cpad = g.co; a.s1_scale = BN_BS; a.s2_scale = BN_BS;
@@ -1299,6 +1350,14 @@
     }
     if (nt != 1) return 1;
     const bool full = !out_nchw && g.co == nt * 16 && g.hm % 8 == 0 && g.wm % 16 == 0;
+    if (g.in_stride != 1) {
+        if (g.in_stride != 2 || a.KS != 5 || a.HH * a.HWp * (g.ci / 8) > 5 * 256 || use_xf || out_nchw || stat_acc || groups != 1) return 1;
+        if (in_acc && g.ci != 16) return 1;
+        if (in_acc) { if (full) k_conv_small<1, 5, false, 2, false, 5, true><<<blocks, 256, lds, s>>>(a); else k_conv_small<1, 5, false, 1, false, 5, true><<<blocks, 256, lds, s>>>(a); }
+        else { if (full) k_conv_small<1, 5, false, 2, false, 5, false><<<blocks, 256, lds, s>>>(a); else k_conv_small<1, 5, false, 1, false, 5, false><<<blocks, 256, lds, s>>>(a); }
+        return 0;
+    }
+    if (in_acc) return 1;
 #define LAUNCH_SMALL(N_, K_, F_) do { if (use_xf) k_conv_small<N_, K_, true, F_><<<blocks, 256, lds, s>>>(a); else k_conv_small<N_, K_, false, F_><<<blocks, 256, lds, s>>>(a); } while (0)
 #define LAUNCH_SMALL_K(N_, K_) do { if (full) LAUNCH_SMALL(N_, K_, 2); else LAUNCH_SMALL(N_, K_, 1); } while (0)
 #define LAUNCH_SMALL_N(N_) do { \
@@ -1311,6 +1370,150 @@
 #undef LAUNCH_SMALL_K
 #undef LAUNCH_SMALL_N
 #undef LAUNCH_SMALL
+    return 0;
+}
+
+struct UpconvSmallArgs {
+    const bf16* in;
+    const bf16* wf[4];
+    const float* bias;
+    bf16* out;
+    int n, h, w, ldi, Ho, Wo, ldo;
+    int tiles_x, tiles_y, ntiles;
+};
+constexpr int UPS_HWP = 17, UPS_HH = 9, UPS_NPIECE = UPS_HH * UPS_HWP * 2, UPS_HALO_ELEMS = ((UPS_HH * UPS_HWP * 16 * 2 + 255) & ~255) / 2;
+
+__global__ void __launch_bounds__(256, 2)
+k_upconv_small(const UpconvSmallArgs a) {
+    constexpr int Ci = 16, HWp = UPS_HWP, MAXP = 2, NF = 5;
+    __shared__ __attribute__((aligned(16))) bf16 halo[2 * UPS_HALO_ELEMS];
+    const int tid = threadIdx.x, lane = tid & 63, wid = tid >> 6;
+    const int q = lane >> 4, r = lane & 15;
+
+    bf16x8 wreg[NF];
+    int aoff[NF];
+#pragma unroll
+    for (int f = 0; f < NF; ++f) {
+        const int ph = f < 4 ? f : 3, ks = f < 4 ? 0 : 1;
+        const int px = ph & 1, ntaps = ((ph >> 1) + 1) * (px + 1);
+        wreg[f] = *reinterpret_cast<const bf16x8*>(a.wf[ph] + ((int64_t)ks * 64 + lane) * 8);
+        const int kl = ks * 32 + 8 * q;
+        int t = kl / Ci, c = kl - t * Ci;
+        if (t >= ntaps) { t = 0; c = 0; }
+        const int tdy = t / (px + 1), tdx = t - tdy * (px + 1);
+        aoff[f] = (tdy * HWp + tdx) * Ci + c;
+    }
+    float bv[4];
+#pragma unroll
+    for (int j = 0; j < 4; ++j) bv[j] = a.bias ? a.bias[4 * q + j] : 0.f;
+
+    int poff[MAXP], phy[MAXP], phx[MAXP];
+#pragma unroll
+    for (int p = 0; p < MAXP; ++p) {
+        const int i = tid + p * 256;
+        const int ch = i & 1, pix = i >> 1;
+        phx[p] = pix % HWp;
+        const bool real = i < UPS_NPIECE;
+        phy[p] = real ? pix / HWp : (1 << 28);
+        poff[p] = real ? (phy[p] * a.w + phx[p]) * a.ldi + ch * 8 : 0;
+    }
+    const int tiles_img = a.tiles_x * a.tiles_y;
+    auto where = [&](int t_, int& n_, int& y_, int& x_) {
+        n_ = t_ / tiles_img;
+        const int rem = t_ - n_ * tiles_img;
+        y_ = rem / a.tiles_x; x_ = rem - y_ * a.tiles_x;
+    };
+    uint4 pre[MAXP];
+    auto fetch = [&](int n_, int y_, int x_) {
+        const int gy0 = y_ * 8, gx0 = x_ * 16;
+        const bf16* org = a.in + (((int64_t)n_ * a.h + gy0) * a.w + gx0) * a.ldi;
+#pragma unroll
+        for (int p = 0; p < MAXP; ++p) {
+            pre[p] = make_uint4(0, 0, 0, 0);
+            if ((unsigned)(gy0 + phy[p]) < (unsigned)a.h && (unsigned)(gx0 + phx[p]) < (unsigned)a.w)
+                pre[p] = *reinterpret_cast<const uint4*>(org + poff[p]);
+        }
+    };
+    auto stash = [&](int buf_) {
+#pragma unroll
+        for (int p = 0; p < MAXP; ++p) {
+            const int i = tid + p * 256;
+            if (i < UPS_NPIECE) *reinterpret_cast<uint4*>(halo + buf_ * UPS_HALO_ELEMS + i * 8) = pre[p];
+        }
+    };
+
+    int tile = blockIdx.x, buf = 0;
+    int tn = 0, tty = 0, ttx = 0;
+    if (tile < a.ntiles) { where(tile, tn, tty, ttx); fetch(tn, tty, ttx); stash(0); }
+    __syncthreads();
+    const int base0 = ((wid * 2) * HWp + r) * Ci, rowstep = HWp * Ci;
+    for (; tile < a.ntiles; tile += gridDim.x, buf ^= 1) {
+        int nn = 0, ny = 0, nx = 0;
+        const bool have_next = tile + (int)gridDim.x < a.ntiles;
+        if (have_next) { where(tile + gridDim.x, nn, ny, nx); fetch(nn, ny, nx); }
+        f32x4 acc[4][2];
+        const bf16* hb = halo + buf * UPS_HALO_ELEMS;
+#pragma unroll
+        for (int f = 0; f < NF; ++f) {
+            const int ph = f < 4 ? f : 3;
+            const bf16x8 a0 = *reinterpret_cast<const bf16x8*>(hb + base0 + aoff[f]);
+            const bf16x8 a1 = *reinterpret_cast<const bf16x8*>(hb + base0 + rowstep + aoff[f]);
+            const f32x4 z = f32x4{0.f, 0.f, 0.f, 0.f};
+            acc[ph][0] = __builtin_amdgcn_mfma_f32_16x16x32_bf16(wreg[f], a0, f < 4 ? z : acc[ph][0], 0, 0, 0);
+            acc[ph][1] = __builtin_amdgcn_mfma_f32_16x16x32_bf16(wreg[f], a1, f < 4 ? z : acc[ph][1], 0, 0, 0);
+        }
+        if (have_next) stash(buf ^ 1);
+        const int mx = ttx * 16 + r;
+#pragma unroll
+        for (int m = 0; m < 2; ++m) {
+            const int my = tty * 8 + wid * 2 + m;
+#pragma unroll
+            for (int py = 0; py < 2; ++py) {
+                bf16* orow = a.out + (((int64_t)tn * a.Ho + 2 * my + py) * a.Wo + 2 * mx) * a.ldo + 4 * q;
+#pragma unroll
+                for (int px = 0; px < 2; ++px) {
+                    const f32x4 v = acc[py * 2 + px][m];
+                    uint2 pk;
+                    pk.x = pack_bf16x2(v[0] + bv[0], v[1] + bv[1]);
+                    pk.y = pack_bf16x2(v[2] + bv[2], v[3] + bv[3]);
+                    *reinterpret_cast<uint2*>(orow + px * a.ldo) = pk;
+                }
+            }
+        }
+        tn = nn; tty = ny; ttx = nx;
+        barrier_lds();
+    }
+}
+
+bool upconv_small_ok(const stcd_conv_geom g[4], const ConvMfmaPlan p[4]) {
+    for (int ph = 0; ph < 4; ++ph) {
+        const stcd_conv_geom& k = g[ph];
+        const int py = ph >> 1, px = ph & 1;
+        if (!p[ph].ok || !p[ph].modeB || p[ph].NTtot != 1 || p[ph].KS != (ph == 3 ? 2 : 1)) return false;
+        if (k.ci != 16 || k.co != 16 || k.in_stride != 1 || k.out_stride != 2 || k.oy0 != py || k.ox0 != px) return false;
+        if (k.ntaps != (py + 1) * (px + 1) || k.hm != k.hi || k.wm != k.wi || k.hm % 8 != 0 || k.wm % 16 != 0) return false;
+        if (k.ho < 2 * k.hm || k.wo < 2 * k.wm || k.ldi < 16 || k.ldi % 8 != 0 || k.ldo < 16 || k.ldo % 4 != 0) return false;
+        if (k.n != g[0].n || k.hi != g[0].hi || k.wi != g[0].wi || k.ldi != g[0].ldi || k.ho != g[0].ho || k.wo != g[0].wo || k.ldo != g[0].ldo) return false;
+        int t = 0;
+        for (int dy = 0; dy <= py; ++dy)
+            for (int dx = 0; dx <= px; ++dx, ++t)
+                if (k.dy[t] != dy || k.dx[t] != dx) return false;
+    }
+    return true;
+}
+int launch_upconv_small(const stcd_conv_geom g[4], const ConvMfmaPlan p[4], const void* in, const void* const wf[4], const float* bias,
+                        void* out, hipStream_t s) {
+    if (!upconv_small_ok(g, p)) return 1;
+    UpconvSmallArgs a;
+    a.in = (const bf16*)in; a.bias = bias; a.out = (bf16*)out;
+    for (int ph = 0; ph < 4; ++ph) a.wf[ph] = (const bf16*)wf[ph];
+    a.n = g[0].n; a.h = g[0].hi; a.w = g[0].wi; a.ldi = g[0].ldi; a.Ho = g[0].ho; a.Wo = g[0].wo; a.ldo = g[0].ldo;
+    a.tiles_x = a.w / 16; a.tiles_y = a.h / 8;
+    const int64_t ntiles = (int64_t)a.n * a.tiles_x * a.tiles_y;
+    if (ntiles > INT32_MAX) return 1;
+    a.ntiles = (int)ntiles;
+    const int blocks = (int)std::min<int64_t>(ntiles, 1024);
+    k_upconv_small<<<blocks, 256, 0, s>>>(a);
     return 0;
 }
 
```

Result: no change. 7917 image-pairs/sec, median of 6 (+0.4%).
